# facebookresearch/DLRM-FlexFlow

Hardware: AMD Instinct MI355X
Metric: dlrm_training_samples_per_sec (higher is better)
Workload: dtype f32; 1 GPU; criteo-terabyte-shape: 26 tables (rows 39884406-39043-17289-7420-20263-3-7120-1543-63-38532951-2953546-403346-10-2208-11938-155-4-976-14-39979771-25641295-39664984-585935-12972-108-36), emb_dim 128, bag 1, bot 13-512-256-128, top 3456-1024-1024-512-256-1, cat interaction, SGD lr 0.01, MSE loss; global_batch=32768, per_gpu_batch=32768, parallelism=single GPU, hipGraph-replayed step, step_graph=True

## Files before the change

### dlrm_flexflow_amd/capi.py

```python
from __future__ import annotations

import ctypes as C
import os
import re

_HERE = os.path.dirname(os.path.abspath(__file__))
REPO_ROOT = os.path.dirname(_HERE)
HIP_LIB_PATH = os.path.join(_HERE, "csrc", "libffhip.so")
HEADER_PATH = os.path.join(REPO_ROOT, "include", "ff_hip.h")

FFH_OK = 0
FFH_ERR_BAD_ARG, FFH_ERR_HIP, FFH_ERR_UNSUPPORTED, FFH_ERR_WORKSPACE, FFH_ERR_NOMEM = -1, -2, -3, -4, -5
AC_MODE_NONE, AC_MODE_RELU, AC_MODE_SIGMOID, AC_MODE_TANH, AC_MODE_GELU = 10, 11, 12, 13, 14
AGGR_MODE_NONE, AGGR_MODE_SUM, AGGR_MODE_AVG = 20, 21, 22
MAX_TABLES = 64
EMB_CHUNK, EMB_CHUNK1 = 32, 1024
OPT_ZERO_GRAD = 1
CONCAT_BWD_OVERWRITE = 1
LINEAR_DX_OVERWRITE, LINEAR_ONLY_DW, LINEAR_ONLY_DX, LINEAR_DY_PREMASKED, LINEAR_DX_MASK_BY_X = 1, 2, 4, 8, 16
METRIC_ACCURACY, METRIC_MSE, METRIC_RMSE, METRIC_MAE = 1, 2, 4, 8

P = C.c_void_p
I = C.c_int
L = C.c_int64
# ... 692 lines not shown
        return getattr(self.lib, name)(self.ctx, *conv)

    def call(self, name: str, *args):
        self.base.check(self.rc(name, *args), name)


def cross_api(lib: FFHLib) -> CrossApi:
    return CrossApi(lib)


class AdagradApi:

    def __init__(self, lib: FFHLib):
        self.base = lib
        for name, (res, args) in _SIGS_ADAGRAD.items():
            fn = getattr(lib.lib, name, None)
            if fn is None:
                raise FFHError(f"{lib.path}: no Adagrad extension ({name} missing; include/ff_hip_adagrad.h)")
            fn.restype = res
            fn.argtypes = args
        got = lib.lib.ffh_adagrad_abi_version()
        if got != adagrad_header_abi_version():
            raise FFHError(f"{lib.path}: Adagrad ABI version {got}, include/ff_hip_adagrad.h says {adagrad_header_abi_version()} (rebuild)")
        self.lib = lib.lib
        self.ctx = lib.ctx

    def rc(self, name: str, *args) -> int:
        sig = _SIGS_ADAGRAD[name][1][1:]
        if len(args) != len(sig):
            raise TypeError(f"{name}: expected {len(sig)} args, got {len(args)}")
        conv = [ptr(a) if t is P else a for a, t in zip(args, sig)]
        return getattr(self.lib, name)(self.ctx, *conv)

    def call(self, name: str, *args):
        self.base.check(self.rc(name, *args), name)


def adagrad_api(lib: FFHLib) -> AdagradApi:
    return AdagradApi(lib)


class RowwiseApi:

    def __init__(self, lib: FFHLib):
        self.base = lib
        for name, (res, args) in _SIGS_ROWWISE.items():
            fn = getattr(lib.lib, name, None)
            if fn is None:
                raise FFHError(f"{lib.path}: no row-wise Adagrad extension ({name} missing; include/ff_hip_rowwise.h)")
            fn.restype = res
            fn.argtypes = args
        got = lib.lib.ffh_rowwise_abi_version()
        if got != rowwise_header_abi_version():
            raise FFHError(f"{lib.path}: row-wise Adagrad ABI version {got}, include/ff_hip_rowwise.h says {rowwise_header_abi_version()} (rebuild)")
        self.lib = lib.lib
        self.ctx = lib.ctx


def rowwise_api(lib: FFHLib) -> RowwiseApi:
    return RowwiseApi(lib)


FOLD_HEADER_PATH = os.path.join(REPO_ROOT, "include", "ff_hip_fold.h")


class FoldGroup(C.Structure):
    _fields_ = [("e", P), ("lde", L), ("col0", L), ("p", P), ("rows", L)]


class FoldSeg(C.Structure):
    _fields_ = [("k0", C.c_int32), ("len", C.c_int32)]


_SIGS_FOLD = {
    "ffh_fold_abi_version": (I, []),
    "ffh_fold_product": (I, [P, C.POINTER(FoldGroup), I, P, L, I, I, P]),
    "ffh_fold_gather_add": (I, [P, C.POINTER(EmbTable), I, I, I, L, I, P, L, P]),
    "ffh_fold_linear_fwd": (I, [P, P, L, P, L, P, P, I, I, L, I, C.POINTER(FoldSeg), I, P, L, P]),
    "ffh_fold_linear_fwd_plan": (I, [P, P, L, P, L, P, P, I, I, L, C.POINTER(FoldSeg), I, P, L]),
    "ffh_fold_segment_sum": (I, [P, C.POINTER(EmbTable), I, I, I, L, P]),
    "ffh_fold_dw_product": (I, [P, C.POINTER(FoldGroup), I, P, L, I, I, P]),
    "ffh_fold_linear_bwd_dw": (I, [P, P, L, P, L, P, P, I, I, L, C.POINTER(C.c_int32), I, P]),
    "ffh_fold_linear_bwd_dw_plan": (I, [P, P, L, P, L, P, P, I, I, L, C.POINTER(C.c_int32), I]),
}


def fold_header_symbols(header_path: str = FOLD_HEADER_PATH) -> list[str]:
    m = re.search(r"#define FFH_FOLD_API_LIST\(X\)(.*?)\n\n", open(header_path).read(), re.S)
    if not m:
        raise RuntimeError("FFH_FOLD_API_LIST not found in " + header_path)
    return re.findall(r"X\((\w+)\)", m.group(1))


def fold_header_abi_version(header_path: str = FOLD_HEADER_PATH) -> int:
    m = re.search(r"#define\s+FFH_FOLD_ABI_VERSION\s+(\d+)", open(header_path).read())
    if not m:
        raise RuntimeError("FFH_FOLD_ABI_VERSION not found in " + header_path)
    return int(m.group(1))


class FoldApi:

    def __init__(self, lib: "FFHLib"):
        self.base = lib
        for name, (res, args) in _SIGS_FOLD.items():
            fn = getattr(lib.lib, name, None)
            if fn is None:
                raise FFHError(f"{lib.path}: no fold extension ({name} missing; include/ff_hip_fold.h)")
            fn.restype = res
            fn.argtypes = args
        got = lib.lib.ffh_fold_abi_version()
        if got != fold_header_abi_version():
            raise FFHError(f"{lib.path}: fold ABI version {got}, include/ff_hip_fold.h says {fold_header_abi_version()} (rebuild)")
        self.lib = lib.lib
        self.ctx = lib.ctx

    @staticmethod
    def groups(entries) -> "C.Array":
        entries = list(entries)
        arr = (FoldGroup * len(entries))()
        for k, (e, lde, col0, p, rows) in enumerate(entries):
            arr[k] = FoldGroup(ptr(e), int(lde), int(col0), ptr(p), int(rows))
        return arr

    @staticmethod
    def segs(entries) -> "C.Array":
        entries = list(entries)
        arr = (FoldSeg * max(1, len(entries)))()
        for k, (k0, n) in enumerate(entries):
            arr[k] = FoldSeg(int(k0), int(n))
        return arr

    def rc(self, name: str, *args) -> int:
        sig = _SIGS_FOLD[name][1][1:]
        if len(args) != len(sig):
            raise TypeError(f"{name}: expected {len(sig)} args, got {len(args)}")
        conv = [ptr(a) if t is P else a for a, t in zip(args, sig)]
        return getattr(self.lib, name)(self.ctx, *conv)

    def call(self, name: str, *args):
        self.base.check(self.rc(name, *args), name)


def fold_api(lib: "FFHLib") -> FoldApi:
    return FoldApi(lib)


_hip_singleton: FFHLib | None = None


def load_hip(device: int = 0) -> FFHLib:
    global _hip_singleton
    if _hip_singleton is None:
        import torch
        _hip_singleton = FFHLib(HIP_LIB_PATH, device)
        if not _hip_singleton.backend.startswith("hip"):
            raise FFHError(f"{HIP_LIB_PATH} is not the HIP backend ({_hip_singleton.backend})")
    return _hip_singleton
```

### dlrm_flexflow_amd/csrc/fold.hip

```cpp
#include "fold_sum.h"
#include "linear_gemm.h"

#include "../../include/ff_hip_fold.h"

using namespace ffh_gemm;

namespace {

typedef float f32x4 __attribute__((ext_vector_type(4)));

struct FoldGemmGroup { const float* a; int64_t lda; int64_t wcol0; float* c; int64_t ldc; int rows; int tile0; };
struct FoldGemmArgs {
  FoldGemmGroup grp[FFH_FOLD_MAX_GROUPS];
  ffh_fold_seg  seg[FFH_FOLD_MAX_SEGS];
  const float*  w; int64_t ldw;
  const float*  bias;
  const float*  addend; int64_t ldadd;
  int ngroups, nseg, N, act, ntiles;
};
static_assert(sizeof(FoldGemmArgs) <= 4096, "kernel arguments");

template <bool EPI>
__global__ __launch_bounds__(256) void fold_gemm_kernel(const FoldGemmArgs g) {
  ffh_kernel_prio();
  const int lane = threadIdx.x & 63;
  const int wave = __builtin_amdgcn_readfirstlane((int)(threadIdx.x >> 6));
  const int c = lane & 15, q = lane >> 4;
  const int wt = (int)blockIdx.x * 4 + wave;
  if (wt >= g.ntiles) return;
  int gi = 0;
  while (gi + 1 < g.ngroups && g.grp[gi + 1].tile0 <= wt) gi++;
  const FoldGemmGroup G = g.grp[gi];
  const int ct = g.N / 64, local = wt - G.tile0;
  const int r0 = (local / ct) * 32, n0 = (local % ct) * 64;
  const float* ap[2];
  const float* wp[4];
#pragma unroll
  for (int mt = 0; mt < 2; mt++) {
    int r = r0 + 16 * mt + c;
    if (r > G.rows - 1) r = G.rows - 1;
    ap[mt] = G.a + (int64_t)r * G.lda + 4 * q;
  }
#pragma unroll
  for (int nt = 0; nt < 4; nt++) wp[nt] = g.w + (int64_t)(n0 + 16 * nt + c) * g.ldw + G.wcol0 + 4 * q;
  f32x4 acc[4][2];
#pragma unroll
  for (int nt = 0; nt < 4; nt++)
#pragma unroll
    for (int mt = 0; mt < 2; mt++) acc[nt][mt] = f32x4{0.f, 0.f, 0.f, 0.f};
  for (int si = 0; si < g.nseg; si++) {
    const int k0 = g.seg[si].k0, k1 = k0 + g.seg[si].len;
    for (int k = k0; k < k1; k += 16) {
      f32x4 a[2], b[4];
#pragma unroll
      for (int mt = 0; mt < 2; mt++) a[mt] = *reinterpret_cast<const f32x4*>(ap[mt] + k);
#pragma unroll
      for (int nt = 0; nt < 4; nt++) b[nt] = *reinterpret_cast<const f32x4*>(wp[nt] + k);
#pragma unroll
      for (int e = 0; e < 4; e++)
#pragma unroll
        for (int nt = 0; nt < 4; nt++)
#pragma unroll
          for (int mt = 0; mt < 2; mt++) acc[nt][mt] = __builtin_amdgcn_mfma_f32_16x16x4f32(b[nt][e], a[mt][e], acc[nt][mt], 0, 0, 0);
    }
  }
#pragma unroll
  for (int mt = 0; mt < 2; mt++) {
    const int r = r0 + 16 * mt + c;
    if (r >= G.rows) continue;
#pragma unroll
    for (int nt = 0; nt < 4; nt++) {
      const int n = n0 + 16 * nt + 4 * q;
      f32x4 v = acc[nt][mt];
      if constexpr (EPI) {
        if (g.addend) v += *reinterpret_cast<const f32x4*>(g.addend + (int64_t)r * g.ldadd + n);
        if (g.bias) v += f32x4{g.bias[n], g.bias[n + 1], g.bias[n + 2], g.bias[n + 3]};
        if (g.act != FFH_AC_MODE_NONE) { v.x = act_apply(v.x, g.act); v.y = act_apply(v.y, g.act); v.z = act_apply(v.z, g.act); v.w = act_apply(v.w, g.act); }
      }
      *reinterpret_cast<f32x4*>(G.c + (int64_t)r * G.ldc + n) = v;
    }
  }
}

struct FoldGatherTable { const int64_t* idx; const float* p; };
// ... 25 lines not shown
        }
      }
#pragma unroll
      for (int u = 0; u < 4; u++)
        if (j0 + u < n) acc = (j0 + u == 0) ? v[u] : acc + v[u];
    }
    *reinterpret_cast<f32x4*>(g.S + b * g.ldS + cv) = acc;
  }
}

constexpr int FOLD_DW_EP_LD = 68;
struct FoldDwGroup { const float* g; const float* e; int64_t lde; int64_t col0; int rows; int tile0; };
struct FoldDwArgs {
  FoldDwGroup grp[FFH_FOLD_MAX_GROUPS];
  float* dw; int64_t lddw;
  int ngroups, out, d, ntiles;
};
static_assert(sizeof(FoldDwArgs) <= 4096, "kernel arguments");

__global__ __launch_bounds__(256) void fold_dw_product_kernel(const FoldDwArgs g) {
  __shared__ __attribute__((aligned(16))) float ep_all[4][16 * FOLD_DW_EP_LD];
  ffh_kernel_prio();
  const int lane = threadIdx.x & 63;
  const int wave = __builtin_amdgcn_readfirstlane((int)(threadIdx.x >> 6));
  const int c = lane & 15, q = lane >> 4;
  const int wt = (int)blockIdx.x * 4 + wave;
  if (wt >= g.ntiles) return;
  int gi = 0;
  while (gi + 1 < g.ngroups && g.grp[gi + 1].tile0 <= wt) gi++;
  const FoldDwGroup G = g.grp[gi];
  const int ot = g.out / 64, dt = g.d / 64, local = wt - G.tile0;
  const int chunk = local / (ot * dt), rem = local - chunk * (ot * dt);
  const int o0 = (rem / dt) * 64, d0 = (rem % dt) * 64;
  const int rb = chunk * FFH_FOLD_DW_CHUNK;
  const int re = rb + FFH_FOLD_DW_CHUNK < G.rows ? rb + FFH_FOLD_DW_CHUNK : G.rows;
  const float* gp = G.g + o0 + 4 * c;
  const float* epn = G.e + d0 + 4 * c;
  f32x4 acc[4][4];
#pragma unroll
  for (int tm = 0; tm < 4; tm++)
#pragma unroll
    for (int tn = 0; tn < 4; tn++) acc[tm][tn] = f32x4{0.f, 0.f, 0.f, 0.f};
  f32x4 a[4], b[4], an[4], bn[4];
  auto load16 = [&](int k, f32x4* av, f32x4* bv) {
#pragma unroll
    for (int u = 0; u < 4; u++) {
      const int r = k + 4 * u + q;
      const int rc = r < re ? r : re - 1;
      av[u] = *reinterpret_cast<const f32x4*>(gp + (int64_t)rc * g.out);
      bv[u] = *reinterpret_cast<const f32x4*>(epn + (int64_t)rc * G.lde);
      if (r >= re) av[u] = f32x4{0.f, 0.f, 0.f, 0.f};
    }
  };
  load16(rb, a, b);
  for (int k = rb; k < re; k += 16) {
    if (k + 16 < re) load16(k + 16, an, bn);
#pragma unroll
    for (int u = 0; u < 4; u++)
#pragma unroll
      for (int tm = 0; tm < 4; tm++)
#pragma unroll
        for (int tn = 0; tn < 4; tn++) acc[tm][tn] = __builtin_amdgcn_mfma_f32_16x16x4f32(a[u][tm], b[u][tn], acc[tm][tn], 0, 0, 0);
#pragma unroll
    for (int u = 0; u < 4; u++) { a[u] = an[u]; b[u] = bn[u]; }
  }
  float* const ep = ep_all[wave];
  float* crow = g.dw + (int64_t)o0 * g.lddw + G.col0 + d0 + lane;
#pragma unroll
  for (int p = 0; p < 4; p++) {
    if (q == p) {
#pragma unroll
      for (int tm = 0; tm < 4; tm++)
#pragma unroll
        for (int i = 0; i < 4; i++)
          *reinterpret_cast<f32x4*>(ep + (4 * i + tm) * FOLD_DW_EP_LD + 4 * c) = f32x4{acc[tm][0][i], acc[tm][1][i], acc[tm][2][i], acc[tm][3][i]};
    }
    __builtin_amdgcn_wave_barrier();
#pragma unroll
    for (int r = 0; r < 16; r++) atomicAdd(crow + (int64_t)(16 * p + r) * g.lddw, ep[r * FOLD_DW_EP_LD + lane]);
    __builtin_amdgcn_wave_barrier();
  }
}

inline bool al16(const void* p) { return ((uintptr_t)p & 15) == 0; }

int fold_dw_check(ffh_ctx* c, const float* x, int64_t ldx, const float* dy, int64_t lddy, const float* dw, int in, int out, int64_t batch,
                  const int32_t* kept, int nkept) {
  FFH_REQUIRE(c, in > 0 && out > 0 && batch >= 0 && ldx >= in && lddy >= out, "fold_linear_bwd_dw: bad dims");
  FFH_REQUIRE(c, batch == 0 || (x && dy && dw), "fold_linear_bwd_dw: null pointer");
  FFH_REQUIRE(c, batch < (1LL << 31), "fold_linear_bwd_dw: batch too large");
  FFH_REQUIRE(c, nkept >= 1 && kept, "fold_linear_bwd_dw: bad tile list");
  for (int i = 0; i < nkept; i++)
    FFH_REQUIRE(c, kept[i] >= 0 && ((int64_t)kept[i] + 1) * FFH_FOLD_DW_NTILE <= in && (i == 0 || kept[i] > kept[i - 1]), "fold_linear_bwd_dw: tiles must ascend inside [0, in_dim)");
  return FFH_OK;
}
GemmArgs fold_dw_gemm(const float* x, int64_t ldx, const float* dy, int64_t lddy, float* dw, float* db, int in, int out, int64_t batch) {
  GemmArgs g{};
  g.A = dy; g.sAm = 1; g.sAk = lddy;
  g.B = x; g.sBn = 1; g.sBk = ldx;
  g.C = dw; g.ldc = in;
  g.M = out; g.N = in; g.K = (int)batch;
  g.epi = EPI_ATOMIC; g.act = FFH_AC_MODE_NONE;
  g.db = db;
  return g;
}

int fold_fwd_check(ffh_ctx* c, const float* x, int64_t ldx, const float* y, int64_t ldy, const float* w, int in, int out, int64_t batch,
                   const ffh_fold_seg* keep, int nkeep, const float* addend, int64_t ldadd) {
  FFH_REQUIRE(c, in > 0 && out > 0 && batch >= 0 && ldx >= in && ldy >= out, "fold_linear_fwd: bad dims");
  FFH_REQUIRE(c, batch == 0 || (x && y && w), "fold_linear_fwd: null pointer");
  FFH_REQUIRE(c, batch < (1LL << 31), "fold_linear_fwd: batch too large");
  FFH_REQUIRE(c, nkeep >= 0 && (nkeep == 0 || keep), "fold_linear_fwd: bad segment list");
  FFH_REQUIRE(c, !addend || ldadd >= out, "fold_linear_fwd: bad addend");
  int prev = 0;
  for (int i = 0; i < nkeep; i++) {
    FFH_REQUIRE(c, keep[i].k0 >= prev && keep[i].len > 0 && (int64_t)keep[i].k0 + keep[i].len <= in, "fold_linear_fwd: segments must ascend inside [0, in_dim)");
    prev = keep[i].k0 + keep[i].len;
  }
  return FFH_OK;
}
bool fold_fwd_served(const ffh_ctx* c, const float* x, int64_t ldx, const float* y, int64_t ldy, const float* w, int in, int out,
                     const ffh_fold_seg* keep, int nkeep, const float* addend, int64_t ldadd) {
  if (c->math_mode != FFH_MATH_DEFAULT) return false;
  if (in % FFH_FOLD_KTILE || out % FFH_FOLD_NTILE || nkeep > FFH_FOLD_MAX_SEGS) return false;
  if (!al16(x) || !al16(y) || !al16(w) || ldx % 4 || ldy % 4 || (addend && (!al16(addend) || ldadd % 4))) return false;
  for (int i = 0; i < nkeep; i++)
    if (keep[i].k0 % FFH_FOLD_KTILE || keep[i].len % FFH_FOLD_KTILE) return false;
  return true;
}
bool fold_keep_mask(int in, const ffh_fold_seg* keep, int nkeep, unsigned long long mask[2], int* nk_kept) {
  mask[0] = mask[1] = 0;
  *nk_kept = 0;
  if (in % 64 || in > 128 * 64) return false;
  const ffh_fold_seg all{0, in};
  if (nkeep == 0) { keep = &all; nkeep = 1; }
  for (int i = 0; i < nkeep; i++) {
    if (keep[i].k0 % 64 || keep[i].len % 64) return false;
    for (int kt = keep[i].k0 / 64; kt < (keep[i].k0 + keep[i].len) / 64; kt++) { mask[kt >> 6] |= 1ull << (kt & 63); (*nk_kept)++; }
  }
  return *nk_kept > 0;
}
GemmArgs fold_fwd_gemm(const float* x, int64_t ldx, float* y, int64_t ldy, const float* w, const float* bias, int in, int out, int64_t batch, int act) {
  GemmArgs g{};
  g.A = x; g.sAm = ldx; g.sAk = 1;
  g.B = w; g.sBn = in; g.sBk = 1;
  g.C = y; g.ldc = ldy; g.bias = bias;
  g.M = (int)batch; g.N = out; g.K = in;
  g.epi = EPI_STORE; g.act = act;
  return g;
}

}

extern "C" {

int ffh_fold_abi_version(void) { return FFH_FOLD_ABI_VERSION; }

int ffh_fold_product(ffh_ctx* c, const ffh_fold_group* groups, int ngroups, const float* w, int64_t ldw, int d, int out, ffh_stream s) {
  FFH_REQUIRE(c, groups && w && ngroups >= 1 && d > 0 && out > 0 && ldw >= d, "fold_product: bad arguments");
  if (ngroups > FFH_FOLD_MAX_GROUPS || d % FFH_FOLD_KTILE || out % FFH_FOLD_NTILE || !al16(w) || ldw % 4)
    return ffh_fail(c, FFH_ERR_UNSUPPORTED, "fold_product: d a multiple of 16, out_dim a multiple of 64, at most 64 tables, aligned weight");
  FoldGemmArgs a{};
  int64_t tiles = 0;
  for (int i = 0; i < ngroups; i++) {
    const ffh_fold_group& gr = groups[i];
    FFH_REQUIRE(c, gr.e && gr.p && gr.rows >= 1 && gr.rows < (1LL << 31) && gr.lde >= d && gr.col0 >= 0 && gr.col0 + d <= ldw, "fold_product: bad group");
    if (!al16(gr.e) || !al16(gr.p) || gr.lde % 4 || gr.col0 % FFH_FOLD_KTILE) return ffh_fail(c, FFH_ERR_UNSUPPORTED, "fold_product: group not aligned");
// ... 51 lines not shown
  unsigned long long mask[2]; int nk = 0;
  if (fold_keep_mask(in, keep, nkeep, mask, &nk) && (!bias || al16(bias))) {
    const int r = launch_gemm_sk_fold(c, g, mask, nk, addend, ldadd, false, s, "fold_linear_fwd gemm");
    if (r != 0) return r < 0 ? r : FFH_OK;
  }
  FoldGemmArgs a{};
  a.grp[0] = FoldGemmGroup{x, ldx, 0, y, ldy, (int)batch, 0};
  if (nkeep == 0) { a.seg[0] = ffh_fold_seg{0, in}; a.nseg = 1; }
  else { for (int i = 0; i < nkeep; i++) a.seg[i] = keep[i]; a.nseg = nkeep; }
  const int64_t tiles = ((batch + 31) / 32) * (out / 64);
  FFH_REQUIRE(c, tiles < (1LL << 30), "fold_linear_fwd: too many tiles");
  a.w = w; a.ldw = in; a.bias = bias; a.addend = addend; a.ldadd = ldadd; a.ngroups = 1; a.N = out; a.act = act; a.ntiles = (int)tiles;
  hipLaunchKernelGGL(fold_gemm_kernel<true>, dim3((unsigned)((tiles + 3) / 4)), dim3(256), 0, as_stream(s), a);
  FFH_LAUNCH_CHECK(c, "fold_gemm_kernel (forward)");
  ffh_route_add(c, "fold_linear_fwd gemm|mfma_32x64x16");
  return FFH_OK;
}

int ffh_fold_segment_sum(ffh_ctx* c, const ffh_emb_table* tables, int ntables, int in_dim, int width, int64_t batch, ffh_stream s) {
  FFH_REQUIRE(c, tables && ntables >= 1 && in_dim >= 1 && width > 0 && batch >= 0, "fold_segment_sum: bad arguments");
  if (ntables > FFH_MAX_TABLES || batch * in_dim >= (1LL << 31)) return ffh_fail(c, FFH_ERR_UNSUPPORTED, "fold_segment_sum: at most 64 tables, batch * in_dim < 2^31");
  for (int t = 0; t < ntables; t++)
    FFH_REQUIRE(c, tables[t].weight && tables[t].num_entries >= 1 && (batch == 0 || (tables[t].idx && tables[t].io && tables[t].ld >= width)), "fold_segment_sum: bad table");
  if (batch > 0 && (!c->ws || c->ws_bytes < ffh_embedding_bwd_workspace_bytes(ntables, in_dim, width, batch) || ((uintptr_t)c->ws & 15)))
    return ffh_fail(c, FFH_ERR_WORKSPACE, "fold_segment_sum: workspace too small (ffh_embedding_bwd_workspace_bytes) or not 16-byte aligned");
  if (batch > 0) {
    const int wide = ffh_emb::fold_sum_wide(c, tables, ntables, in_dim, width, batch, s);
    if (wide != 0) return wide < 0 ? wide : FFH_OK;
  }
  for (int t = 0; t < ntables;) {
    char* p0 = (char*)tables[t].weight;
    size_t bytes = 0;
    for (; t < ntables && (char*)tables[t].weight == p0 + bytes; t++) bytes += (size_t)tables[t].num_entries * (size_t)width * 4;
    const int rc = ffh_zero(c, p0, bytes, s);
    if (rc != FFH_OK) return rc;
  }
  if (batch == 0) return FFH_OK;
  return ffh_embedding_bwd_sgd_fused_multi(c, tables, ntables, in_dim, width, batch, FFH_AGGR_MODE_SUM, -1.0f, s);
}

int ffh_fold_dw_product(ffh_ctx* c, const ffh_fold_group* groups, int ngroups, float* dw, int64_t lddw, int d, int out, ffh_stream s) {
  FFH_REQUIRE(c, groups && dw && ngroups >= 1 && d > 0 && out > 0 && lddw >= d, "fold_dw_product: bad arguments");
  if (ngroups > FFH_FOLD_MAX_GROUPS || d % 64 || out % FFH_FOLD_NTILE) return ffh_fail(c, FFH_ERR_UNSUPPORTED, "fold_dw_product: d and out_dim multiples of 64, at most 64 tables");
  FoldDwArgs a{};
  int64_t tiles = 0;
  for (int i = 0; i < ngroups; i++) {
    const ffh_fold_group& gr = groups[i];
    FFH_REQUIRE(c, gr.e && gr.p && gr.rows >= 1 && gr.rows < (1LL << 31) && gr.lde >= d && gr.col0 >= 0 && gr.col0 + d <= lddw, "fold_dw_product: bad group");
    if (!al16(gr.e) || !al16(gr.p) || gr.lde % 4) return ffh_fail(c, FFH_ERR_UNSUPPORTED, "fold_dw_product: group not aligned");
    a.grp[i] = FoldDwGroup{gr.p, gr.e, gr.lde, gr.col0, (int)gr.rows, (int)tiles};
    tiles += ((gr.rows + FFH_FOLD_DW_CHUNK - 1) / FFH_FOLD_DW_CHUNK) * (out / 64) * (d / 64);
    FFH_REQUIRE(c, tiles < (1LL << 30), "fold_dw_product: too many rows");
  }
  a.dw = dw; a.lddw = lddw; a.ngroups = ngroups; a.out = out; a.d = d; a.ntiles = (int)tiles;
  hipLaunchKernelGGL(fold_dw_product_kernel, dim3((unsigned)((tiles + 3) / 4)), dim3(256), 0, as_stream(s), a);
  FFH_LAUNCH_CHECK(c, "fold_dw_product_kernel");
  return FFH_OK;
}

int ffh_fold_linear_bwd_dw_plan(ffh_ctx* c, const float* x, int64_t ldx, const float* dy, int64_t lddy, const float* dw, const float* db, int in, int out,
                                int64_t batch, const int32_t* kept, int nkept) {
  const int rc = fold_dw_check(c, x, ldx, dy, lddy, dw, in, out, batch, kept, nkept);
  if (rc != FFH_OK) return rc;
  if (batch == 0 || c->math_mode != FFH_MATH_DEFAULT) return 0;
  const GemmArgs g = fold_dw_gemm(x, ldx, dy, lddy, const_cast<float*>(dw), const_cast<float*>(db), in, out, batch);
  if (!gemm_sk_serves(c, g, SK_FORM_DW)) return 0;
  return launch_gemm_sk_kept(c, g, kept, nkept, true, nullptr, "") == 1 ? 1 : 0;
}

int ffh_fold_linear_bwd_dw(ffh_ctx* c, const float* x, int64_t ldx, const float* dy, int64_t lddy, float* dw, float* db, int in, int out, int64_t batch,
                           const int32_t* kept, int nkept, ffh_stream s) {
  const int rc = fold_dw_check(c, x, ldx, dy, lddy, dw, in, out, batch, kept, nkept);
  if (rc != FFH_OK) return rc;
  ffh_route_clear(c);
  if (batch == 0 || c->math_mode != FFH_MATH_DEFAULT) return ffh_fail(c, FFH_ERR_UNSUPPORTED, "fold_linear_bwd_dw: empty batch / math mode not served");
  const GemmArgs g = fold_dw_gemm(x, ldx, dy, lddy, dw, db, in, out, batch);
  if (!gemm_sk_serves(c, g, SK_FORM_DW)) return ffh_fail(c, FFH_ERR_UNSUPPORTED, "fold_linear_bwd_dw: the layer's weight gradient does not run the stream-K form");
  const int r = launch_gemm_sk_kept(c, g, kept, nkept, false, s, "fold_linear_bwd_dw gemm");
  if (r < 0) return r;
  if (r == 0) return ffh_fail(c, FFH_ERR_UNSUPPORTED, "fold_linear_bwd_dw: too few kept tiles for the stream-K form, deterministic mode, or a bias gradient without tile 0");
  return FFH_OK;
}

}
```

### dlrm_flexflow_amd/csrc/linear_gemm.h

```cpp
#pragma once
#include "ffh_common.h"

#include <hip/hip_runtime.h>

namespace ffh_gemm {

typedef float f32x16 __attribute__((ext_vector_type(16)));

enum { EPI_STORE = 0, EPI_ADD = 1, EPI_ATOMIC = 2 };

struct GemmArgs {
  const float* A;
  const float* B;
  float*       C;
  const float* bias;
  int64_t sAm, sAk, sBn, sBk, ldc;
  int64_t bsA, bsB, bsC;
  int M, N, K;
  int k_per_split;
  int splitk;
  int epi;
  int act;
  const float* act_y;
  int64_t      ld_act_y;
  float*       db;
  int          fuse;
  const float* mask;
  int64_t      ldmask;
  const ffh_col_dest* colmap;
  float* colsum;
  const unsigned short* A16;
  const unsigned short* B16;
  unsigned short*       C16;
  int                   a_not_twinned;
  int                   db_done;
};

constexpr int kSplitGran = 32;

__device__ __forceinline__ float act_apply(float v, int act) {
  if (act == FFH_AC_MODE_RELU) return v > 0.0f ? v : 0.0f;
  if (act == FFH_AC_MODE_SIGMOID) return 1.0f / (1.0f + expf(-v));
  if (act == FFH_AC_MODE_GELU) {
    constexpr float B = 0.7978845608028654f, C = 0.035677408136300125f;
    return v * (0.5f + 0.5f * tanhf(v * (C * v * v + B)));
  }
  return v;
}

__device__ __forceinline__ float4 load4_guard(const float* p, bool row_ok, int c0, int climit, bool vec_ok) {
  float4 v = make_float4(0.f, 0.f, 0.f, 0.f);
  if (!row_ok) return v;
  if (vec_ok && c0 + 3 < climit) return ld4u(p);
  if (c0 + 0 < climit) v.x = p[0];
  if (c0 + 1 < climit) v.y = p[1];
  if (c0 + 2 < climit) v.z = p[2];
  if (c0 + 3 < climit) v.w = p[3];
  return v;
}

template <typename K>
bool glds_set_lds(K kern, int bytes) {
  if (hipFuncSetAttribute((const void*)kern, hipFuncAttributeMaxDynamicSharedMemorySize, bytes) != hipSuccess) { (void)hipGetLastError(); return false; }
  return true;
}

inline bool use_bf16(const ffh_ctx* c, int in, int out, int64_t batch) {
  if (in < FFH_BF16_MIN_DIM || out < FFH_BF16_MIN_DIM) return false;
  if (c->math_mode == FFH_MATH_TENSOR_OP_BF16) return true;
  return c->math_mode == FFH_MATH_FP32_SPLIT_BF16X3_ALL || (c->math_mode == FFH_MATH_FP32_SPLIT_BF16X3 && 2.0 * (double)batch * (double)in * (double)out >= FFH_BF16X3_MIN_FLOP);
}

enum { BF16_FORM_FWD = 0,
       BF16_FORM_DW = 1,
       BF16_FORM_DX = 2,
       BF16_FORM_DX_MASK = 3 };
int launch_gemm_bf16_form(ffh_ctx* c, GemmArgs& g, int form, ffh_stream s, const char* name);
int launch_gemm_bf16_dma(ffh_ctx* c, const GemmArgs& g, int form, ffh_stream s, const char* name);
int launch_gemm_x3_dma(ffh_ctx* c, const GemmArgs& g, int form, ffh_stream s, const char* name);
float* dw_tile_slots(const ffh_ctx* c, ffh_stream s, int64_t tiles, int splitk, int64_t ldc);
void launch_dw_tile_reduce(const float* slots, float* C, int64_t ldc, int M, int N, int64_t tiles, int splitk, ffh_stream s);

enum { SK_FORM_FWD = 0, SK_FORM_DX = 1, SK_FORM_DW = 2 };
bool gemm_sk_serves(const ffh_ctx* c, const GemmArgs& g, int form);
int launch_gemm_sk(ffh_ctx* c, const GemmArgs& g, int form, ffh_stream s, const char* name);
int launch_gemm_sk_fold(ffh_ctx* c, const GemmArgs& g, const unsigned long long keep[2], int nk_kept, const float* addend, int64_t ldadd, bool dry,
                        ffh_stream s, const char* name);
int launch_gemm_sk_kept(ffh_ctx* c, const GemmArgs& g, const int* tiles, int nkept, bool dry, ffh_stream s, const char* name);

}
```

### dlrm_flexflow_amd/csrc/linear_sk.hip

```cpp
#include "linear_gemm.h"

#include <stdlib.h>
#include <atomic>
#include <type_traits>
#include <utility>

using namespace ffh_gemm;

namespace {

typedef float f32x4 __attribute__((ext_vector_type(4)));
typedef unsigned u32x4 __attribute__((ext_vector_type(4)));

constexpr int SK_BM = 128, SK_BN = 128, SK_BK = 64;
constexpr int SK_LDS_KC = 128 * 256 + 32 * 32;
constexpr int SK_LDS_KR = 64 * 512;
constexpr int sk_lds_kc_a(int TMW) { return 32 * TMW * 256 + 32 * 32; }

enum { SK_EPI_FWD = 0, SK_EPI_DX_STORE = 1, SK_EPI_DX_ADD = 2, SK_EPI_DW_ATOMIC = 3, SK_EPI_DX_CMAP = 4 };

struct SkArgs {
  const float* A; const float* B; float* C;
  const float* bias;
  float*       db;
  const float* mask;
  const ffh_col_dest* colmap;
  float*       colsum;
  int64_t lda, ldb, ldc, ldmask;
  int M, N, K;
  int act;
  unsigned a_bytes, b_bytes, bias_bytes, mask_bytes;
  float*    sk_slots;
  unsigned* sk_cnt;
};

struct SkArgsFold : SkArgs {
  unsigned long long keep[2];
  unsigned           nk_kept;
  const float*       addend;
  int64_t            ldadd;
};

struct SkArgsKept : SkArgs {
  unsigned       nkept;
  unsigned short tile[128];
};

template <int... I, class F>
__device__ __forceinline__ void sk_static_for_impl(std::integer_sequence<int, I...>, F&& f) { (f(std::integral_constant<int, I>{}), ...); }
template <int N_, class F>
__device__ __forceinline__ void sk_static_for(F&& f) { sk_static_for_impl(std::make_integer_sequence<int, N_>{}, static_cast<F&&>(f)); }

#define SK_PIN() __builtin_amdgcn_sched_barrier(0)

constexpr int SK_EP_LD = 68;
constexpr int SK_EP_ROWS = 16;
constexpr int SK_EP_WAVE = SK_EP_ROWS * SK_EP_LD * 4;

template <bool AKR, bool BKR, int EPI, bool DB = false, bool SPLIT = false, int TMW = 4, bool FOLD = false, bool KEPT = false>
__global__ __launch_bounds__(256, 1) void gemm_sk_kernel(const std::conditional_t<KEPT, SkArgsKept, std::conditional_t<FOLD, SkArgsFold, SkArgs>> g) {
  static_assert(!KEPT || (EPI == SK_EPI_DW_ATOMIC && AKR && BKR && !FOLD), "kept column tiles: the weight-gradient form");
  static_assert(!FOLD || (EPI == SK_EPI_FWD && !SPLIT && !DB && TMW == 4), "kept k-tiles + addend: the whole-tile forward form");
  static_assert(!DB || (EPI == SK_EPI_DW_ATOMIC && AKR), "the bias gradient rides on the weight-gradient form");
  static_assert(!SPLIT || EPI != SK_EPI_DW_ATOMIC, "the weight gradient meets by atomics");
  static_assert(TMW == 4 || (TMW == 2 && !AKR && EPI != SK_EPI_DW_ATOMIC), "64-row tiles: forward and data gradient (A k-contiguous)");
  extern __shared__ __attribute__((aligned(16))) char sk_lds[];
  constexpr bool ATOMIC = EPI == SK_EPI_DW_ATOMIC;
  constexpr bool STREAMK = ATOMIC || SPLIT;
  constexpr int BM = 32 * TMW;
  constexpr int NM = 64 * TMW;
  constexpr int NPA = 2 * TMW, NP = NPA + 8;
  constexpr int LDS_A = AKR ? SK_LDS_KR : sk_lds_kc_a(TMW);
  char* const ldsA = sk_lds;
  char* const ldsB = sk_lds + LDS_A;
  const int tid = threadIdx.x, lane = tid & 63;
  const int wave = __builtin_amdgcn_readfirstlane(tid >> 6);
  const int wy = wave >> 1, wx = wave & 1;
  const int c16 = lane & 15, q = lane >> 4;

  const int fra = AKR ? (q * 2048 + wy * 256 + c16 * 16) : ((16 * TMW * wy + TMW * c16) * 256 + (16 * wy + c16) * 32 + q * 16);
  const int frb = BKR ? (q * 2048 + wx * 256 + c16 * 16) : ((64 * wx + 4 * c16) * 256 + (16 * wx + c16) * 32 + q * 16);
  const int srowA = AKR ? (tid >> 5) : (tid >> 4), schA = AKR ? (tid & 31) : (tid & 15);
  const int srowB = BKR ? (tid >> 5) : (tid >> 4), schB = BKR ? (tid & 31) : (tid & 15);
  const unsigned voffA = (unsigned)((srowA * g.lda + schA * 4) * 4);
  const unsigned voffB = (unsigned)((srowB * g.ldb + schB * 4) * 4);
  const int swA = AKR ? (srowA * 512 + schA * 16) : (srowA * 256 + (srowA / TMW) * 32 + schA * 16);
  const int swB = BKR ? (srowB * 512 + schB * 16) : (srowB * 256 + (srowB >> 2) * 32 + schB * 16);
  constexpr int SW_STEP_A = AKR ? 4096 : (4096 + (16 / TMW) * 32), SW_STEP_B = BKR ? 4096 : 4224;
  const unsigned ioffA = (unsigned)((AKR ? 8 : 16) * g.lda * 4), ioffB = (unsigned)((BKR ? 8 : 16) * g.ldb * 4);
  const unsigned kadvA = AKR ? (unsigned)(SK_BK * g.lda * 4) : (unsigned)(SK_BK * 4), kadvB = BKR ? (unsigned)(SK_BK * g.ldb * 4) : (unsigned)(SK_BK * 4);

  const __amdgpu_buffer_rsrc_t rsA = __builtin_amdgcn_make_buffer_rsrc(const_cast<float*>(g.A), 0, g.a_bytes, 0x00020000);
  const __amdgpu_buffer_rsrc_t rsB = __builtin_amdgcn_make_buffer_rsrc(const_cast<float*>(g.B), 0, g.b_bytes, 0x00020000);

  unsigned nbx = (unsigned)(g.N / SK_BN);
  if constexpr (KEPT) nbx = g.nkept;
  const unsigned nby = (unsigned)(g.M / BM), ntiles = nbx * nby;
  unsigned nk = (unsigned)(g.K / SK_BK);
  if constexpr (FOLD) nk = g.nk_kept;
  auto first_kept = [&]() -> unsigned {
    if constexpr (FOLD) return g.keep[0] ? (unsigned)__builtin_ctzll(g.keep[0]) : 64u + (unsigned)__builtin_ctzll(g.keep[1]);
    else return 0u;
  };
  auto next_kept = [&](unsigned p) -> unsigned {
    if constexpr (FOLD) {
      p++;
      if (p < 64u) {
        const unsigned long long m = g.keep[0] >> p;
        if (m) return p + (unsigned)__builtin_ctzll(m);
        p = 64u;
      }
      const unsigned long long m = p < 128u ? g.keep[1] >> (p - 64u) : 0ull;
      return m ? p + (unsigned)__builtin_ctzll(m) : p;
    } else return p + 1u;
  };
  const unsigned G = gridDim.x, w = blockIdx.x;
  const unsigned total_it = ntiles * nk;
  const unsigned wperm = (w & 7u) * (G >> 3) + (w >> 3);
  unsigned it_b, it_e;
  const unsigned ipw = (total_it + G - 1) / G;
  const unsigned rng = SPLIT ? wperm : w;
  if (STREAMK) {
    it_b = rng * ipw; it_e = it_b + ipw < total_it ? it_b + ipw : total_it;
    if (it_b > total_it) it_b = total_it;
  } else {
    const unsigned mine = ntiles / G + (wperm < ntiles % G ? 1u : 0u);
    it_b = 0; it_e = mine * nk;
  }
  const unsigned n_it = it_e - it_b;
  if (n_it == 0) return;

  struct Cursor { unsigned seq, kt, m0, n0, offA, offB, kp; };
  auto place = [&](Cursor& c) {
    unsigned lin;
    if (STREAMK) lin = it_b / nk + c.seq;
    else lin = c.seq * G + wperm;
    if (lin >= ntiles) lin = ntiles - 1;
    const unsigned by = lin / nbx, bx = lin - by * nbx;
    c.m0 = by * BM;
    if constexpr (KEPT) c.n0 = (unsigned)g.tile[bx] * SK_BN;
    else c.n0 = bx * SK_BN;
    c.kp = FOLD ? first_kept() : c.kt;
    c.offA = (AKR ? c.m0 * 4u : (unsigned)(c.m0 * g.lda * 4)) + c.kp * kadvA;
    c.offB = (BKR ? c.n0 * 4u : (unsigned)(c.n0 * g.ldb * 4)) + c.kp * kadvB;
// ... 382 lines not shown
    const hipError_t e = hipGetLastError();
    if (e == hipErrorInvalidValue || e == hipErrorInvalidConfiguration || e == hipErrorLaunchOutOfResources || e == hipErrorSharedObjectInitFailed) return 0;
    if (e != hipSuccess) return ffh_fail_hip(c, e, name);
  }
  { char tok[96]; snprintf(tok, sizeof tok, "%s|sk_%dx128x64%s%s%s|wgs=%d", name, 32 * p.tmw, g.colmap ? "|colmap" : "", p.split ? "|streamk" : "", a.colsum ? "|colsum" : "", G); ffh_route_add(c, tok); }
  return 1;
}

int launch_gemm_sk_fold(ffh_ctx* c, const GemmArgs& g, const unsigned long long keep[2], int nk_kept, const float* addend, int64_t ldadd, bool dry,
                        ffh_stream s, const char* name) {
  if (g.K % SK_BK || g.K > 128 * SK_BK || nk_kept < 1 || nk_kept > g.K / SK_BK) return 0;
  if (addend && !sk_aligned(addend, ldadd)) return 0;
  GemmArgs gk = g;
  gk.K = nk_kept * SK_BK;
  SkPlan p{};
  if (!sk_plan(c, gk, SK_FORM_FWD, p) || p.split || p.tmw != 4) return 0;
  const int64_t a_bytes = ((int64_t)(g.M - 1) * p.lda + g.K) * 4, b_bytes = ((int64_t)(g.N - 1) * p.ldb + g.K) * 4;
  if (a_bytes >= (1LL << 32) || b_bytes >= (1LL << 32)) return 0;
  if (dry) return 1;
  SkArgsFold a{};
  a.A = g.A; a.B = g.B; a.C = g.C; a.bias = g.bias;
  a.lda = p.lda; a.ldb = p.ldb; a.ldc = g.ldc;
  a.M = g.M; a.N = g.N; a.K = g.K; a.act = g.act;
  a.a_bytes = (unsigned)a_bytes; a.b_bytes = (unsigned)b_bytes;
  a.bias_bytes = g.bias ? (unsigned)g.N * 4u : 0u;
  a.keep[0] = keep[0]; a.keep[1] = keep[1]; a.nk_kept = (unsigned)nk_kept; a.addend = addend; a.ldadd = ldadd;
  {
    auto kern = gemm_sk_kernel<false, false, SK_EPI_FWD, false, false, 4, true>;
    constexpr int LDSB = 2 * SK_LDS_KC;
    static std::atomic<signed char> ok[64];
    const int dev = c->device & 63;
    if (ok[dev].load(std::memory_order_acquire) == 0) ok[dev].store(sk_set_lds(kern, LDSB) ? 1 : -1, std::memory_order_release);
    if (ok[dev].load(std::memory_order_acquire) < 0) return 0;
    hipLaunchKernelGGL(kern, dim3((unsigned)p.G), dim3(256), LDSB, as_stream(s), a);
    const hipError_t e = hipGetLastError();
    if (e == hipErrorInvalidValue || e == hipErrorInvalidConfiguration || e == hipErrorLaunchOutOfResources || e == hipErrorSharedObjectInitFailed) return 0;
    if (e != hipSuccess) return ffh_fail_hip(c, e, name);
  }
  { char tok[96]; snprintf(tok, sizeof tok, "%s|sk_128x128x64|kept=%d/%d%s|wgs=%d", name, nk_kept, g.K / SK_BK, addend ? "|addend" : "", p.G); ffh_route_add(c, tok); }
  return 1;
}

int launch_gemm_sk_kept(ffh_ctx* c, const GemmArgs& g, const int* tiles, int nkept, bool dry, ffh_stream s, const char* name) {
  if (g.N % SK_BN || g.N / SK_BN > 128 || nkept < 1 || nkept > g.N / SK_BN) return 0;
  for (int i = 0; i < nkept; i++)
    if (tiles[i] < 0 || tiles[i] >= g.N / SK_BN || (i > 0 && tiles[i] <= tiles[i - 1])) return 0;
  if (g.db && tiles[0] != 0) return 0;
  GemmArgs gk = g;
  gk.N = nkept * SK_BN;
  SkPlan p{};
  if (!sk_plan(c, gk, SK_FORM_DW, p)) return 0;
  const int64_t b_bytes = ((int64_t)(g.K - 1) * p.ldb + g.N) * 4;
  if (b_bytes >= (1LL << 32)) return 0;
  if (dry) return 1;
  SkArgsKept a{};
  a.A = g.A; a.B = g.B; a.C = g.C; a.db = g.db;
  a.lda = p.lda; a.ldb = p.ldb; a.ldc = g.ldc;
  a.M = g.M; a.N = g.N; a.K = g.K; a.act = g.act;
  a.a_bytes = (unsigned)p.a_bytes; a.b_bytes = (unsigned)b_bytes;
  a.nkept = (unsigned)nkept;
  for (int i = 0; i < nkept; i++) a.tile[i] = (unsigned short)tiles[i];
  constexpr int LDSB = 2 * SK_LDS_KR + 4 * SK_EP_WAVE;
#define FFH_SK_KEPT_LAUNCH(DBV)                                                                                  \
  {                                                                                                              \
    auto kern = gemm_sk_kernel<true, true, SK_EPI_DW_ATOMIC, DBV, false, 4, false, true>;                        \
    static std::atomic<signed char> ok[64];       \
    const int dev = c->device & 63;                                                                              \
    if (ok[dev].load(std::memory_order_acquire) == 0) ok[dev].store(sk_set_lds(kern, LDSB) ? 1 : -1, std::memory_order_release); \
    if (ok[dev].load(std::memory_order_acquire) < 0) return 0;                                                   \
    hipLaunchKernelGGL(kern, dim3((unsigned)p.G), dim3(256), LDSB, as_stream(s), a);                             \
  }
  if (g.db) FFH_SK_KEPT_LAUNCH(true)
  else FFH_SK_KEPT_LAUNCH(false)
#undef FFH_SK_KEPT_LAUNCH
  {
    const hipError_t e = hipGetLastError();
    if (e == hipErrorInvalidValue || e == hipErrorInvalidConfiguration || e == hipErrorLaunchOutOfResources || e == hipErrorSharedObjectInitFailed) return 0;
    if (e != hipSuccess) return ffh_fail_hip(c, e, name);
  }
  { char tok[96]; snprintf(tok, sizeof tok, "%s|sk_128x128x64|kept=%d/%d%s|wgs=%d", name, nkept, g.N / SK_BN, g.db ? "|db" : "", p.G); ffh_route_add(c, tok); }
  return 1;
}

}
```

### dlrm_flexflow_amd/host/backend.cc

```cpp
#include "backend.h"

#include <dlfcn.h>
#include <cstdio>
#include <cstdlib>
#include <map>
#include <mutex>

static bool g_env_override = false;
std::string default_backend_path() {
  if (const char* e = getenv("FFH_BACKEND_LIB")) { g_env_override = true; return std::string(e); }
  Dl_info info;
  std::string dir = ".";
  if (dladdr((void*)&default_backend_path, &info) && info.dli_fname) {
    std::string p(info.dli_fname);
    size_t k = p.rfind('/');
    if (k != std::string::npos) dir = p.substr(0, k);
  }
  return dir + "/../csrc/libffhip.so";
}

const KernelApi* load_kernel_api(const std::string& path_in) {
  static std::map<std::string, KernelApi*>& cache = *new std::map<std::string, KernelApi*>();
  static std::mutex mu;
  std::lock_guard<std::mutex> lock(mu);
  const std::string path = path_in.empty() ? default_backend_path() : path_in;
  auto it = cache.find(path);
  if (it != cache.end()) return it->second;
  void* h = dlopen(path.c_str(), RTLD_NOW | RTLD_LOCAL);
  if (!h) {
    fprintf(stderr, "FATAL: cannot load kernel library %s: %s\n"
                    "       build it with: python -c 'import __graft_entry__ as g; g.build()'\n", path.c_str(), dlerror());
    abort();
  }
  KernelApi* api = new KernelApi();
  api->handle = h;
  api->path = path;
  api->overridden = !path_in.empty() || g_env_override;
#define FFH_LOAD(name)                                                        \
  api->name = reinterpret_cast<decltype(api->name)>(dlsym(h, #name));         \
  if (!api->name) {                                                           \
    fprintf(stderr, "FATAL: %s does not export %s\n", path.c_str(), #name);   \
    abort();                                                                  \
  }
  FFH_API_LIST(FFH_LOAD)
#undef FFH_LOAD
  if (api->ffh_abi_version() != FFH_ABI_VERSION) {
    fprintf(stderr, "FATAL: %s has ABI version %d, expected %d\n", path.c_str(), api->ffh_abi_version(), FFH_ABI_VERSION);
    abort();
  }
  if (dlsym(h, "ffh_bf16_abi_version")) {
    KernelApiBf16* b = new KernelApiBf16();
#define FFH_LOAD(name)                                                        \
  b->name = reinterpret_cast<decltype(b->name)>(dlsym(h, #name));             \
  if (!b->name) {                                                             \
    fprintf(stderr, "FATAL: %s exports part of include/ff_hip_bf16.h: %s is missing\n", path.c_str(), #name);   \
    abort();                                                                  \
  }
    FFH_BF16_API_LIST(FFH_LOAD)
#undef FFH_LOAD
    if (b->ffh_bf16_abi_version() != FFH_BF16_ABI_VERSION) {
      fprintf(stderr, "FATAL: %s has bf16 ABI version %d, expected %d\n", path.c_str(), b->ffh_bf16_abi_version(), FFH_BF16_ABI_VERSION);
      abort();
    }
    api->bf16 = b;
  }
  if (dlsym(h, "ffh_ctr_abi_version")) {
    KernelApiCtr* b = new KernelApiCtr();
#define FFH_LOAD(name)                                                        \
  b->name = reinterpret_cast<decltype(b->name)>(dlsym(h, #name));             \
  if (!b->name) {                                                             \
    fprintf(stderr, "FATAL: %s exports part of include/ff_hip_ctr.h: %s is missing\n", path.c_str(), #name);   \
    abort();                                                                  \
  }
    FFH_CTR_API_LIST(FFH_LOAD)
#undef FFH_LOAD
    if (b->ffh_ctr_abi_version() != FFH_CTR_ABI_VERSION) {
      fprintf(stderr, "FATAL: %s has CTR ABI version %d, expected %d\n", path.c_str(), b->ffh_ctr_abi_version(), FFH_CTR_ABI_VERSION);
      abort();
    }
    api->ctr = b;
  }
  if (dlsym(h, "ffh_lr_abi_version")) {
    KernelApiLr* b = new KernelApiLr();
#define FFH_LOAD(name)                                                        \
  b->name = reinterpret_cast<decltype(b->name)>(dlsym(h, #name));             \
  if (!b->name) {                                                             \
    fprintf(stderr, "FATAL: %s exports part of include/ff_hip_lr.h: %s is missing\n", path.c_str(), #name);   \
// ... 9 lines not shown
  }
  if (dlsym(h, "ffh_data_abi_version")) {
    KernelApiData* b = new KernelApiData();
#define FFH_LOAD(name)                                                        \
  b->name = reinterpret_cast<decltype(b->name)>(dlsym(h, #name));             \
  if (!b->name) {                                                             \
    fprintf(stderr, "FATAL: %s exports part of include/ff_hip_data.h: %s is missing\n", path.c_str(), #name);   \
    abort();                                                                  \
  }
    FFH_DATA_API_LIST(FFH_LOAD)
#undef FFH_LOAD
    if (b->ffh_data_abi_version() != FFH_DATA_ABI_VERSION) {
      fprintf(stderr, "FATAL: %s has data ABI version %d, expected %d\n", path.c_str(), b->ffh_data_abi_version(), FFH_DATA_ABI_VERSION);
      abort();
    }
    api->data = b;
  }
  if (dlsym(h, "ffh_cross_abi_version")) {
    KernelApiCross* b = new KernelApiCross();
#define FFH_LOAD(name)                                                        \
  b->name = reinterpret_cast<decltype(b->name)>(dlsym(h, #name));             \
  if (!b->name) {                                                             \
    fprintf(stderr, "FATAL: %s exports part of include/ff_hip_cross.h: %s is missing\n", path.c_str(), #name);   \
    abort();                                                                  \
  }
    FFH_CROSS_API_LIST(FFH_LOAD)
#undef FFH_LOAD
    if (b->ffh_cross_abi_version() != FFH_CROSS_ABI_VERSION) {
      fprintf(stderr, "FATAL: %s has cross ABI version %d, expected %d\n", path.c_str(), b->ffh_cross_abi_version(), FFH_CROSS_ABI_VERSION);
      abort();
    }
    api->cross = b;
  }
  if (dlsym(h, "ffh_digest_abi_version")) {
    KernelApiDigest* b = new KernelApiDigest();
#define FFH_LOAD(name)                                                        \
  b->name = reinterpret_cast<decltype(b->name)>(dlsym(h, #name));             \
  if (!b->name) {                                                             \
    fprintf(stderr, "FATAL: %s exports part of include/ff_hip_digest.h: %s is missing\n", path.c_str(), #name);   \
    abort();                                                                  \
  }
    FFH_DIGEST_API_LIST(FFH_LOAD)
#undef FFH_LOAD
    if (b->ffh_digest_abi_version() != FFH_DIGEST_ABI_VERSION) {
      fprintf(stderr, "FATAL: %s has digest ABI version %d, expected %d\n", path.c_str(), b->ffh_digest_abi_version(), FFH_DIGEST_ABI_VERSION);
      abort();
    }
    api->digest = b;
  }
  if (dlsym(h, "ffh_adagrad_abi_version")) {
    KernelApiAdagrad* b = new KernelApiAdagrad();
#define FFH_LOAD(name)                                                        \
  b->name = reinterpret_cast<decltype(b->name)>(dlsym(h, #name));             \
  if (!b->name) {                                                             \
    fprintf(stderr, "FATAL: %s exports part of include/ff_hip_adagrad.h: %s is missing\n", path.c_str(), #name);   \
    abort();                                                                  \
  }
    FFH_ADAGRAD_API_LIST(FFH_LOAD)
#undef FFH_LOAD
    if (b->ffh_adagrad_abi_version() != FFH_ADAGRAD_ABI_VERSION) {
      fprintf(stderr, "FATAL: %s has Adagrad ABI version %d, expected %d\n", path.c_str(), b->ffh_adagrad_abi_version(), FFH_ADAGRAD_ABI_VERSION);
      abort();
    }
    api->adagrad = b;
  }
  if (dlsym(h, "ffh_rowwise_abi_version")) {
    KernelApiRowwise* b = new KernelApiRowwise();
#define FFH_LOAD(name)                                                        \
  b->name = reinterpret_cast<decltype(b->name)>(dlsym(h, #name));             \
  if (!b->name) {                                                             \
    fprintf(stderr, "FATAL: %s exports part of include/ff_hip_rowwise.h: %s is missing\n", path.c_str(), #name);   \
    abort();                                                                  \
  }
    FFH_ROWWISE_API_LIST(FFH_LOAD)
#undef FFH_LOAD
    if (b->ffh_rowwise_abi_version() != FFH_ROWWISE_ABI_VERSION) {
      fprintf(stderr, "FATAL: %s has row-wise Adagrad ABI version %d, expected %d\n", path.c_str(), b->ffh_rowwise_abi_version(), FFH_ROWWISE_ABI_VERSION);
      abort();
    }
    api->rowwise = b;
  }
  if (dlsym(h, "ffh_fold_abi_version")) {
    KernelApiFold* b = new KernelApiFold();
#define FFH_LOAD(name)                                                        \
  b->name = reinterpret_cast<decltype(b->name)>(dlsym(h, #name));             \
  if (!b->name) {                                                             \
    fprintf(stderr, "FATAL: %s exports part of include/ff_hip_fold.h: %s is missing\n", path.c_str(), #name);   \
    abort();                                                                  \
  }
    FFH_FOLD_API_LIST(FFH_LOAD)
#undef FFH_LOAD
    if (b->ffh_fold_abi_version() != FFH_FOLD_ABI_VERSION) {
      fprintf(stderr, "FATAL: %s has fold ABI version %d, expected %d\n", path.c_str(), b->ffh_fold_abi_version(), FFH_FOLD_ABI_VERSION);
      abort();
    }
    api->fold = b;
  }
  if (path_in.empty() && g_env_override)
    fprintf(stderr, "[DLRM] FFH_BACKEND_LIB: kernel library %s (%s)\n", path.c_str(), api->ffh_backend_name());
  cache[path] = api;
  return api;
}
```

### dlrm_flexflow_amd/host/ffmodel.h

```cpp
#pragma once

#include <cstddef>
#include <cstdint>
#include <condition_variable>
#include <deque>
#include <functional>
#include <map>
#include <mutex>
#include <thread>
#include <string>
#include <vector>

#include "../../include/ff_hip.h"
#include "../../include/ff_hip_bf16.h"
#include "../../include/ff_hip_ctr.h"
#include "../../include/ff_hip_lr.h"
#include "../../include/ff_hip_cross.h"
#include "../../include/ff_hip_adagrad.h"
#include "../../include/ff_hip_rowwise.h"
#include "../../include/ff_hip_fold.h"
#include "ffcomm.h"

enum ActiMode { AC_MODE_NONE = 10, AC_MODE_RELU = 11, AC_MODE_SIGMOID = 12, AC_MODE_TANH = 13, AC_MODE_GELU = 14 };
enum AggrMode { AGGR_MODE_NONE = 20, AGGR_MODE_SUM = 21, AGGR_MODE_AVG = 22 };
// ... 8 lines not shown
};
enum CompMode { COMP_MODE_TRAINING = 70, COMP_MODE_INFERENCE = 71 };
enum ParameterSyncType { NONE = 80, PS = 81, NCCL = 82 };
enum MetricsType {
  METRICS_ACCURACY = 1001,
  METRICS_CATEGORICAL_CROSSENTROPY = 1002,
  METRICS_SPARSE_CATEGORICAL_CROSSENTROPY = 1004,
  METRICS_MEAN_SQUARED_ERROR = 1008,
  METRICS_ROOT_MEAN_SQUARED_ERROR = 1016,
  METRICS_MEAN_ABSOLUTE_ERROR = 1032,
  METRICS_BINARY_CROSSENTROPY = 2001,
  METRICS_AUC = 2002,
};
enum OperatorType { OP_INPUT, OP_LINEAR, OP_EMBEDDING, OP_CONCAT, OP_BATCHMATMUL, OP_TRANSPOSE, OP_RESHAPE, OP_FLAT, OP_TRIL, OP_DOT_INTERACTION, OP_CROSS_COMBINE };

#define MAX_TENSOR_DIM 4
#define MAX_NUM_INPUTS 256
#define MAX_OPNAME 64

class FFModel;
class Op;
struct KernelApi;

struct ParallelConfig {
  enum DeviceType { GPU = 0, CPU = 1 };
  ParallelConfig() : device_type(GPU), nDims(0) { for (int& d : dim) d = 1; }
  int num_parts() const { int n = 1; for (int i = 0; i < nDims; i++) n *= dim[i]; return n; }
  bool is_data_parallel() const;
  bool operator==(const ParallelConfig& rhs) const;
  DeviceType device_type;
  int nDims, dim[MAX_TENSOR_DIM];
  std::vector<int> device_ids;
};
typedef size_t MappingTagID;
bool load_strategies_from_file(const std::string& filename, std::map<MappingTagID, ParallelConfig>& strategies);
bool save_strategies_to_file(const std::string& filename, const std::map<std::string, ParallelConfig>& strategies);

class FFConfig {
 public:
  FFConfig();
  void parse_args(char** argv, int argc);
  int epochs, batchSize, printFreq;
  int numNodes, cpusPerNode, workersPerNode;
  float learningRate, weightDecay;
  size_t workSpaceSize;
  bool syntheticInput, profiling, perform_fusion;
  CompMode computationMode;
  std::string dataset_path;
  std::string import_strategy_file, export_strategy_file;
  std::map<MappingTagID, ParallelConfig> strategies;
  static MappingTagID get_hash_id(const std::string& pcname);
  bool find_parallel_config(int ndims, const std::string& pcname, ParallelConfig& config) const;
  std::string save_checkpoint_dir, load_checkpoint_dir;
  int checkpoint_every_epochs;
  std::string backend_lib;
  int device;
  uint64_t seed;
  bool enable_graph;
  bool overlap_embedding;
  bool dense_embedding_update;
  int64_t column_shard_rows;
  bool deterministic;
  bool fp32_split_bf16x3;
  bool allow_tensor_op_math_conversion;
  bool bf16_convert_twins;
  bool bf16_exact_small_backward;
  bool bf16_twins, force_async_launch;
  bool capture_exchange;
  bool pad_linear_k;
  bool sparse_embedding_optimizer;
  int early_sort;
  bool dx_colsum;
  bool dx_scatter;
  bool fuse_pair;
  int  bucket_allreduce;
  bool direct_allreduce;
  int64_t allreduce_bucket_floats;
  int64_t big_dw_min_weights;
  int  big_dw_chunks;
  int  trace_mode;
  bool fold_small_tables;
  int64_t fold_max_rows;
  bool fold_dw;
  bool mlp_chain;
  int64_t mlp_chain_max_batch;
  int64_t mlp_chain_fwd_max_batch;
  int64_t mlp_chain_fwd_min_batch;
  int64_t mlp_chain_max_weights;
  bool attach_events;
  bool timing_events;
  int driver_loss;
  int eval_batches;
  int synthetic_labels;
  bool eval_only;
  int data_randomize;
  bool fuse_loss;
  int64_t replicate_embedding_rows;
  int64_t row_shard_rows;
  bool async_launch;
  bool parallel_dw;
  bool force_exchange;
  DataType embedding_dtype;
  int embedding_rounding;
  int64_t lr_warmup_steps, lr_decay_start_step, lr_num_decay_steps;
  bool device_lr;
  bool host_lr_schedule;
  double adagrad_eps;
  double adagrad_initial_accumulator;
  bool adagrad_rowwise;
  ffcomm comm;
};

struct TensorPiece {
  float*  ptr;
  float*  grad;
  int64_t ld;
  int     cols;
};

struct TensorImpl {
  void*   ptr = nullptr;
  int64_t ld = 0;
  float*  grad = nullptr;
  int64_t grad_ld = 0;
  bool    alias = false;
  bool    grad_alias = false;
  bool    is_input = false;
  size_t  bytes = 0;
  int64_t rows_local = 0;
  int     guid = -1;
  std::vector<TensorPiece> pieces;
};

struct Tensor {
  Tensor(void);
  size_t get_volume() const;
  int64_t rows() const;
  int64_t cols() const { return adim[0]; }
  template <typename T> bool set_tensor(const FFModel* model, const std::vector<int>& dims, const T* data);
  template <typename T> bool get_tensor(const FFModel* model, T* data) const;
  template <typename T> bool get_grad(const FFModel* model, T* data) const;
  int numDim, adim[MAX_TENSOR_DIM];
  DataType data_type;
  ParameterSyncType sync_type;
  Op* owner_op;
  int owner_idx;
  TensorImpl* impl;
};

struct Parameter : Tensor {
  template <typename T> bool set_weights(const FFModel* model, const std::vector<int>& dims, const T* data);
  template <typename T> bool get_weights(const FFModel* model, T* data) const;
};

class Initializer {
 public:
  virtual ~Initializer() {}
  virtual void init(const FFModel* ff, const Parameter* p) = 0;
};
class ZeroInitializer : public Initializer {
 public:
  void init(const FFModel* ff, const Parameter* p) override;
};
class ConstantInitializer : public Initializer {
 public:
  explicit ConstantInitializer(float v) : value(v) {}
// ... 362 lines not shown
  bool use_workers() const { return dw_worker != nullptr && capturing_trace < 0; }
  ffh_event ev_fork, ev_join, ev_grad_ready, ev_update_done;
  int rank, world_size;
  bool exchange;
  int64_t local_batch;
  bool compiled;

  void* dmalloc(size_t bytes) const;
  void check(int rc, const char* what) const;

  std::vector<Embedding*> embeddings;
  void embedding_group_forward(ffh_stream s, ffh_ctx* on_ctx = nullptr) const;
  void replicated_embedding_grads() const;
  void embedding_group_update(ffh_stream s, ffh_ctx* on_ctx = nullptr) const;
  void embedding_kernels_only(bool fwd, ffh_stream s, const std::vector<const int64_t*>* idx_override = nullptr) const;
  mutable bool probe_events_on = false;
  static constexpr int kProbeEvents = 30;
  mutable ffh_event probe_ev[kProbeEvents] = {};
  void probe_record(int which, ffh_stream s, ffh_ctx* cx) const;
  uint64_t* bf16_counter = nullptr;
  ffh_bf16_rounding bf16_rounding() const;
  uint64_t read_bf16_counter() const;
  void advance_bf16_counter(ffh_stream s, ffh_ctx* cx) const;
  size_t bf16_tables_per_launch() const;
  enum LrRoute { kLrOff = 0, kLrHost = 1, kLrDevice = 2 };
  int lr_route = kLrOff;
  std::string lr_route_why;
  double lr_base = 0.0;
  int64_t lr_host_steps = 0;
  ffh_lr_state* lr_block[2] = {nullptr, nullptr};
  void lr_choose_route();
  void lr_allocate();
  void lr_host_set(int64_t k);
  void advance_lr(int which, ffh_stream s, ffh_ctx* cx) const;
  double current_lr();
  int64_t lr_steps();
  std::string lr_schedule_line() const;
  struct CheckpointInfo { int64_t epochs_done = 0, steps = 0; uint64_t digest = 0; size_t bytes = 0; };
  CheckpointInfo save_checkpoint(const std::string& dir, int64_t epochs_done);
  CheckpointInfo load_checkpoint(const std::string& dir);
  uint64_t state_digest();
  int64_t n_update_calls = 0;
  uint64_t* digest_acc = nullptr;
  mutable int64_t n_graph_replays = 0;
  mutable int64_t n_early_sorts = 0;
  bool fused_embedding_update() const;
  bool sparse_rule(ffh_sparse_opt& rule) const;
  mutable bool opt_next_done = false;
  void embedding_dense_update() const;
  void issue_embedding_forward_on_side_stream() const;
  void join_embedding_forward() const;
  void issue_embedding_update_on_side_stream() const;
  void order_input_writes_behind_update() const;
  void profiled(const Op* op, bool fwd, const std::function<void()>& fn) const;
  mutable bool emb_forward_issued, emb_forward_joined, emb_update_pending;
  static constexpr int early_sort_big_batch_mode = 0;
  bool early_sort_possible(int where) const;
  mutable bool emb_sorted_early;
  int scatter_attach_layer;
  std::vector<Initializer*> owned_initializers;
  int grad_attach_layer;
  void* w_twin = nullptr; void* act_twin = nullptr; void* grad_twin = nullptr;
  mutable bool w_twin_dirty = false;
  void refresh_weight_twin() const;
  int64_t weight_mirror_stale_bytes();
  void note_weight_write(const void* p) const;
  mutable bool bwd_alltoall_issued = false;
  int n_twin_regions = 0;
  struct FoldRoute {
    Linear* layer = nullptr;
    std::vector<Embedding*> tables;
    std::vector<ffh_fold_group> groups;
    std::vector<ffh_emb_table> gather;
    std::vector<ffh_fold_seg> keep;
    float* P = nullptr;
    float* S = nullptr;
    std::vector<Embedding*> dw_tables;
    std::vector<ffh_emb_table> dw_sum;
    std::vector<ffh_fold_group> dw_groups;
    std::vector<int32_t> dw_kept;
    float* G = nullptr;
    ffh_ctx* sum_ctx = nullptr;
    void* sum_ws = nullptr;
  } fold;
  ffh_event ev_fold_e_read = nullptr;
  mutable bool fold_e_read_recorded = false;
  void fold_weight_gradient(const Linear* li, float* dbp, ffh_stream dws) const;
  ffh_event ev_fold_w = nullptr;
  ffh_event ev_fold_done = nullptr;
  mutable bool fold_w_recorded = false, fold_on_side = false;
  void plan_fold();
  void plan_fold_dw(FoldRoute& r);
  void fold_products_and_sum(ffh_stream s, ffh_ctx* cx) const;
  void fold_linear_forward(const Linear* li) const;
  int z_reader_layer;
  ffh_event ev_z_free;
  mutable bool z_free_recorded;
  mutable bool grad_ready_attached;

  float *mlp_weights, *mlp_grads;  size_t mlp_count;
  char* act_slab;
  char* act_grad_slab;  size_t act_grad_bytes;
  void* workspace;  size_t workspace_bytes;
  void* repl_workspace;  size_t repl_workspace_bytes;
  ffh_perf_metrics* d_perf;
  float* d_bce_sum;
  ffh_ctr_eval* d_eval;
  bool want_eval;
  bool evaluating;
  struct EmbShard { Embedding* e; int owner; int col0; int cols; int64_t off; };
  std::vector<EmbShard> shards;
  std::vector<int64_t> rank_width;
  float *xsend, *xrecv, *gsend, *grecv;
  std::vector<int64_t> fwd_send_counts, fwd_recv_counts;
  std::vector<int> owned_tables;
  int tables_of_rank(int r) const;

  std::map<int, ffh_graph> graphs;
  int capturing_trace, replaying_trace;
  struct TraceTune { int calls = 0; int decided = 0; ffh_event ev[4] = {nullptr, nullptr, nullptr, nullptr}; float eager_ms = 0.f, graph_ms = 0.f; };
  std::map<int, TraceTune> trace_tune;
  bool trace_adaptive() const { return config.trace_mode == 0 && !exchange; }
  bool trace_replays(int trace_id) const;
  mutable bool inputs_dirty;
  mutable bool fork_recorded;

  std::vector<TensorImpl*> tensor_impls;
  std::vector<Tensor*> input_tensors;
 private:
  void allocate();
  void apply_strategies();
};
```

### dlrm_flexflow_amd/host/ffmodel_c.cc

```cpp
#include <cstring>
#include "ffmodel_c.h"
#include <string>

#include <chrono>

#include <cstdio>
#include <cstdlib>
#include <vector>

#include "backend.h"
#include "dlrm.h"
#include "ffmodel.h"

namespace {
FFConfig* C(flexflow_config_t h) { return (FFConfig*)h.impl; }
FFModel* M(flexflow_model_t h) { return (FFModel*)h.impl; }
Tensor* T(flexflow_tensor_t h) { return (Tensor*)h.impl; }
Initializer* I(flexflow_initializer_t h) { return (Initializer*)h.impl; }
DLRMApp* A(flexflow_dlrm_t h) { return (DLRMApp*)h.impl; }
flexflow_tensor_t wrap(const Tensor& t) { flexflow_tensor_t h; h.impl = new Tensor(t); return h; }
std::vector<int> dims_vec(const int* dims, int n) { return std::vector<int>(dims, dims + n); }
}

extern "C" {
// ... 71 lines not shown
}
flexflow_tensor_t flexflow_model_add_batch_matmul(flexflow_model_t m, flexflow_tensor_t a, flexflow_tensor_t b, int asd, int bsd) {
  return wrap(M(m)->batch_matmul(*T(a), *T(b), asd, bsd));
}
flexflow_initializer_t flexflow_zero_initializer_create(void) { flexflow_initializer_t h; h.impl = new ZeroInitializer(); return h; }
flexflow_initializer_t flexflow_uniform_initializer_create(int seed, float lo, float hi) { flexflow_initializer_t h; h.impl = new UniformInitializer(seed, lo, hi); return h; }
flexflow_initializer_t flexflow_norm_initializer_create(int seed, float mean, float sd) { flexflow_initializer_t h; h.impl = new NormInitializer(seed, mean, sd); return h; }
flexflow_initializer_t flexflow_glorot_uniform_initializer_create(int seed) { flexflow_initializer_t h; h.impl = new GlorotUniform(seed); return h; }
flexflow_sgd_optimizer_t flexflow_sgd_optimizer_create(flexflow_model_t m, double lr, double mom, bool nest, double wd) {
  flexflow_sgd_optimizer_t h; h.impl = new SGDOptimizer(M(m), lr, mom, nest, wd); return h;
}
void flexflow_model_set_sgd_optimizer(flexflow_model_t m, flexflow_sgd_optimizer_t o) { M(m)->optimizer = (SGDOptimizer*)o.impl; }
flexflow_adam_optimizer_t flexflow_adam_optimizer_create(flexflow_model_t m, double alpha, double b1, double b2, double wd, double eps) {
  flexflow_adam_optimizer_t h; h.impl = new AdamOptimizer(M(m), alpha, b1, b2, wd, eps); return h;
}
void flexflow_adam_optimizer_set_lr(flexflow_adam_optimizer_t o, double lr) { ((AdamOptimizer*)o.impl)->alpha = lr; }
void flexflow_model_set_adam_optimizer(flexflow_model_t m, flexflow_adam_optimizer_t o) { M(m)->optimizer = (AdamOptimizer*)o.impl; }
int64_t flexflow_model_weight_mirror_stale_bytes(flexflow_model_t m) { return M(m)->weight_mirror_stale_bytes(); }
void flexflow_config_set_adagrad(flexflow_config_t h, double eps, double acc) { C(h)->adagrad_eps = eps; C(h)->adagrad_initial_accumulator = acc; }
flexflow_adagrad_optimizer_t flexflow_adagrad_optimizer_create(flexflow_model_t m, double lr, double wd, double eps, double acc) {
  flexflow_adagrad_optimizer_t h;
  h.impl = new AdagradOptimizer(M(m), lr, wd, eps != eps ? M(m)->config.adagrad_eps : eps, acc != acc ? M(m)->config.adagrad_initial_accumulator : acc);
  return h;
}
void flexflow_model_set_adagrad_optimizer(flexflow_model_t m, flexflow_adagrad_optimizer_t o) { M(m)->optimizer = (AdagradOptimizer*)o.impl; }
void flexflow_config_set_adagrad_rowwise(flexflow_config_t h, int on) { C(h)->adagrad_rowwise = on != 0; }
void flexflow_adagrad_optimizer_set_rowwise(flexflow_adagrad_optimizer_t o, int on) { ((AdagradOptimizer*)o.impl)->rowwise = on != 0; }
void flexflow_model_compile(flexflow_model_t m, int loss, const int* metrics, int nb, int comp_mode) {
  std::vector<MetricsType> v;
  for (int i = 0; i < nb; i++) v.push_back((MetricsType)metrics[i]);
  M(m)->compile((LossType)loss, v, (CompMode)comp_mode);
}
void flexflow_model_init_layers(flexflow_model_t m) { M(m)->init_layers(); }
void flexflow_model_reset_metrics(flexflow_model_t m) { M(m)->reset_metrics(); }
void flexflow_model_forward(flexflow_model_t m, int sl) { M(m)->forward(sl); }
void flexflow_model_zero_gradients(flexflow_model_t m) { M(m)->zero_gradients(); }
void flexflow_model_backward(flexflow_model_t m, int sl) { M(m)->backward(sl); }
void flexflow_model_update(flexflow_model_t m) { M(m)->update(); }
void flexflow_model_begin_trace(flexflow_model_t m, int id) { M(m)->begin_trace(id); }
void flexflow_model_end_trace(flexflow_model_t m, int id) { M(m)->end_trace(id); }
void flexflow_model_sync(flexflow_model_t m) { M(m)->sync(); }
const char* flexflow_model_get_backend_name(flexflow_model_t m) { return M(m)->api->ffh_backend_name(); }
const char* flexflow_model_get_backend_path(flexflow_model_t m) { return M(m)->api->path.c_str(); }
void flexflow_model_get_perf_metrics(flexflow_model_t m, flexflow_perf_metrics_t* out) {
  PerfMetrics p = M(m)->get_perf_metrics();
  out->train_all = p.train_all; out->train_correct = p.train_correct; out->cce_loss = p.cce_loss;
  out->sparse_cce_loss = p.sparse_cce_loss; out->mse_loss = p.mse_loss; out->rmse_loss = p.rmse_loss; out->mae_loss = p.mae_loss;
}
flexflow_tensor_t flexflow_model_get_label_tensor(flexflow_model_t m) { return wrap(M(m)->label_tensor); }
int flexflow_model_get_num_layers(flexflow_model_t m) { return (int)M(m)->layers.size(); }
const char* flexflow_model_get_layer_name(flexflow_model_t m, int l) { return M(m)->layers.at(l)->name; }
int flexflow_model_get_layer_num_weights(flexflow_model_t m, int l) { return M(m)->layers.at(l)->numWeights; }
flexflow_tensor_t flexflow_model_get_parameter(flexflow_model_t m, int l, int i) {
  Op* op = M(m)->layers.at(l);
  if (i < 0 || i >= op->numWeights) { fprintf(stderr, "FATAL: %s has %d weights\n", op->name, op->numWeights); abort(); }
  return wrap(op->weights[i]);
}
flexflow_tensor_t flexflow_model_get_layer_output(flexflow_model_t m, int l) { return wrap(M(m)->layers.at(l)->outputs[0]); }
void* flexflow_model_get_stream(flexflow_model_t m) { return M(m)->stream; }
double flexflow_model_get_current_lr(flexflow_model_t m) { return M(m)->current_lr(); }
int flexflow_model_uses_graph(flexflow_model_t m) { return M(m)->config.enable_graph ? 1 : 0; }
void flexflow_model_set_trace_mode(flexflow_model_t m, int mode) { M(m)->config.trace_mode = mode; }
int flexflow_model_trace_replays(flexflow_model_t m, int trace_id) { return M(m)->trace_replays(trace_id) ? 1 : 0; }
int64_t flexflow_model_get_counter(flexflow_model_t m, const char* name) {
  const std::string n(name ? name : "");
  if (n == "mlp_chain_fwd_calls") return M(m)->n_chain_fwd_calls;
  if (n == "mlp_chain_bwd_calls") return M(m)->n_chain_bwd_calls;
  if (n == "fused_loss_calls") return M(m)->n_fused_loss_calls;
  if (n == "allreduce_bucket_calls") return M(m)->n_bucket_allreduces;
  if (n == "allreduce_buckets") return (int64_t)M(m)->grad_buckets.size();
  if (n.rfind("allreduce_bucket_floats_", 0) == 0) {
    const size_t k = (size_t)atoi(n.c_str() + 24);
    return k < M(m)->grad_buckets.size() ? (int64_t)M(m)->grad_buckets[k].count : -1;
  }
  if (n == "allreduce_bucket_channel_own") return M(m)->config.comm.bucket_channel_own;
  if (n == "direct_allreduces") return M(m)->n_direct_allreduces;
  if (n == "bf16_updates") return (int64_t)M(m)->read_bf16_counter();
  if (n == "early_sorts") return M(m)->n_early_sorts;
  if (n == "lr_steps") return M(m)->lr_steps();
  if (n == "lr_route") return M(m)->lr_route;
  if (n == "graph_replays") return M(m)->n_graph_replays;
  if (n == "folded_tables") return (int64_t)M(m)->fold.tables.size();
  if (n == "folded_dw_tables") return (int64_t)M(m)->fold.dw_tables.size();
  if (n == "tensor_op_exact_backward_layers") {
    int64_t k = 0;
    for (Op* op : M(m)->layers) if (op->op_type == OP_LINEAR && static_cast<Linear*>(op)->bwd_exact) k++;
    return k;
  }
  return -1;
}

int flexflow_model_save_checkpoint(flexflow_model_t m, const char* dir, int64_t epochs_done) { M(m)->save_checkpoint(dir ? dir : "", epochs_done); return 0; }
int flexflow_model_load_checkpoint(flexflow_model_t m, const char* dir, int64_t* epochs_done) {
  const FFModel::CheckpointInfo info = M(m)->load_checkpoint(dir ? dir : "");
  if (epochs_done) *epochs_done = info.epochs_done;
  return 0;
}
uint64_t flexflow_model_state_digest(flexflow_model_t m) { return M(m)->state_digest(); }
uint64_t flexflow_state_digest_host(const void* base, int64_t rows, int64_t row_bytes, int64_t ld_bytes, uint64_t seed, uint64_t index_base) {
  return ffh_state_digest_host(base, rows, row_bytes, ld_bytes, seed, index_base);
}
uint64_t flexflow_digest_record_seed(uint64_t ordinal) { return ffh_digest_record_seed(ordinal); }

int flexflow_tensor_get_num_dims(flexflow_tensor_t t) { return T(t)->numDim; }
void flexflow_tensor_get_dims(flexflow_tensor_t t, int* dims) { for (int i = 0; i < T(t)->numDim; i++) dims[i] = T(t)->adim[T(t)->numDim - 1 - i]; }
int64_t flexflow_tensor_get_local_rows(flexflow_tensor_t t) { return T(t)->impl ? T(t)->impl->rows_local : 0; }
bool flexflow_tensor_is_local(flexflow_tensor_t t) { return T(t)->impl && T(t)->impl->ptr != nullptr; }
void* flexflow_tensor_get_device_ptr(flexflow_tensor_t t) { return T(t)->impl ? T(t)->impl->ptr : nullptr; }
int64_t flexflow_tensor_get_ld(flexflow_tensor_t t) { return T(t)->impl ? T(t)->impl->ld : 0; }
void flexflow_tensor_set_float(flexflow_tensor_t t, flexflow_model_t m, const int* dims, int nd, const float* d) { T(t)->set_tensor<float>(M(m), dims_vec(dims, nd), d); }
void flexflow_tensor_set_int64(flexflow_tensor_t t, flexflow_model_t m, const int* dims, int nd, const int64_t* d) { T(t)->set_tensor<int64_t>(M(m), dims_vec(dims, nd), d); }
void flexflow_tensor_get_float(flexflow_tensor_t t, flexflow_model_t m, float* d) { T(t)->get_tensor<float>(M(m), d); }
void flexflow_tensor_get_int64(flexflow_tensor_t t, flexflow_model_t m, int64_t* d) { T(t)->get_tensor<int64_t>(M(m), d); }
void flexflow_tensor_get_grad_float(flexflow_tensor_t t, flexflow_model_t m, float* d) { T(t)->get_grad<float>(M(m), d); }
int flexflow_tensor_get_data_type(flexflow_tensor_t t) { return (int)T(t)->data_type; }
void flexflow_tensor_set_bf16(flexflow_tensor_t t, flexflow_model_t m, const int* dims, int nd, const uint16_t* d) {
  if (T(t)->data_type != DT_BF16) { fprintf(stderr, "FATAL: flexflow_tensor_set_bf16: not a bf16 tensor\n"); abort(); }
  T(t)->set_tensor<uint16_t>(M(m), dims_vec(dims, nd), d);
}
void flexflow_tensor_get_bf16(flexflow_tensor_t t, flexflow_model_t m, uint16_t* d) {
  if (T(t)->data_type != DT_BF16) { fprintf(stderr, "FATAL: flexflow_tensor_get_bf16: not a bf16 tensor\n"); abort(); }
  T(t)->get_tensor<uint16_t>(M(m), d);
}

flexflow_dlrm_t flexflow_dlrm_create(int argc, char** argv, const ffcomm* comm) { flexflow_dlrm_t h; h.impl = new DLRMApp(argc, argv, comm); return h; }
void flexflow_dlrm_destroy(flexflow_dlrm_t h) { delete A(h); }
int flexflow_dlrm_get_start_epoch(flexflow_dlrm_t h) { return A(h)->start_epoch; }
flexflow_model_t flexflow_dlrm_get_model(flexflow_dlrm_t h) { flexflow_model_t m; m.impl = A(h)->ff; return m; }
int flexflow_dlrm_get_num_samples(flexflow_dlrm_t h) { return A(h)->loader->num_samples; }
int flexflow_dlrm_get_num_tables(flexflow_dlrm_t h) { return (int)A(h)->sparse_inputs.size(); }
flexflow_tensor_t flexflow_dlrm_get_sparse_input(flexflow_dlrm_t h, int t) { return wrap(A(h)->sparse_inputs.at(t)); }
flexflow_tensor_t flexflow_dlrm_get_dense_input(flexflow_dlrm_t h) { return wrap(A(h)->dense_input); }
void flexflow_dlrm_warmup(flexflow_dlrm_t h) { A(h)->warmup(); }
static void to_c(const EvalMetrics& m, flexflow_eval_metrics_t* out) {
  out->samples = m.samples; out->positives = m.positives; out->correct = m.correct; out->nan_predictions = m.nan_predictions;
  out->logloss_sum = m.logloss_sum; out->auc = m.auc;
}
double flexflow_dlrm_evaluate(flexflow_dlrm_t h, int epoch, flexflow_eval_metrics_t* out) {
  EvalMetrics m;
  const double secs = A(h)->evaluate(epoch, &m);
  if (out) to_c(m, out);
  return secs;
}
float flexflow_perf_metrics_get_bce_loss(flexflow_model_t m) { return M(m)->get_perf_metrics().bce_loss; }
void flexflow_model_eval_batch(flexflow_model_t m) { M(m)->eval_batch(); }
void flexflow_model_reset_eval_metrics(flexflow_model_t m) { M(m)->reset_eval_metrics(); }
void flexflow_model_get_eval_metrics(flexflow_model_t m, flexflow_eval_metrics_t* out, uint64_t* hist_pos, uint64_t* hist_neg) {
  const EvalMetrics e = M(m)->get_eval_metrics(hist_pos || hist_neg);
  to_c(e, out);
  if (hist_pos) memcpy(hist_pos, e.hist_pos.data(), sizeof(uint64_t) * FFH_AUC_BINS);
  if (hist_neg) memcpy(hist_neg, e.hist_neg.data(), sizeof(uint64_t) * FFH_AUC_BINS);
}
int flexflow_auc_bins(void) { return FFH_AUC_BINS; }
double flexflow_auc_from_histograms(const uint64_t* hist_pos, const uint64_t* hist_neg, int bins) { return ffh_auc_from_histograms(hist_pos, hist_neg, bins); }
void flexflow_dlrm_train_steps(flexflow_dlrm_t h, int n, bool trace) { A(h)->train_steps(n, trace); }
double flexflow_dlrm_run_epochs(flexflow_dlrm_t h) { return A(h)->run_epochs(); }

void flexflow_dlrm_probe_step(flexflow_dlrm_t h, int iters, float* out, int nout) {
  DLRMApp* app = A(h);
  FFModel* ff = app->ff;
  for (int k = 0; k < nout; k++) out[k] = 0.0f;
  if (!app->warmed_up) app->warmup();
  ff->sync();
  ff->probe_events_on = true;
  const int npairs = FFModel::kProbeEvents / 2;
  std::vector<double> sum(npairs, 0.0);
// ... 115 lines not shown
```

### dlrm_flexflow_amd/host/model.cc

```cpp
#include "ffmodel.h"
#include "model_internal.h"


LaunchWorker::LaunchWorker(const KernelApi* _api, int _device) : api(_api), device(_device), wctx(nullptr), stop(false), busy(false) {
  th = std::thread([this] { run(); });
  drain();
}
LaunchWorker::~LaunchWorker() {
  {
    std::lock_guard<std::mutex> lk(mu);
    stop = true;
  }
  cv.notify_all();
  if (th.joinable()) th.join();
  if (wctx) api->ffh_ctx_destroy(wctx);
}
void LaunchWorker::run() {
  {
    ffh_ctx* c = nullptr;
    if (api->ffh_ctx_create(&c, device) != FFH_OK) die("launch worker: ffh_ctx_create(device %d) failed", device);
    std::lock_guard<std::mutex> lk(mu);
    wctx = c;
  }
  cv_idle.notify_all();
// ... 263 lines not shown
    c.overlap_embedding = false; c.enable_graph = false; c.parallel_dw = false; c.async_launch = false;
    c.fuse_pair = false; c.mlp_chain = false; c.attach_events = false; c.dx_scatter = false; c.timing_events = true;
  }
  return c;
}

FFModel::FFModel(FFConfig& _config)
    : op_global_guid(100), config(profiling_schedule(_config)), optimizer(nullptr), loss_type(LOSS_MEAN_SQUARED_ERROR_AVG_REDUCE),
      metrics_flags(0), seq_length(-1), api(nullptr), ctx(nullptr), stream(nullptr), side_stream(nullptr),
      ev_fork(nullptr), ev_join(nullptr), ev_grad_ready(nullptr), ev_update_done(nullptr), compiled(false),
      emb_forward_issued(false), emb_forward_joined(false), emb_update_pending(false), emb_sorted_early(false), mlp_weights(nullptr), mlp_grads(nullptr), mlp_count(0),
      act_slab(nullptr), act_grad_slab(nullptr), act_grad_bytes(0), workspace(nullptr), workspace_bytes(0), repl_workspace(nullptr), repl_workspace_bytes(0), d_perf(nullptr), d_bce_sum(nullptr), d_eval(nullptr), want_eval(false), evaluating(false),
      xsend(nullptr), xrecv(nullptr), gsend(nullptr), grecv(nullptr), capturing_trace(-1), replaying_trace(-1), inputs_dirty(true), fork_recorded(false) {
  seed_counter = 0;
  dw_stream = nullptr; ev_dw_done = nullptr; big_dw_layer = -1; need_zero_act_grads = true; need_zero_gsend = true; dw_forked = false; mlp_grads_clean = false; dw_worker = side_worker = nullptr;
  rank = config.comm.world_size > 1 ? config.comm.rank : 0;
  world_size = config.comm.world_size > 1 ? config.comm.world_size : 1;
  if (world_size == 1 && config.workersPerNode > 1)
    die("-ll:gpu %d: one process per GPU and no communicator was supplied; use the `dlrm` binary (it starts its own %d ranks),\n"
        "       python dlrm_flexflow_amd/run_dlrm.py <flags>, or bench.py --gpus %d",
        config.workersPerNode, config.workersPerNode, config.workersPerNode);
  if (world_size > 1 && (!config.comm.alltoall_f32 || !config.comm.allreduce_sum_f32))
    die("world_size %d needs the ffcomm callbacks", world_size);
  if (config.batchSize % world_size != 0) die("batch size %d is not divisible by %d ranks", config.batchSize, world_size);
  local_batch = config.batchSize / world_size;
  exchange = world_size > 1 || (config.force_exchange && config.comm.alltoall_f32 && config.comm.allreduce_sum_f32);
  api = load_kernel_api(config.backend_lib);
  int rc = api->ffh_ctx_create(&ctx, config.device);
  if (rc != FFH_OK || !ctx) die("ffh_ctx_create(device %d) failed with %d on %s -- no usable GPU?", config.device, rc, api->path.c_str());
  if (config.allow_tensor_op_math_conversion) check(api->ffh_ctx_set_math_mode(ctx, FFH_MATH_TENSOR_OP_BF16), "tensor-op math mode");
  else if (config.fp32_split_bf16x3) check(api->ffh_ctx_set_math_mode(ctx, FFH_MATH_FP32_SPLIT_BF16X3), "split-bf16x3 math mode");
  if (config.deterministic) { check(api->ffh_ctx_set_deterministic(ctx, 1), "deterministic mode"); config.async_launch = false; }
  check(api->ffh_stream_create(ctx, &stream), "stream create");
  check(api->ffh_ctx_reserve_scratch(ctx, stream), "reserve scratch");
  check(api->ffh_stream_create(ctx, &side_stream), "stream create");
  check(api->ffh_stream_create(ctx, &dw_stream), "stream create");
  check(api->ffh_ctx_reserve_scratch(ctx, dw_stream), "reserve scratch");
  check(api->ffh_stream_create(ctx, &ar_stream), "stream create");
  check((config.timing_events ? api->ffh_event_create : api->ffh_event_create_sync)(ctx, &ev_dw_done), "event create");
  check((config.timing_events ? api->ffh_event_create : api->ffh_event_create_sync)(ctx, &ev_z_free), "event create");
  z_reader_layer = -1; z_free_recorded = false;
  dw_worker = side_worker = nullptr;
  if (config.async_launch && (std::string(api->ffh_backend_name()).rfind("hip", 0) == 0 || config.force_async_launch)) {
    dw_worker = new LaunchWorker(api, config.device);
    side_worker = new LaunchWorker(api, config.device);
    const int mm = config.allow_tensor_op_math_conversion ? FFH_MATH_TENSOR_OP_BF16 : (config.fp32_split_bf16x3 ? FFH_MATH_FP32_SPLIT_BF16X3 : FFH_MATH_DEFAULT);
    if (mm != FFH_MATH_DEFAULT) {
      check(api->ffh_ctx_set_math_mode(dw_worker->ctx(), mm), "math mode");
      check(api->ffh_ctx_set_math_mode(side_worker->ctx(), mm), "math mode");
    }
  }
  check((config.timing_events ? api->ffh_event_create : api->ffh_event_create_sync)(ctx, &ev_fork), "event create");
  check((config.timing_events ? api->ffh_event_create : api->ffh_event_create_sync)(ctx, &ev_join), "event create");
  check((config.timing_events ? api->ffh_event_create : api->ffh_event_create_sync)(ctx, &ev_grad_ready), "event create");
  check((config.timing_events ? api->ffh_event_create : api->ffh_event_create_sync)(ctx, &ev_update_done), "event create");
}

FFModel::~FFModel() {
  if (!ctx) return;
  delete dw_worker; delete side_worker;
  api->ffh_device_sync(ctx);
  for (ffh_event e : layer_events) api->ffh_event_destroy(ctx, e);
  for (auto& kv : graphs) api->ffh_graph_destroy(ctx, kv.second);
  for (TensorImpl* t : tensor_impls) {
    if (t->ptr && !t->alias && t->bytes) api->ffh_free(ctx, t->ptr);
    delete t;
  }
  for (void* p : {w_twin, act_twin, grad_twin, (void*)ar_scratch}) if (p) api->ffh_free(ctx, p);
  for (void* p : {(void*)mlp_weights, (void*)mlp_grads, (void*)act_slab, (void*)act_grad_slab, workspace, repl_workspace, (void*)d_perf, (void*)d_bce_sum, (void*)d_eval, (void*)digest_acc, (void*)xsend,
                  (void*)xrecv, (void*)gsend, (void*)grecv})
    if (p) api->ffh_free(ctx, p);
  for (Embedding* e : embeddings)
    for (void* p : {(void*)e->local_idx, (void*)e->partial, (void*)e->gfull, (void*)e->opt_state[0], (void*)e->opt_state[1]})
      if (p) api->ffh_free(ctx, p);
  for (Op* op : layers)
    if (op->op_type == OP_LINEAR && static_cast<Linear*>(op)->dx_map) api->ffh_free(ctx, static_cast<Linear*>(op)->dx_map);
  api->ffh_event_destroy(ctx, ev_fork); api->ffh_event_destroy(ctx, ev_join);
  api->ffh_event_destroy(ctx, ev_grad_ready); api->ffh_event_destroy(ctx, ev_update_done);
  api->ffh_event_destroy(ctx, ev_dw_done);
  api->ffh_event_destroy(ctx, ev_z_free);
  if (ev_fold_w) api->ffh_event_destroy(ctx, ev_fold_w);
  if (ev_fold_done) api->ffh_event_destroy(ctx, ev_fold_done);
  if (ev_fold_e_read) api->ffh_event_destroy(ctx, ev_fold_e_read);
  for (void* p : {(void*)fold.P, (void*)fold.S, (void*)fold.G, fold.sum_ws}) if (p) api->ffh_free(ctx, p);
  if (fold.sum_ctx) api->ffh_ctx_destroy(fold.sum_ctx);
  for (auto& kv : trace_tune) for (ffh_event& e : kv.second.ev) if (e) { api->ffh_event_destroy(ctx, e); e = nullptr; }
  for (ffh_event& e : probe_ev) if (e) { api->ffh_event_destroy(ctx, e); e = nullptr; }
  api->ffh_stream_destroy(ctx, stream); api->ffh_stream_destroy(ctx, side_stream); api->ffh_stream_destroy(ctx, dw_stream); api->ffh_stream_destroy(ctx, ar_stream);
  for (GradBucket& b : grad_buckets) { api->ffh_event_destroy(ctx, b.ready); api->ffh_event_destroy(ctx, b.ready_dw); api->ffh_event_destroy(ctx, b.done); }
  api->ffh_ctx_destroy(ctx);
  for (Op* op : layers) delete op;
  for (Initializer* i : owned_initializers) delete i;
  for (Tensor* t : input_tensors) delete t;
}

void FFModel::check(int rc, const char* what) const {
  if (rc != FFH_OK) die("%s failed (%d): %s", what, rc, api->ffh_last_error_string(ctx));
}

void* FFModel::dmalloc(size_t bytes) const {
  void* p = nullptr;
  int rc = api->ffh_malloc(ctx, &p, bytes);
  if (rc != FFH_OK || !p) die("device allocation of %zu bytes failed: %s", bytes, api->ffh_last_error_string(ctx));
  return p;
}

template <int NDIM>
Tensor FFModel::create_tensor(const int dims[], DataType data_type, const Op* owner_op, bool create_grad) {
  (void)create_grad;
  Tensor t;
  t.numDim = NDIM;
  t.data_type = data_type;
  t.owner_op = const_cast<Op*>(owner_op);
  for (int i = 0; i < NDIM; i++) t.adim[i] = dims[NDIM - 1 - i];
  t.impl = new TensorImpl();
  tensor_impls.push_back(t.impl);
  t.impl->guid = (int)tensor_impls.size() - 1;
  t.impl->is_input = owner_op == nullptr;
  if (owner_op == nullptr) {
    Tensor* keep = new Tensor(t);
    input_tensors.push_back(keep);
  }
  return t;
}
template Tensor FFModel::create_tensor<1>(const int[], DataType, const Op*, bool);
template Tensor FFModel::create_tensor<2>(const int[], DataType, const Op*, bool);
template Tensor FFModel::create_tensor<3>(const int[], DataType, const Op*, bool);
template Tensor FFModel::create_tensor<4>(const int[], DataType, const Op*, bool);

template <int NDIM>
Parameter FFModel::create_weight(const int dims[], const Op* op, DataType data_type, Initializer* initializer, bool) {
  Parameter p;
  p.numDim = NDIM;
  p.data_type = data_type;
  p.owner_op = const_cast<Op*>(op);
  p.sync_type = world_size > 1 ? NCCL : PS;
  for (int i = 0; i < NDIM; i++) p.adim[i] = dims[NDIM - 1 - i];
  p.impl = new TensorImpl();
  tensor_impls.push_back(p.impl);
  p.impl->guid = (int)tensor_impls.size() - 1;
  (void)initializer;
  return p;
}
template Parameter FFModel::create_weight<1>(const int[], const Op*, DataType, Initializer*, bool);
template Parameter FFModel::create_weight<2>(const int[], const Op*, DataType, Initializer*, bool);

Tensor FFModel::dense(const Tensor& input, int outDim, ActiMode activation, bool use_bias, const Op* shared_op,
                      Initializer* kernel_initializer, Initializer* bias_initializer, const char* name) {
  if (kernel_initializer == nullptr) kernel_initializer = new GlorotUniform(next_seed());
  if (bias_initializer == nullptr) bias_initializer = new ZeroInitializer();
  Linear* li = new Linear(*this, input, outDim, activation, use_bias, shared_op, kernel_initializer, bias_initializer, name);
  li->layer_index = (int)layers.size();
  layers.push_back(li);
  return li->outputs[0];
}

Tensor FFModel::embedding(const Tensor& input, int num_entries, int outDim, AggrMode aggr, const Op* shared_op,
                          Initializer* kernel_initializer, const char* name) {
  if (kernel_initializer == nullptr) kernel_initializer = new GlorotUniform(next_seed());
  Embedding* e = new Embedding(*this, input, num_entries, outDim, aggr, shared_op, kernel_initializer, name);
  e->layer_index = (int)layers.size();
  layers.push_back(e);
  return e->outputs[0];
}

Tensor FFModel::concat(int n, const Tensor* tensors, int axis, const char* name) {
// ... 24 lines not shown
  outputs[0].adim[0] = out_dim;
  numWeights = use_bias ? 2 : 1;
}
void Linear::create_output_and_partition(FFModel&) {}
void Linear::create_weights(FFModel& model) {
  const int kdims[2] = {out_channels, in_channels};
  weights[0] = model.create_weight<2>(kdims, this, DT_FLOAT, kernel_initializer);
  if (use_bias) {
    const int bdims[1] = {out_channels};
    weights[1] = model.create_weight<1>(bdims, this, DT_FLOAT, bias_initializer);
  }
}
void Linear::forward(const FFModel& ff) {
  const Tensor& x = inputs[0];
  const Tensor& y = outputs[0];
  const int64_t b = local_rows(y, &ff);
  if (fwd_done_by_pair) { fwd_done_by_pair = false; return; }
  if (fwd_done_by_chain) { fwd_done_by_chain = false; return; }
  if (!chain_fwd.empty() && ff.mlp_chain_usable(b, true)) {
    const int rc = ff.run_chain_fwd(this);
    if (rc == FFH_OK) { for (size_t i = 1; i < chain_fwd.size(); i++) chain_fwd[i]->fwd_done_by_chain = true; return; }
    if (rc != FFH_ERR_UNSUPPORTED) ff.check(rc, name);
    chain_fwd.clear();
  }
  if (pair_upper) {
    Linear* up = pair_upper;
    const Tensor& yu = up->outputs[0];
    const int rc = ff.api->ffh_linear_pair_fwd(ff.ctx, (const float*)x.impl->ptr, x.impl->ld, (const float*)weights[0].impl->ptr,
                                               use_bias ? (const float*)weights[1].impl->ptr : nullptr, in_channels, (int)activation, (float*)y.impl->ptr,
                                               y.impl->ld, out_channels, (const float*)up->weights[0].impl->ptr,
                                               up->use_bias ? (const float*)up->weights[1].impl->ptr : nullptr, up->out_channels, (int)up->activation,
                                               (float*)yu.impl->ptr, yu.impl->ld, b, ff.stream);
    if (rc == FFH_OK) { up->fwd_done_by_pair = true; return; }
    if (rc != FFH_ERR_UNSUPPORTED) ff.check(rc, name);
    pair_upper = nullptr;
  }
  if (ff.fold.layer == this) { ff.fold_linear_forward(this); return; }
  ff.check(ff.api->ffh_linear_fwd(ff.ctx, (const float*)x.impl->ptr, x.impl->ld, (float*)y.impl->ptr, y.impl->ld,
                                  (const float*)weights[0].impl->ptr, use_bias ? (const float*)weights[1].impl->ptr : nullptr,
                                  in_padded, out_channels, b, (int)activation, ff.stream), name);
  if (out_twin && out_twin_x3) ff.check(ff.api->ffh_convert_f32_to_bf16x3(ff.ctx, (const float*)y.impl->ptr, b, out_channels, y.impl->ld, ff.stream), name);
  else if (out_twin) ff.check(ff.api->ffh_convert_f32_to_bf16(ff.ctx, out_twin, (const float*)y.impl->ptr, b * (int64_t)y.impl->ld, ff.stream), name);
}
int Linear::backward_pair(const FFModel& ff) {
  Linear* lo = pair_lower;
  const Tensor &xu = inputs[0], &yu = outputs[0], &xl = lo->inputs[0];
  const int64_t b = local_rows(yu, &ff);
  const int flags_u = dy_premasked ? FFH_LINEAR_DY_PREMASKED : 0;
  const int flags_l = (lo->dx_overwrite ? FFH_LINEAR_DX_OVERWRITE : 0) | (lo->dx_mask_by_x ? FFH_LINEAR_DX_MASK_BY_X : 0);
  const int rc = ff.api->ffh_linear_pair_bwd(
      ff.ctx, (const float*)xu.impl->ptr, xu.impl->ld, (const float*)yu.impl->ptr, yu.impl->ld, yu.impl->grad, yu.impl->grad_ld,
      (const float*)weights[0].impl->ptr, weights[0].impl->grad, (use_bias && !db_from_upper) ? weights[1].impl->grad : nullptr, in_channels, out_channels,
      (int)activation, flags_u, (const float*)xl.impl->ptr, xl.impl->ld, xl.impl->grad, xl.impl->grad_ld, xu.impl->grad, xu.impl->grad_ld,
      (const float*)lo->weights[0].impl->ptr, lo->in_channels, (int)lo->activation, flags_l, b, ff.stream);
  if (rc != FFH_OK) return rc;
  db_from_upper = false;
  ff.check(ff.api->ffh_linear_bwd_ex(ff.ctx, (const float*)xl.impl->ptr, xl.impl->ld, nullptr, xl.impl->grad_ld, (const float*)xu.impl->ptr, xu.impl->ld,
                                     xu.impl->grad, xu.impl->grad_ld, (const float*)lo->weights[0].impl->ptr, lo->weights[0].impl->grad,
                                     lo->use_bias ? lo->weights[1].impl->grad : nullptr, lo->in_channels, lo->out_channels, b, (int)lo->activation,
                                     FFH_LINEAR_ONLY_DW | FFH_LINEAR_DY_PREMASKED, ff.stream, nullptr), lo->name);
  return FFH_OK;
}
void Linear::backward(const FFModel& ff) { backward_part(ff, 0); }

void Linear::backward_part(const FFModel& ff, int part) {
  if (activation == AC_MODE_GELU) die("%s: GELU has no backward (forward / inference only, as in the reference)", name);
  const Tensor& x = inputs[0];
  const Tensor& y = outputs[0];
  const int64_t b = local_rows(y, &ff);
  float* dx = discard_input_grad ? nullptr : x.impl->grad;
  const double macs = (double)in_channels * out_channels * (double)b;
  const bool fork = ff.config.parallel_dw && macs >= 1.0e8;
  const int flags = (dx_overwrite ? FFH_LINEAR_DX_OVERWRITE : 0) | (dx_mask_by_x ? FFH_LINEAR_DX_MASK_BY_X : 0) | (dy_premasked ? FFH_LINEAR_DY_PREMASKED : 0);
  const float *xp = (const float*)x.impl->ptr, *yp = (const float*)y.impl->ptr, *wp = (const float*)weights[0].impl->ptr;
  float *dyp = y.impl->grad, *dwp = weights[0].impl->grad, *dbp = (use_bias && !db_from_upper) ? weights[1].impl->grad : nullptr;
  const int64_t ldx = x.impl->ld, lddx = x.impl->grad_ld, ldy = y.impl->ld, lddy = y.impl->grad_ld;
  if (part != 1) db_from_upper = false;
  struct ColsumScope {
    const FFModel& ff; Linear* lo;
    ColsumScope(const FFModel& f, Linear* l, bool produces_dx) : ff(f), lo(produces_dx ? l : nullptr) {
      if (lo) ff.check(ff.api->ffh_linear_bwd_set_dx_colsum(ff.ctx, lo->weights[1].impl->grad, lo->out_channels), "dx colsum");
    }
    ~ColsumScope() { if (lo) lo->db_from_upper = ff.api->ffh_linear_dx_colsum_used(ff.ctx) != 0; }
  } colsum_scope(ff, colsum_lower, dx != nullptr && (part == 0 || part == 1) && !ff.use_workers() && !ff.config.profiling);
  auto image_dx = [&] {
    if (dx_image && dx) ff.check(ff.api->ffh_convert_f32_to_bf16x3(ff.ctx, dx, b, in_channels, lddx, ff.stream), name);
    if (bwd_exact && dx && dx_twin) ff.check(ff.api->ffh_convert_f32_to_bf16(ff.ctx, dx_twin, dx, b * (int64_t)in_channels, ff.stream), name);
  };
  struct ExactScope {
    const FFModel& ff; bool on;
    ExactScope(const FFModel& f, bool o) : ff(f), on(o) { if (on) ff.check(ff.api->ffh_ctx_set_math_mode(ff.ctx, FFH_MATH_DEFAULT), "math mode"); }
    ~ExactScope() { if (on) ff.check(ff.api->ffh_ctx_set_math_mode(ff.ctx, FFH_MATH_TENSOR_OP_BF16), "math mode"); }
  } exact_scope(ff, bwd_exact && !ff.use_workers());
  if (part == 1) {
    ff.check(ff.api->ffh_linear_bwd_ex(ff.ctx, xp, ldx, dx, lddx, yp, ldy, dyp, lddy, wp, dwp, dbp, in_padded, out_channels, b, (int)activation,
                                       flags | FFH_LINEAR_ONLY_DX, ff.stream, nullptr), name);
    image_dx();
    return;
  }
  if (fork && ff.use_workers()) {
    const KernelApi* api = ff.api;
    ffh_stream dws = ff.dw_stream;
    ffh_event ev = ff.layer_events[layer_index];
    const int in = in_padded, out = out_channels, act = (int)activation;
    const char* nm = name;
    auto dw_call = [=](ffh_ctx* wc) {
      int rc = api->ffh_stream_wait_event(wc, dws, ev);
      if (rc == FFH_OK) rc = api->ffh_linear_bwd_ex(wc, xp, ldx, nullptr, lddx, yp, ldy, dyp, lddy, wp, dwp, dbp, in, out, b, act, flags | FFH_LINEAR_ONLY_DW, dws, nullptr);
      if (rc != FFH_OK) die("%s (weight gradient) failed (%d): %s", nm, rc, api->ffh_last_error_string(wc));
    };
    const bool sig = activation == AC_MODE_SIGMOID;
    if (!sig) { ff.check(api->ffh_event_record(ff.ctx, ev, ff.stream), "event"); ff.dw_worker->post(dw_call); }
    ff.check(api->ffh_linear_bwd_ex(ff.ctx, xp, ldx, dx, lddx, yp, ldy, dyp, lddy, wp, dwp, dbp, in, out, b, act, flags | FFH_LINEAR_ONLY_DX, ff.stream, nullptr), name);
    if (sig) { ff.check(api->ffh_event_record(ff.ctx, ev, ff.stream), "event"); ff.dw_worker->post(dw_call); }
    ff.dw_forked = true;
    return;
  }
  ffh_stream dws = ff.dw_stream;
  if (part == 0 && ff.fold.layer == this && !ff.fold.dw_tables.empty()) {
    if (fork) {
      ffh_event ev = ff.layer_events[layer_index];
      ff.check(ff.api->ffh_event_record(ff.ctx, ev, ff.stream), "event");
      ff.check(ff.api->ffh_stream_wait_event(ff.ctx, dws, ev), "event");
    }
    if (dx) {
      ff.check(ff.api->ffh_linear_bwd_ex(ff.ctx, xp, ldx, dx, lddx, yp, ldy, dyp, lddy, wp, dwp, dbp, in_padded, out_channels, b, (int)activation,
                                         flags | FFH_LINEAR_ONLY_DX, ff.stream, nullptr), name);
      image_dx();
    }
    ff.fold_weight_gradient(this, dbp, fork ? dws : ff.stream);
    if (fork) { ff.dw_forked = true; ff.dw1_used = true; ff.dw_stream_used_directly = true; }
    return;
  }
  ff.check(ff.api->ffh_linear_bwd_ex(ff.ctx, xp, ldx, dx, lddx, yp, ldy, dyp, lddy, wp, dwp, dbp, in_padded, out_channels, b, (int)activation,
                                     flags, ff.stream, fork ? dws : nullptr), name);
  image_dx();
  if (fork) { ff.dw_forked = true; ff.dw1_used = true; }
}

void Linear::backward_dw_rows(const FFModel& ff, int row0, int nrows) {
  const Tensor& x = inputs[0];
  const Tensor& y = outputs[0];
  const int64_t b = local_rows(y, &ff);
  const float *xp = (const float*)x.impl->ptr, *yp = (const float*)y.impl->ptr + row0;
  float *dyp = y.impl->grad + row0, *dwp = weights[0].impl->grad + (size_t)row0 * (size_t)weights[0].impl->ld;
  const float* wp = (const float*)weights[0].impl->ptr + (size_t)row0 * (size_t)weights[0].impl->ld;
  float* dbp = (use_bias && !db_from_upper) ? weights[1].impl->grad + row0 : nullptr;
  const int flags = FFH_LINEAR_ONLY_DW | FFH_LINEAR_DY_PREMASKED;
  ff.check(ff.api->ffh_linear_bwd_ex(ff.ctx, xp, x.impl->ld, nullptr, x.impl->grad_ld, yp, y.impl->ld, dyp, y.impl->grad_ld, wp, dwp, dbp, in_padded, nrows, b,
                                     (int)activation, flags, ff.dw_stream, nullptr), name);
  ff.dw_forked = true;
  ff.dw1_used = true;
  ff.dw_stream_used_directly = true;
}

bool FFModel::mlp_chain_usable(int64_t rows, bool fwd) const {
  return config.mlp_chain && !config.profiling && !use_workers() && !config.allow_tensor_op_math_conversion && rows <= config.mlp_chain_max_batch && (!fwd || (rows >= config.mlp_chain_fwd_min_batch && rows <= config.mlp_chain_fwd_max_batch));
}
static void fill_chain(const std::vector<Linear*>& ch, ffh_chain_layer* out) {
  for (size_t i = 0; i < ch.size(); i++) {
    const Linear* li = ch[i];
    ffh_chain_layer& d = out[i];
    d.w = (const float*)li->weights[0].impl->ptr;
    d.bias = li->use_bias ? (const float*)li->weights[1].impl->ptr : nullptr;
    d.y = (float*)li->outputs[0].impl->ptr; d.ldy = li->outputs[0].impl->ld;
    d.dy = li->outputs[0].impl->grad; d.lddy = li->outputs[0].impl->grad_ld;
    d.dw = li->weights[0].impl->grad;
    d.db = (li->use_bias && !li->db_from_upper) ? li->weights[1].impl->grad : nullptr;
    d.ldw = (int)li->weights[0].impl->ld; d.in_dim = li->in_padded; d.out_dim = li->out_channels; d.activation = (int)li->activation;
  }
}
int FFModel::run_chain_fwd(const Linear* lowest) const {
  const std::vector<Linear*>& ch = lowest->chain_fwd;
  ffh_chain_layer ls[FFH_CHAIN_MAX_LAYERS];
  fill_chain(ch, ls);
  const Tensor& x = lowest->inputs[0];
  const int rc = api->ffh_mlp_chain_fwd(ctx, (const float*)x.impl->ptr, x.impl->ld, ls, (int)ch.size(), local_rows(lowest->outputs[0], this), stream);
  if (rc == FFH_OK) n_chain_fwd_calls++;
  return rc;
}
int FFModel::run_chain_bwd(Linear* top) {
  const std::vector<Linear*>& ch = top->chain_bwd;
  ffh_chain_layer ls[FFH_CHAIN_MAX_LAYERS];
  fill_chain(ch, ls);
  Linear* lo = ch.front();
  const Tensor& x = lo->inputs[0];
  const int flags = (top->dy_premasked ? FFH_LINEAR_DY_PREMASKED : 0) | (lo->dx_overwrite ? FFH_LINEAR_DX_OVERWRITE : 0) |
                    (lo->dx_mask_by_x ? FFH_LINEAR_DX_MASK_BY_X : 0);
  const int rc = api->ffh_mlp_chain_bwd(ctx, (const float*)x.impl->ptr, x.impl->ld, lo->discard_input_grad ? nullptr : x.impl->grad, x.impl->grad_ld, ls,
                                        (int)ch.size(), local_rows(top->outputs[0], this), flags, stream);
  if (rc == FFH_OK) { n_chain_bwd_calls++; for (Linear* li : ch) li->db_from_upper = false; }
  return rc;
}

Embedding::Embedding(FFModel& model, const Tensor& input, int _num_entries, int outDim, AggrMode _aggr, const Op* shared_op,
                     Initializer* ki, const char* name)
    : Op(model, OP_EMBEDDING, name, 1, &input), num_entries(_num_entries), out_channels(outDim), aggr(_aggr),
      kernel_initializer(ki) {
  if (shared_op) die("%s: weight sharing is not supported on this path", this->name);
  if (input.data_type != DT_INT64) die("%s: input must be DT_INT64", this->name);
  if (input.numDim != 2) die("%s: input must be [batch][bag]", this->name);
  if (input.owner_op != nullptr) die("%s: input must be a model input tensor", this->name);
  if (aggr != AGGR_MODE_SUM && aggr != AGGR_MODE_AVG) die("%s: aggr must be SUM or AVG", this->name);
  outputs[0].numDim = 2;
  outputs[0].adim[0] = outDim;
  outputs[0].adim[1] = input.adim[1];
  numWeights = 1;
  table_index = (int)model.embeddings.size();
// ... 491 lines not shown
```

### dlrm_flexflow_amd/host/model_allocate.cc

```cpp
#include "model_internal.h"

int FFModel::tables_of_rank(int r) const {
  int n = 0;
  for (const Embedding* e : embeddings) n += e->owner_rank == r;
  return n;
}

int FFModel::next_seed() {
  return (int)(ffh_hash(config.seed * 0x9E3779B97F4A7C15ULL + 0x5EED, seed_counter++) & 0x7fffffffULL);
}

bool FFModel::fused_embedding_update() const {
  if (config.dense_embedding_update) return false;
  const SGDOptimizer* sgd = dynamic_cast<const SGDOptimizer*>(optimizer);
  if (sgd && sgd->momentum == 0.0 && sgd->weight_decay == 0.0) return true;
  const AdagradOptimizer* adagrad = dynamic_cast<const AdagradOptimizer*>(optimizer);
  if (adagrad && adagrad->weight_decay == 0.0) return true;
  return config.sparse_embedding_optimizer && (sgd || adagrad || dynamic_cast<const AdamOptimizer*>(optimizer));
}

bool FFModel::sparse_rule(ffh_sparse_opt& o) const {
  memset(&o, 0, sizeof o);
  if (const SGDOptimizer* sgd = dynamic_cast<const SGDOptimizer*>(optimizer)) {
    o.lr = (float)sgd->lr;
// ... 875 lines not shown
    const int out = li->out_channels;
    r.P = (float*)dmalloc((size_t)prows * out * 4);
    r.S = (float*)dmalloc((size_t)local_batch * out * 4);
    const int plan = api->fold->ffh_fold_linear_fwd_plan(ctx, (const float*)x.impl->ptr, x.impl->ld, (const float*)li->outputs[0].impl->ptr, li->outputs[0].impl->ld,
                                                         (const float*)li->weights[0].impl->ptr, li->use_bias ? (const float*)li->weights[1].impl->ptr : nullptr,
                                                         li->in_padded, out, local_rows(li->outputs[0], this), r.keep.data(), (int)r.keep.size(), r.S, out);
    if (plan < 1) { api->ffh_free(ctx, r.P); api->ffh_free(ctx, r.S); continue; }
    int64_t prow = 0, col = 0;
    size_t k = 0;
    for (int i = 0; i < c->numInputs; i++) {
      const Tensor& in = c->inputs[i];
      if (k < r.tables.size() && in.owner_op == r.tables[k]) {
        Embedding* e = r.tables[k++];
        float* p = r.P + (size_t)prow * out;
        r.groups.push_back(ffh_fold_group{(const float*)e->weights[0].impl->ptr, (int64_t)e->out_channels, col, p, (int64_t)e->num_entries});
        ffh_emb_table t;
        t.idx = (const int64_t*)e->inputs[0].impl->ptr;
        t.weight = p;
        t.num_entries = e->num_entries;
        t.io = nullptr;
        t.ld = out;
        r.gather.push_back(t);
        prow += e->num_entries;
      }
      col += in.adim[0];
    }
    r.layer = li;
    plan_fold_dw(r);
    fold = r;
    if (!ev_fold_w) check((config.timing_events ? api->ffh_event_create : api->ffh_event_create_sync)(ctx, &ev_fold_w), "event create");
    if (!ev_fold_done) check((config.timing_events ? api->ffh_event_create : api->ffh_event_create_sync)(ctx, &ev_fold_done), "event create");
    return;
  }
}

void FFModel::plan_fold_dw(FoldRoute& r) {
  Linear* li = r.layer;
  if (!config.fold_dw || config.deterministic || config.profiling || dw_worker || side_worker) return;
  if (!(li->dy_premasked || li->activation == AC_MODE_NONE) || li->pair_lower || li->bwd_exact || li->dx_image || li->dx_map) return;
  const int64_t rows = local_rows(li->outputs[0], this);
  if (!li->chain_bwd.empty() && mlp_chain_usable(rows, false)) return;
  if (li->in_padded % FFH_FOLD_DW_NTILE || li->weights[0].impl->ld != li->in_padded) return;
  const int out = li->out_channels, ntile = li->in_padded / FFH_FOLD_DW_NTILE;
  std::vector<char> folded(ntile, 0);
  std::vector<size_t> pick;
  int64_t grows = 0;
  for (size_t k = 0; k < r.tables.size(); k++) {
    const int64_t col0 = r.groups[k].col0, d = r.tables[k]->out_channels;
    if (col0 % FFH_FOLD_DW_NTILE || d % FFH_FOLD_DW_NTILE) continue;
    for (int64_t t = col0 / FFH_FOLD_DW_NTILE; t < (col0 + d) / FFH_FOLD_DW_NTILE; t++) folded[t] = 1;
    pick.push_back(k);
    grows += r.tables[k]->num_entries;
  }
  if (pick.empty()) return;
  for (int t = 0; t < ntile; t++) if (!folded[t]) r.dw_kept.push_back(t);
  const Tensor &x = li->inputs[0], &y = li->outputs[0];
  const int plan = r.dw_kept.empty() ? 0 : api->fold->ffh_fold_linear_bwd_dw_plan(ctx, (const float*)x.impl->ptr, x.impl->ld, y.impl->grad, y.impl->grad_ld, li->weights[0].impl->grad,
                                                                                  li->use_bias ? li->weights[1].impl->grad : nullptr, li->in_padded, out, rows,
                                                                                  r.dw_kept.data(), (int)r.dw_kept.size());
  if (plan != 1) { r.dw_kept.clear(); return; }
  const Embedding* e0 = r.tables[pick[0]];
  const int L = (int)e0->inputs[0].adim[0];
  r.G = (float*)dmalloc((size_t)grows * out * 4);
  const size_t ws_bytes = api->ffh_embedding_bwd_workspace_bytes((int)pick.size(), L, out, local_batch) + 256;
  r.sum_ws = dmalloc(ws_bytes);
  if (api->ffh_ctx_create(&r.sum_ctx, config.device) != FFH_OK || !r.sum_ctx) die("fold: ffh_ctx_create(device %d) failed", config.device);
  check(api->ffh_ctx_set_workspace(r.sum_ctx, r.sum_ws, ws_bytes), "set workspace");
  int64_t grow = 0;
  for (size_t k : pick) {
    Embedding* e = r.tables[k];
    float* g = r.G + (size_t)grow * out;
    r.dw_tables.push_back(e);
    r.dw_groups.push_back(ffh_fold_group{(const float*)e->weights[0].impl->ptr, (int64_t)e->out_channels, r.groups[k].col0, g, (int64_t)e->num_entries});
    ffh_emb_table t;
    t.idx = (const int64_t*)e->inputs[0].impl->ptr;
    t.weight = g;
    t.num_entries = e->num_entries;
    t.io = y.impl->grad;
    t.ld = y.impl->grad_ld;
    r.dw_sum.push_back(t);
    grow += e->num_entries;
  }
  if (!ev_fold_e_read) check((config.timing_events ? api->ffh_event_create : api->ffh_event_create_sync)(ctx, &ev_fold_e_read), "event create");
}

void FFModel::init_layers() {
  if (!compiled) die("init_layers() before compile()");
  for (Op* op : layers) op->init(*this);
}

void FFModel::print_layers(int id) {
  if (id == -1) for (Op* op : layers) op->print_layer(*this);
  else layers.at(id)->print_layer(*this);
}
```

### dlrm_flexflow_amd/host/model_exchange.cc

```cpp
#include "model_internal.h"

void launch_shard_groups(const FFModel* ff, ShardLaunch what, ffh_stream s, ffh_ctx* cx, const std::vector<const int64_t*>* idx_override) {
  const bool fwd = what == kGather;
  ffh_sparse_opt rule;
  const bool ruled = (what == kFusedUpdate || what == kApplyOnly) && ff->sparse_rule(rule);
  const ffh_lr_state* lrb = ff->lr_route == FFModel::kLrDevice ? ff->lr_block[1] : nullptr;
  const KernelApiLr* lra = ff->api->lr;
  const int L = ff->embeddings[0]->inputs[0].adim[0];
  const int aggr = (int)ff->embeddings[0]->aggr;
  struct Group { std::vector<ffh_emb_table> t; std::vector<ffh_emb_table_bf16> t16; std::vector<ffh_emb_state> st; };
  std::map<std::pair<int, bool>, Group> groups;
  size_t owned_i = 0;
  for (const FFModel::EmbShard& sh : ff->shards) {
    if (sh.owner != ff->rank) continue;
    const Embedding* e = sh.e;
    ffh_emb_table t;
    t.idx = (const int64_t*)e->inputs[0].impl->ptr;
    if (idx_override && owned_i < idx_override->size()) t.idx = (*idx_override)[owned_i];
    owned_i++;
    t.weight = (float*)e->weights[0].impl->ptr;
    t.num_entries = e->num_entries;
    if (!ff->exchange) {
      t.io = fwd ? (float*)e->outputs[0].impl->ptr : e->outputs[0].impl->grad;
      t.ld = fwd ? e->outputs[0].impl->ld : e->outputs[0].impl->grad_ld;
    } else {
      t.io = (fwd ? ff->xsend : ff->grecv) + sh.off;
      t.ld = ff->rank_width[ff->rank];
    }
    Group& g = groups[{sh.cols, e->bf16_weights()}];
    if (e->bf16_weights()) g.t16.push_back(ffh_emb_table_bf16{t.idx, (uint16_t*)t.weight, t.io, t.num_entries, t.ld, e->table_index, sh.col0});
    else g.t.push_back(t);
    g.st.push_back(ffh_emb_state{e->opt_state[0], e->opt_state[1]});
  }
  const int64_t B = ff->config.batchSize;
  for (auto& kv : groups) {
    const int D = kv.first.first;
    const Group& g = kv.second;
    if (kv.first.second) {
      const KernelApiBf16* b16 = ff->api->bf16;
      const ffh_bf16_rounding rnd = ff->bf16_rounding();
      const size_t per = ff->bf16_tables_per_launch();
      for (size_t b = 0; b < g.t16.size(); b += per) {
        const int n = (int)std::min<size_t>(per, g.t16.size() - b);
        const ffh_emb_table_bf16* tb = g.t16.data() + b;
        const ffh_emb_state* st = g.st.data() + b;
        switch (what) {
          case kGather: ff->check(b16->ffh_embedding_fwd_multi_bf16(cx, tb, n, L, D, B, aggr, s), "embedding_fwd_multi_bf16"); break;
          case kFusedUpdate:
            if (lrb) ff->check(lra->ffh_embedding_bwd_opt_fused_multi_bf16_lr(cx, tb, st, n, L, D, B, aggr, &rule, &rnd, lrb, s), "embedding_bwd_opt_fused_multi_bf16_lr");
            else if (ruled) ff->check(b16->ffh_embedding_bwd_opt_fused_multi_bf16(cx, tb, st, n, L, D, B, aggr, &rule, &rnd, s), "embedding_bwd_opt_fused_multi_bf16");
            else ff->check(b16->ffh_embedding_bwd_sgd_fused_multi_bf16(cx, tb, n, L, D, B, aggr, rule.lr, &rnd, s), "embedding_bwd_sgd_fused_multi_bf16");
            break;
          case kSortOnly: ff->check(b16->ffh_embedding_bwd_sort_multi_bf16(cx, tb, n, L, D, B, s), "embedding_bwd_sort_multi_bf16"); ff->n_early_sorts++; break;
          case kApplyOnly:
            if (lrb) ff->check(lra->ffh_embedding_bwd_opt_apply_multi_bf16_lr(cx, tb, st, n, L, D, B, aggr, &rule, &rnd, lrb, s), "embedding_bwd_opt_apply_multi_bf16_lr");
            else if (ruled) ff->check(b16->ffh_embedding_bwd_opt_apply_multi_bf16(cx, tb, st, n, L, D, B, aggr, &rule, &rnd, s), "embedding_bwd_opt_apply_multi_bf16");
            else ff->check(b16->ffh_embedding_bwd_sgd_apply_multi_bf16(cx, tb, n, L, D, B, aggr, rule.lr, &rnd, s), "embedding_bwd_sgd_apply_multi_bf16");
            break;
        }
      }
      continue;
    }
    const std::vector<ffh_emb_table>& tabs = g.t;
    const std::vector<ffh_emb_state>& sts = g.st;
    for (size_t b = 0; b < tabs.size(); b += FFH_MAX_TABLES) {
      const int n = (int)std::min<size_t>(FFH_MAX_TABLES, tabs.size() - b);
      switch (what) {
        case kGather: ff->check(ff->api->ffh_embedding_fwd_multi(cx, tabs.data() + b, n, L, D, B, aggr, s), "embedding_fwd_multi"); break;
        case kFusedUpdate:
          if (lrb) ff->check(lra->ffh_embedding_bwd_opt_fused_multi_lr(cx, tabs.data() + b, sts.data() + b, n, L, D, B, aggr, &rule, lrb, s), "embedding_bwd_opt_fused_multi_lr");
          else if (ruled) ff->check(ff->api->ffh_embedding_bwd_opt_fused_multi(cx, tabs.data() + b, sts.data() + b, n, L, D, B, aggr, &rule, s), "embedding_bwd_opt_fused_multi");
          else ff->check(ff->api->ffh_embedding_bwd_sgd_fused_multi(cx, tabs.data() + b, n, L, D, B, aggr, rule.lr, s), "embedding_bwd_sgd_fused_multi");
          break;
        case kSortOnly: ff->check(ff->api->ffh_embedding_bwd_sort_multi(cx, tabs.data() + b, n, L, D, B, s), "embedding_bwd_sort_multi"); ff->n_early_sorts++; break;
        case kApplyOnly:
          if (lrb) ff->check(lra->ffh_embedding_bwd_opt_apply_multi_lr(cx, tabs.data() + b, sts.data() + b, n, L, D, B, aggr, &rule, lrb, s), "embedding_bwd_opt_apply_multi_lr");
          else if (ruled) ff->check(ff->api->ffh_embedding_bwd_opt_apply_multi(cx, tabs.data() + b, sts.data() + b, n, L, D, B, aggr, &rule, s), "embedding_bwd_opt_apply_multi");
          else ff->check(ff->api->ffh_embedding_bwd_sgd_apply_multi(cx, tabs.data() + b, n, L, D, B, aggr, rule.lr, s), "embedding_bwd_sgd_apply_multi");
          break;
      }
    }
  }
}

static constexpr uint64_t kBf16SeedSalt = 0xBF16;
ffh_bf16_rounding FFModel::bf16_rounding() const {
  ffh_bf16_rounding r;
  r.mode = config.embedding_rounding;
  r.reserved_ = 0;
  r.seed = ffh_hash(config.seed, kBf16SeedSalt);
  r.counter = bf16_counter;
  return r;
}
void FFModel::advance_bf16_counter(ffh_stream s, ffh_ctx* cx) const {
  if (bf16_counter) check(api->bf16->ffh_bf16_counter_advance(cx, bf16_counter, s), "bf16_counter_advance");
}
size_t FFModel::bf16_tables_per_launch() const {
  ffh_sparse_opt rule;
  bool any16 = false;
  for (const Embedding* e : embeddings) any16 = any16 || e->bf16_weights();
  return any16 && fused_embedding_update() && sparse_rule(rule) && rule.kind != FFH_SPARSE_OPT_ADAGRAD && rule.kind != FFH_SPARSE_OPT_ROWWISE_ADAGRAD ? FFH_BF16_MAX_STATEFUL_TABLES : FFH_MAX_TABLES;
}
uint64_t FFModel::read_bf16_counter() const {
  if (!bf16_counter) return 0;
  if (dw_worker) dw_worker->drain();
  if (side_worker) side_worker->drain();
  check(api->ffh_stream_sync(ctx, side_stream), "bf16 counter sync");
  check(api->ffh_stream_sync(ctx, stream), "bf16 counter sync");
  uint64_t v = 0;
  check(api->ffh_memcpy_d2h(ctx, &v, bf16_counter, sizeof v, stream), "bf16 counter");
  check(api->ffh_stream_sync(ctx, stream), "bf16 counter sync");
  return v;
}

void FFModel::embedding_kernels_only(bool fwd, ffh_stream s, const std::vector<const int64_t*>* idx_override) const {
  if (embeddings.empty() || (!fwd && !fused_embedding_update())) return;
  launch_shard_groups(this, fwd ? kGather : kFusedUpdate, s, ctx, idx_override);
  if (!fwd) advance_bf16_counter(s, ctx);
}

bool FFModel::early_sort_possible(int where) const {
  if (!config.early_sort || !config.overlap_embedding || !fused_embedding_update() || config.profiling) return false;
  if (config.computationMode != COMP_MODE_TRAINING || use_workers() || evaluating) return false;
  const bool exact_gemms = !config.allow_tensor_op_math_conversion && !config.fp32_split_bf16x3;
  const int mode = config.early_sort > 0 ? config.early_sort : ((!exchange && local_batch >= 8192 && exact_gemms) ? early_sort_big_batch_mode : 1);
  if (mode != where) return false;
  int n = 0, cols = -1;
  for (const EmbShard& sh : shards) {
    if (sh.owner != rank) continue;
    if (cols >= 0 && sh.cols != cols) return false;
    cols = sh.cols;
    n++;
  }
  for (const Embedding* e : embeddings)
    if (e->row_sharded) return false;
  return n > 0 && (size_t)n <= bf16_tables_per_launch();
}

void FFModel::probe_record(int which, ffh_stream s, ffh_ctx* cx) const {
  if (!probe_events_on) return;
  if (!probe_ev[which]) check(api->ffh_event_create(ctx, &probe_ev[which]), "probe event");
  check(api->ffh_event_record(cx, probe_ev[which], s), "probe event");
}

void FFModel::embedding_group_forward(ffh_stream s, ffh_ctx* on_ctx) const {
  if (embeddings.empty()) return;
  launch_shard_groups(this, kGather, s, on_ctx ? on_ctx : ctx);
  ffh_ctx* cx = on_ctx ? on_ctx : ctx;
  if (exchange) {
    probe_record(4, s, cx);
    if (!shards.empty() && config.comm.alltoall_f32(config.comm.user, xsend, fwd_send_counts.data(), xrecv, fwd_recv_counts.data(), s) != 0)
      die("alltoall (embedding forward) failed");
    probe_record(5, s, cx);
  }
  {
    std::vector<ffh_emb_table> tabs;
    const int Lr = embeddings[0]->inputs[0].adim[0];
    for (const Embedding* e : embeddings) {
      if (!e->replicated) continue;
      ffh_emb_table t;
      t.idx = (const int64_t*)e->inputs[0].impl->ptr + (int64_t)rank * local_batch * Lr;
      t.weight = (float*)e->weights[0].impl->ptr;
      t.num_entries = e->num_entries;
      t.io = (float*)e->outputs[0].impl->ptr;
      t.ld = e->outputs[0].impl->ld;
      tabs.push_back(t);
    }
    for (size_t b = 0; b < tabs.size(); b += FFH_MAX_TABLES) {
      const int n = (int)std::min<size_t>(FFH_MAX_TABLES, tabs.size() - b);
      check(api->ffh_embedding_fwd_multi(cx, tabs.data() + b, n, Lr, embeddings[0]->out_channels, local_batch, (int)embeddings[0]->aggr, s),
            "embedding_fwd_multi (data-parallel tables)");
    }
  }
  for (const Embedding* e : embeddings) {
    if (!e->row_sharded) continue;
    const int L = e->inputs[0].adim[0], D = e->out_channels;
    check(api->ffh_embedding_localize_rows(cx, (const int64_t*)e->inputs[0].impl->ptr, e->local_idx, (int64_t)config.batchSize * L,
                                           e->row_begin, e->rows_local, s), "embedding_localize_rows");
    check(api->ffh_embedding_fwd(cx, e->local_idx, e->partial, (const float*)e->weights[0].impl->ptr, L, D, config.batchSize,
                                 e->rows_local + 1, D, (int)e->aggr, s), e->name);
    if (config.comm.reduce_scatter_sum_f32(config.comm.user, e->partial, (float*)e->outputs[0].impl->ptr, local_batch * D, s) != 0)
      die("reduce-scatter (row-sharded embedding forward) failed");
  }
}

void FFModel::replicated_embedding_grads() const {
  if (!repl_workspace) return;
  std::vector<ffh_emb_table> tabs;
  const int L = embeddings[0]->inputs[0].adim[0], D = embeddings[0]->out_channels;
  for (const Embedding* e : embeddings) {
    if (!e->replicated) continue;
    ffh_emb_table t;
    t.idx = (const int64_t*)e->inputs[0].impl->ptr + (int64_t)rank * local_batch * L;
    t.weight = e->weights[0].impl->grad;
    t.num_entries = e->num_entries;
    t.io = e->outputs[0].impl->grad;
    t.ld = e->outputs[0].impl->grad_ld;
    tabs.push_back(t);
  }
  check(api->ffh_ctx_set_workspace(ctx, repl_workspace, repl_workspace_bytes), "set workspace");
// ... 138 lines not shown
```

### dlrm_flexflow_amd/host/model_flags.cc

```cpp
#include "model_internal.h"

FFConfig::FFConfig() {
  epochs = 1;
  batchSize = 64;
  printFreq = 10;
  numNodes = 1;
  cpusPerNode = 0;
  workersPerNode = 0;
  learningRate = 0.01f;
  weightDecay = 0.0001f;
  workSpaceSize = (size_t)1 << 30;
  syntheticInput = false;
  profiling = false;
  perform_fusion = false;
  computationMode = COMP_MODE_TRAINING;
  device = 0;
  seed = 0;
  enable_graph = true;
  overlap_embedding = true;
  dense_embedding_update = false;
  force_exchange = false;
  parallel_dw = true;
  async_launch = false;
  column_shard_rows = 0;
  row_shard_rows = 0;
  replicate_embedding_rows = 0;
  fuse_loss = true;
  driver_loss = LOSS_MEAN_SQUARED_ERROR_AVG_REDUCE;
  eval_batches = 0;
  eval_only = false;
  synthetic_labels = 0;
  data_randomize = 0;
  timing_events = false;
  attach_events = true;
  fuse_pair = true;
  mlp_chain = true;
  fold_small_tables = true;
  fold_max_rows = 7420;
  fold_dw = true;
  trace_mode = -1;
  bucket_allreduce = -1;
  allreduce_bucket_floats = 1 << 20;
  direct_allreduce = false;
  big_dw_chunks = 0;
  big_dw_min_weights = 2 << 20;
  mlp_chain_max_batch = 8192;
  mlp_chain_fwd_max_batch = 4096;
  mlp_chain_fwd_min_batch = 4096;
  mlp_chain_max_weights = 200000;
  dx_scatter = true;
  dx_colsum = true;
  early_sort = -1;
  pad_linear_k = true;
  capture_exchange = false;
  bf16_twins = true;
  bf16_convert_twins = true;
  bf16_exact_small_backward = true;
  force_async_launch = false;
  sparse_embedding_optimizer = false;
  allow_tensor_op_math_conversion = false;
  fp32_split_bf16x3 = false;
  deterministic = false;
  embedding_dtype = DT_FLOAT;
  embedding_rounding = FFH_BF16_ROUND_STOCHASTIC;
  lr_warmup_steps = lr_decay_start_step = lr_num_decay_steps = 0;
  device_lr = false;
  host_lr_schedule = false;
  checkpoint_every_epochs = 0;
  adagrad_eps = 1e-10;
  adagrad_initial_accumulator = 0.0;
  adagrad_rowwise = false;
  memset(&comm, 0, sizeof comm);
  comm.rank = 0;
  comm.world_size = 1;
}

void FFConfig::parse_args(char** argv, int argc) {
  for (int i = 1; i < argc; i++) {
    const char* eq = strncmp(argv[i], "--", 2) == 0 ? strchr(argv[i], '=') : nullptr;
    auto is = [&](const char* a) { return eq ? (strlen(a) == (size_t)(eq - argv[i]) && !strncmp(argv[i], a, (size_t)(eq - argv[i]))) : !strcmp(argv[i], a); };
    auto next = [&]() -> const char* {
      if (eq) return eq + 1;
      if (i + 1 >= argc) die("flag %s needs a value", argv[i]);
      return argv[++i];
    };
    if (is("-e") || is("--epochs")) { epochs = atoi(next()); continue; }
    if (is("-b") || is("--batch-size")) { batchSize = atoi(next()); continue; }
    if (is("--lr") || is("--learning-rate")) { learningRate = (float)atof(next()); continue; }
    if (is("--wd") || is("--weight-decay")) { weightDecay = (float)atof(next()); continue; }
    if (is("-p") || is("--print-freq")) { printFreq = atoi(next()); continue; }
    if (is("-d") || is("--dataset")) { dataset_path = next(); continue; }
    if (is("--import") || is("--import-strategy")) { import_strategy_file = next(); continue; }
    if (is("--export") || is("--export-strategy")) { export_strategy_file = next(); continue; }
    if (is("-ll:gpu")) { workersPerNode = atoi(next()); continue; }
    if (is("--nodes")) { numNodes = atoi(next()); continue; }
    if (is("-ll:cpu")) { cpusPerNode = atoi(next()); continue; }
    if (is("--profiling")) { profiling = true; continue; }
    if (is("--fusion")) { perform_fusion = true; continue; }
    if (is("-ll:fsize") || is("-ll:zsize") || is("-ll:util") || is("-ll:csize") || is("--budget") || is("--search-budget") ||
        is("--alpha") || is("--search-alpha") || is("--simulator-workspace-size") || is("--strategy") ||
        is("--machine-model-version") || is("--machine-model-file") || is("--simulator-segment-size") ||
        is("--simulator-max-num-segments") || is("--taskgraph")) { next(); continue; }
    if (is("--allow-tensor-op-math-conversion")) { allow_tensor_op_math_conversion = true; continue; }
    if (is("--fp32-split-bf16x3")) { fp32_split_bf16x3 = true; continue; }
    if (is("-dm:memoize") || is("-dm:memorize") || is("--overlap") || is("--enable-parameter-parallel") ||
        is("--enable-attribute-parallel") || is("--enable-propagation")) continue;
    if (is("--seed")) { seed = strtoull(next(), nullptr, 10); continue; }
    if (is("--deterministic")) { deterministic = true; continue; }
    if (is("--backend")) { backend_lib = next(); continue; }
    if (is("--device")) { device = atoi(next()); continue; }
    if (is("--no-trace")) { enable_graph = false; continue; }
    if (is("--no-overlap")) { overlap_embedding = false; continue; }
    if (is("--dense-embedding-update")) { dense_embedding_update = true; continue; }
    if (is("--force-exchange")) { force_exchange = true; continue; }
    if (is("--serial-dw")) { parallel_dw = false; continue; }
    if (is("--inline-launch")) { async_launch = false; continue; }
    if (is("--async-launch")) { async_launch = true; continue; }
    if (is("--column-shard-rows")) { column_shard_rows = atoll(next()); continue; }
    if (is("--row-shard-rows")) { row_shard_rows = atoll(next()); continue; }
    if (is("--replicate-embedding-rows")) { replicate_embedding_rows = atoll(next()); continue; }
    if (is("--no-fused-loss")) { fuse_loss = false; continue; }
    if (is("--loss")) {
      const char* v = next();
      if (!strcmp(v, "mse")) driver_loss = LOSS_MEAN_SQUARED_ERROR_AVG_REDUCE;
      else if (!strcmp(v, "bce")) driver_loss = LOSS_BINARY_CROSSENTROPY;
      else die("--loss %s: 'mse' or 'bce'", v);
      continue;
    }
    if (is("--eval-batches")) { eval_batches = atoi(next()); if (eval_batches < 0) die("--eval-batches %d: must be >= 0", eval_batches); continue; }
    if (is("--eval-only")) { eval_only = true; continue; }
    if (is("--synthetic-labels")) {
      const char* v = next();
      if (!strcmp(v, "bernoulli")) synthetic_labels = 0;
      else if (!strcmp(v, "logistic")) synthetic_labels = 1;
      else die("--synthetic-labels %s: 'bernoulli' or 'logistic'", v);
      continue;
    }
    if (is("--data-randomize")) {
      const char* v = next();
      if (!strcmp(v, "none")) data_randomize = 0;
      else if (!strcmp(v, "total")) data_randomize = 1;
      else die("--data-randomize %s: 'none' or 'total'", v);
      continue;
    }
    if (is("--timing-events")) { timing_events = true; continue; }
    if (is("--no-attach-event")) { attach_events = false; continue; }
    if (is("--no-fused-pair")) { fuse_pair = false; continue; }
    if (is("--no-mlp-chain")) { mlp_chain = false; continue; }
    if (is("--no-fold-small-tables")) { fold_small_tables = false; continue; }
    if (is("--no-fold-dw")) { fold_dw = false; continue; }
    if (is("--fold-max-rows")) { fold_max_rows = atoll(next()); continue; }
    if (is("--always-replay")) { trace_mode = 1; continue; }
    if (is("--adaptive-replay")) { trace_mode = 0; continue; }
    if (is("--bucket-allreduce")) { bucket_allreduce = 1; continue; }
    if (is("--no-bucket-allreduce")) { bucket_allreduce = 0; continue; }
    if (is("--allreduce-bucket-floats")) { allreduce_bucket_floats = atoll(next()); continue; }
    if (is("--direct-allreduce")) { direct_allreduce = true; continue; }
    if (is("--big-dw-chunks")) { big_dw_chunks = atoi(next()); continue; }
    if (is("--big-dw-min-weights")) { big_dw_min_weights = atoll(next()); continue; }
    if (is("--mlp-chain-max-batch")) { mlp_chain_max_batch = atoll(next()); continue; }
    if (is("--mlp-chain-fwd-min-batch")) { mlp_chain_fwd_min_batch = atoll(next()); continue; }
    if (is("--mlp-chain-fwd-max-batch")) { mlp_chain_fwd_max_batch = atoll(next()); continue; }
    if (is("--mlp-chain-max-weights")) { mlp_chain_max_weights = atoll(next()); continue; }
    if (is("--no-dx-scatter")) { dx_scatter = false; continue; }
    if (is("--no-dx-colsum")) { dx_colsum = false; continue; }
    if (is("--no-early-sort")) { early_sort = 0; continue; }
    if (is("--early-sort")) { early_sort = 1; continue; }
    if (is("--no-pad-linear-k")) { pad_linear_k = false; continue; }
    if (is("--capture-exchange")) { capture_exchange = true; continue; }
    if (is("--no-bf16-exact-small-backward")) { bf16_exact_small_backward = false; continue; }
    if (is("--no-bf16-convert-twins")) { bf16_convert_twins = false; continue; }
    if (is("--no-bf16-twins")) { bf16_twins = false; continue; }
    if (is("--force-async-launch")) { force_async_launch = true; continue; }
    if (is("--sparse-embedding-optimizer")) { sparse_embedding_optimizer = true; continue; }
    if (is("--embedding-dtype")) {
      const char* v = next();
      if (!strcmp(v, "fp32")) embedding_dtype = DT_FLOAT;
      else if (!strcmp(v, "bf16")) embedding_dtype = DT_BF16;
      else die("--embedding-dtype %s: 'fp32' or 'bf16'", v);
      continue;
    }
    if (is("--lr-num-warmup-steps")) { lr_warmup_steps = atoll(next()); continue; }
    if (is("--lr-decay-start-step")) { lr_decay_start_step = atoll(next()); continue; }
    if (is("--lr-num-decay-steps")) { lr_num_decay_steps = atoll(next()); continue; }
    if (is("--save-checkpoint")) { save_checkpoint_dir = next(); if (save_checkpoint_dir.empty()) die("--save-checkpoint: needs a directory"); continue; }
    if (is("--load-checkpoint")) { load_checkpoint_dir = next(); if (load_checkpoint_dir.empty()) die("--load-checkpoint: needs a directory"); continue; }
    if (is("--checkpoint-every-epochs")) {
      checkpoint_every_epochs = atoi(next());
      if (checkpoint_every_epochs < 1) die("--checkpoint-every-epochs %d: must be >= 1", checkpoint_every_epochs);
      continue;
    }
    if (is("--adagrad-eps")) { adagrad_eps = atof(next()); continue; }
    if (is("--adagrad-initial-accumulator")) { adagrad_initial_accumulator = atof(next()); continue; }
    if (is("--adagrad-rowwise")) { adagrad_rowwise = eq ? atoi(eq + 1) != 0 : true; continue; }
    if (is("--device-lr")) { device_lr = true; continue; }
    if (is("--host-lr-schedule")) { host_lr_schedule = true; continue; }
    if (is("--embedding-rounding")) {
      const char* v = next();
      if (!strcmp(v, "stochastic")) embedding_rounding = FFH_BF16_ROUND_STOCHASTIC;
      else if (!strcmp(v, "nearest")) embedding_rounding = FFH_BF16_ROUND_NEAREST;
      else die("--embedding-rounding %s: 'stochastic' or 'nearest'", v);
      continue;
    }
  }
}
```

### dlrm_flexflow_amd/host/model_internal.h

```cpp
#pragma once
#include "ffmodel.h"


#include <algorithm>
#include <set>
#include <cassert>
#include <chrono>
#include <cmath>
#include <cstdarg>
#include <cstdio>
#include <cstdlib>
#include <cstring>
#include <functional>
#include <type_traits>

#include "../../include/ffh_rng.h"
#include "../../include/ffh_bf16.h"
#include "backend.h"

[[noreturn]] inline void die(const char* fmt, ...) {
  va_list ap;
  va_start(ap, fmt);
  fprintf(stderr, "FATAL: ");
  vfprintf(stderr, fmt, ap);
  fprintf(stderr, "\n");
  va_end(ap);
  abort();
}

inline double now_us() {
  return std::chrono::duration<double, std::micro>(std::chrono::steady_clock::now().time_since_epoch()).count();
}

inline size_t dtype_size(DataType t) {
  switch (t) {
    case DT_FLOAT: return 4;
    case DT_DOUBLE: return 8;
    case DT_INT32: return 4;
    case DT_INT64: return 8;
    case DT_BOOLEAN: return 1;
    case DT_BF16: return 2;
    default: return 0;
  }
}

constexpr size_t kBf16Chunk = (size_t)1 << 22;

inline size_t align_up(size_t x, size_t a = 256) { return (x + a - 1) / a * a; }

inline int64_t local_rows(const Tensor& t, const FFModel*) { return t.impl ? t.impl->rows_local : 0; }

inline bool in_dense_slab(const Parameter& p) {
  if (p.owner_op->op_type == OP_LINEAR) return true;
  return p.owner_op->op_type == OP_EMBEDDING && static_cast<const Embedding*>(p.owner_op)->replicated;
}

enum ShardLaunch { kGather, kFusedUpdate, kSortOnly, kApplyOnly };
void launch_shard_groups(const FFModel* ff, ShardLaunch what, ffh_stream s, ffh_ctx* cx, const std::vector<const int64_t*>* idx_override = nullptr);
```

### dlrm_flexflow_amd/host/model_step.cc

```cpp
#include "model_internal.h"

void FFModel::reset_metrics() {
  if (replaying_trace >= 0) return;
  check(api->ffh_zero(ctx, d_perf, sizeof(ffh_perf_metrics), stream), "reset_metrics");
  if (d_bce_sum) check(api->ffh_zero(ctx, d_bce_sum, sizeof(float), stream), "reset_metrics");
}

void FFModel::refresh_weight_twin() const {
  if (!w_twin || !w_twin_dirty) return;
  if (config.fp32_split_bf16x3 && !config.allow_tensor_op_math_conversion) check(api->ffh_convert_f32_to_bf16x3(ctx, mlp_weights, 1, (int64_t)mlp_count, (int64_t)mlp_count, stream), "weight image");
  else check(api->ffh_convert_f32_to_bf16(ctx, w_twin, mlp_weights, (int64_t)mlp_count, stream), "weight twin");
  w_twin_dirty = false;
}
int64_t FFModel::weight_mirror_stale_bytes() {
  if (!w_twin) return -1;
  if (w_twin_dirty) return -2;
  sync();
  const bool x3 = config.fp32_split_bf16x3 && !config.allow_tensor_op_math_conversion;
  const size_t bytes = x3 ? FFH_BF16X3_IMAGE_BYTES((size_t)mlp_count * 4) : (size_t)mlp_count * 2;
  std::vector<char> kept(bytes), fresh(bytes);
  check(api->ffh_memcpy_d2h(ctx, kept.data(), w_twin, bytes, stream), "weight mirror d2h");
  w_twin_dirty = true;
  refresh_weight_twin();
  check(api->ffh_memcpy_d2h(ctx, fresh.data(), w_twin, bytes, stream), "weight mirror d2h");
// ... 28 lines not shown
    profiled(op, true, [&] { op->forward(*this); });
  }
  if (emb_forward_issued && !emb_forward_joined) join_embedding_forward();
}

void FFModel::profiled(const Op* op, bool fwd, const std::function<void()>& fn) const {
  ffh_event e0, e1;
  check(api->ffh_event_create(ctx, &e0), "event");
  check(api->ffh_event_create(ctx, &e1), "event");
  check(api->ffh_event_record(ctx, e0, stream), "event");
  fn();
  check(api->ffh_event_record(ctx, e1, stream), "event");
  check(api->ffh_event_sync(ctx, e1), "event");
  float ms = 0.0f;
  check(api->ffh_event_elapsed_ms(ctx, e0, e1, &ms), "event");
  api->ffh_event_destroy(ctx, e0);
  api->ffh_event_destroy(ctx, e1);
  const char* dir = fwd ? "forward" : "backward";
  switch (op->op_type) {
    case OP_LINEAR:
      if (fwd) printf("%s [Linear] forward time = %.2lfms\n", op->name, (double)ms);
      else printf("Linear backward time = %.2lfms\n", (double)ms);
      break;
    case OP_BATCHMATMUL: printf("BatchMatmul %s time = %.2lfms\n", dir, (double)ms); break;
    case OP_EMBEDDING:
      printf("[Embedding x%zu] %s time = %.4f ms\n", embeddings.size(), dir, ms);
      break;
    default: printf("[%s] %s time = %.4f ms\n", op->name, dir, ms); break;
  }
}

void FFModel::issue_embedding_forward_on_side_stream() const {
  if (use_workers()) {
    const FFModel* self = this;
    side_worker->post([self](ffh_ctx* wc) {
      self->check(self->api->ffh_stream_wait_event(wc, self->side_stream, self->ev_fork), "fork");
      self->embedding_group_forward(self->side_stream, wc);
      self->check(self->api->ffh_event_record(wc, self->ev_join, self->side_stream), "join");
    });
  } else {
    if (fork_recorded) check(api->ffh_stream_wait_event(ctx, side_stream, ev_fork), "fork");
    probe_record(0, side_stream, ctx);
    embedding_group_forward(side_stream);
    probe_record(1, side_stream, ctx);
    check(api->ffh_event_record(ctx, ev_join, side_stream), "join");
    if (fold.layer && fold_w_recorded) {
      check(api->ffh_stream_wait_event(ctx, side_stream, ev_fold_w), "fold: weights ready");
      fold_products_and_sum(side_stream, ctx);
      check(api->ffh_event_record(ctx, ev_fold_done, side_stream), "fold: sum ready");
      fold_on_side = true;
    }
    if (early_sort_possible(1)) {
      launch_shard_groups(this, kSortOnly, side_stream, ctx);
      emb_sorted_early = true;
    }
  }
  emb_forward_issued = true;
  emb_forward_joined = false;
}

void FFModel::fold_products_and_sum(ffh_stream s, ffh_ctx* cx) const {
  const Linear* li = fold.layer;
  const Embedding* e0 = fold.tables[0];
  check(api->fold->ffh_fold_product(cx, fold.groups.data(), (int)fold.groups.size(), (const float*)li->weights[0].impl->ptr, li->in_padded, e0->out_channels,
                                    li->out_channels, s), "fold_product");
  check(api->fold->ffh_fold_gather_add(cx, fold.gather.data(), (int)fold.gather.size(), e0->inputs[0].adim[0], li->out_channels, local_batch, FFH_AGGR_MODE_SUM,
                                       fold.S, li->out_channels, s), "fold_gather_add");
}

void FFModel::fold_weight_gradient(const Linear* li, float* dbp, ffh_stream dws) const {
  const Tensor &x = li->inputs[0], &y = li->outputs[0];
  const Embedding* e0 = fold.dw_tables[0];
  const int64_t b = local_rows(y, this);
  const int out = li->out_channels, ng = (int)fold.dw_groups.size();
  if (api->fold->ffh_fold_segment_sum(fold.sum_ctx, fold.dw_sum.data(), ng, e0->inputs[0].adim[0], out, b, dws) != FFH_OK)
    die("%s: fold_segment_sum failed: %s", li->name, api->ffh_last_error_string(fold.sum_ctx));
  check(api->fold->ffh_fold_dw_product(ctx, fold.dw_groups.data(), ng, li->weights[0].impl->grad, li->in_padded, e0->out_channels, out, dws), "fold_dw_product");
  check(api->ffh_event_record(ctx, ev_fold_e_read, dws), "fold: table rows read");
  fold_e_read_recorded = true;
  check(api->fold->ffh_fold_linear_bwd_dw(ctx, (const float*)x.impl->ptr, x.impl->ld, y.impl->grad, y.impl->grad_ld, li->weights[0].impl->grad, dbp, li->in_padded, out, b,
                                          fold.dw_kept.data(), (int)fold.dw_kept.size(), dws), li->name);
}

void FFModel::fold_linear_forward(const Linear* li) const {
  if (fold_on_side) check(api->ffh_stream_wait_event(ctx, stream, ev_fold_done), "fold: sum ready");
  else fold_products_and_sum(stream, ctx);
  const Tensor& x = li->inputs[0];
  const Tensor& y = li->outputs[0];
  check(api->fold->ffh_fold_linear_fwd(ctx, (const float*)x.impl->ptr, x.impl->ld, (float*)y.impl->ptr, y.impl->ld, (const float*)li->weights[0].impl->ptr,
                                       li->use_bias ? (const float*)li->weights[1].impl->ptr : nullptr, li->in_padded, li->out_channels, local_rows(y, this),
                                       (int)li->activation, fold.keep.data(), (int)fold.keep.size(), fold.S, li->out_channels, stream), li->name);
}

void FFModel::join_embedding_forward() const {
  if (side_worker) side_worker->drain();
  probe_record(10, stream, ctx);
  check(api->ffh_stream_wait_event(ctx, stream, ev_join), "join");
  probe_record(11, stream, ctx);
  emb_forward_joined = true;
}

void FFModel::issue_embedding_update_on_side_stream() const {
  if (use_workers()) {
    const FFModel* self = this;
    side_worker->post([self](ffh_ctx* wc) {
      self->check(self->api->ffh_stream_wait_event(wc, self->side_stream, self->ev_grad_ready), "event");
      self->embedding_group_update(self->side_stream, wc);
      self->check(self->api->ffh_event_record(wc, self->ev_update_done, self->side_stream), "event");
    });
  } else {
    check(api->ffh_stream_wait_event(ctx, side_stream, ev_grad_ready), "event");
    if (fold_e_read_recorded) check(api->ffh_stream_wait_event(ctx, side_stream, ev_fold_e_read), "fold: table rows read");
    probe_record(2, side_stream, ctx);
    embedding_group_update(side_stream);
    probe_record(3, side_stream, ctx);
    check(api->ffh_event_record(ctx, ev_update_done, side_stream), "event");
  }
}

void FFModel::order_input_writes_behind_update() const {
  if (embeddings.empty() || !config.overlap_embedding || !fused_embedding_update()) return;
  if (side_worker) side_worker->drain();
  check(api->ffh_stream_wait_event(ctx, stream, ev_update_done), "inputs behind the table update");
}

void FFModel::zero_gradients() {
  if (replaying_trace >= 0) return;
  if (need_zero_act_grads) check(api->ffh_zero(ctx, act_grad_slab, act_grad_bytes, stream), "zero_gradients");
  if (!mlp_grads_clean) check(api->ffh_zero(ctx, mlp_grads, mlp_count * 4, stream), "zero_gradients");
  if (exchange && gsend && need_zero_gsend) {
    size_t n = 0;
    for (int64_t c : fwd_recv_counts) n += (size_t)c;
    check(api->ffh_zero(ctx, gsend, n * 4, stream), "zero_gradients");
  }
  if (!fused_embedding_update())
    for (Embedding* e : embeddings)
      if (e->held_here(rank) && !e->replicated)
        check(api->ffh_zero(ctx, e->weights[0].impl->grad, e->weights[0].impl->bytes + (e->row_sharded ? (size_t)e->out_channels * 4 : 0), stream), "zero_gradients");
}

void FFModel::compute_metrics() {
  if (replaying_trace >= 0) return;
  const Tensor& fin = layers.back()->outputs[0];
  check(api->ffh_metrics_update(ctx, (const float*)fin.impl->ptr, (const float*)label_tensor.impl->ptr, d_perf,
                                local_rows(fin, this), fin.adim[0], metrics_flags, stream), "compute_metrics");
}

void FFModel::backward(int _seq_length) {
  if (replaying_trace >= 0) return;
  seq_length = _seq_length;
  if (config.computationMode != COMP_MODE_TRAINING) die("backward() in inference mode");
  const Tensor& fin = layers.back()->outputs[0];
  const bool bce = loss_type == LOSS_BINARY_CROSSENTROPY;
  const float scale = (bce || loss_type == LOSS_MEAN_SQUARED_ERROR_AVG_REDUCE) ? 1.0f / (float)fin.adim[fin.numDim - 1] : 1.0f;
  if (fin.impl->grad_ld != fin.adim[0] || fin.impl->ld != fin.adim[0]) die("final layer output must be contiguous");
  dw_forked = false;
  fold_e_read_recorded = false;
  opt_next_done = false;
  int first = (int)layers.size() - 1;
  emb_update_pending = false;
  mlp_grads_clean = false;
  Linear* last = (config.fuse_loss && !config.profiling) ? dynamic_cast<Linear*>(layers.back()) : nullptr;
  int rc = FFH_ERR_UNSUPPORTED;
  if (last) {
    const Tensor& x = last->inputs[0];
    const int flags = (last->dx_overwrite ? FFH_LINEAR_DX_OVERWRITE : 0) | (last->dx_mask_by_x ? FFH_LINEAR_DX_MASK_BY_X : 0);
    if (bce)
      rc = api->ctr->ffh_linear_bwd_bce(ctx, (const float*)x.impl->ptr, x.impl->ld, last->discard_input_grad ? nullptr : x.impl->grad, x.impl->grad_ld,
                                        (const float*)fin.impl->ptr, fin.impl->ld, fin.impl->grad, fin.impl->grad_ld,
                                        (const float*)last->weights[0].impl->ptr, last->weights[0].impl->grad,
                                        last->use_bias ? last->weights[1].impl->grad : nullptr, last->in_channels, last->out_channels,
                                        local_rows(fin, this), (int)last->activation, flags, (const float*)label_tensor.impl->ptr, scale, d_perf,
                                        d_bce_sum, metrics_flags, stream);
    else
    rc = api->ffh_linear_bwd_mse(ctx, (const float*)x.impl->ptr, x.impl->ld, last->discard_input_grad ? nullptr : x.impl->grad, x.impl->grad_ld,
                                 (const float*)fin.impl->ptr, fin.impl->ld, fin.impl->grad, fin.impl->grad_ld,
                                 (const float*)last->weights[0].impl->ptr, last->weights[0].impl->grad,
                                 last->use_bias ? last->weights[1].impl->grad : nullptr, last->in_channels, last->out_channels,
                                 local_rows(fin, this), (int)last->activation, flags, (const float*)label_tensor.impl->ptr, scale, d_perf,
                                 metrics_flags, stream);
    if (rc == FFH_OK) n_fused_loss_calls++;
    if (rc == FFH_OK) first--;
    else if (rc != FFH_ERR_UNSUPPORTED) check(rc, "loss + last layer backward");
  }
  if (rc != FFH_OK && bce)
    check(api->ctr->ffh_bce_bwd_metrics(ctx, fin.impl->grad, (const float*)fin.impl->ptr, (const float*)label_tensor.impl->ptr, d_perf, d_bce_sum,
                                        local_rows(fin, this), fin.adim[0], scale, metrics_flags, stream), "metrics + loss backward (bce)");
  else if (rc != FFH_OK)
    check(api->ffh_mse_bwd_metrics(ctx, fin.impl->grad, (const float*)fin.impl->ptr, (const float*)label_tensor.impl->ptr, d_perf,
                                   local_rows(fin, this), fin.adim[0], scale, metrics_flags, stream), "metrics + loss backward");
  grad_ready_attached = false;
  z_free_recorded = false;
  auto mark_z_free = [&](int l) {
    if (l == z_reader_layer && dw_forked && !dw_worker && capturing_trace < 0) {
      check(api->ffh_event_record(ctx, ev_z_free, dw_stream), "z free");
      z_free_recorded = true;
    }
  };
  bwd_alltoall_issued = false;
  for (GradBucket& b : grad_buckets) b.issued = b.inline_issued = false;
  const int dw_chunks = big_dw_chunks_now();
  auto chunked_big_backward = [&](Linear* up, int l) {
    ffh_event ev = layer_events[l];
    check(api->ffh_event_record(ctx, ev, stream), "event");
    check(api->ffh_stream_wait_event(ctx, dw_stream, ev), "event");
    up->backward_part(*this, 1);
    const int per = up->out_channels / dw_chunks;
    for (size_t k = 0; k < grad_buckets.size(); k++) {
      GradBucket& b = grad_buckets[k];
      if (b.chunk_layer != l) continue;
      up->backward_dw_rows(*this, b.chunk_index * per, per);
      if (!buckets_held()) issue_one_bucket(k, false);
    }
    up->db_from_upper = false;
  };
  for (int l = first; l >= 0; l--) {
    if (bucketed_now()) issue_grad_buckets(l);
    if (l == grad_attach_layer) {
      check(api->ffh_event_record_with_next_linear_bwd(ctx, ev_grad_ready), "attach event");
      grad_ready_attached = true;
    }
    Linear* up = layers[l]->op_type == OP_LINEAR ? static_cast<Linear*>(layers[l]) : nullptr;
    if (up && up->dx_map && !use_workers()) {
      const bool attach = l == scatter_attach_layer;
      check(api->ffh_linear_bwd_set_dx_scatter(ctx, up->dx_map, up->in_channels, attach ? ev_grad_ready : nullptr), "dx scatter");
      if (dw_chunks > 1 && l == big_dw_layer) { chunked_big_backward(up, l); mark_z_free(l); }
      else { up->backward(*this); mark_z_free(l); }
      if (api->ffh_linear_dx_scatter_used(ctx)) {
        up->dx_map_concat->bwd_done = true;
        if (attach) grad_ready_attached = true;
      }
      continue;
    }
    if (config.profiling) {
      if (layers[l]->op_type == OP_EMBEDDING && static_cast<Embedding*>(layers[l])->table_index != (int)embeddings.size() - 1) continue;
      profiled(layers[l], false, [&] {
        layers[l]->backward(*this);
        if (layers[l]->op_type == OP_EMBEDDING && fused_embedding_update()) embedding_group_update(stream);
      });
      continue;
    }
    if (up && !up->chain_bwd.empty() && mlp_chain_usable(local_rows(up->outputs[0], this), false)) {
      const int n = (int)up->chain_bwd.size();
      const int crc = run_chain_bwd(up);
      if (crc == FFH_OK) {
        if (grad_attach_layer > l - n && grad_attach_layer < l && !grad_ready_attached) {
          check(api->ffh_event_record(ctx, ev_grad_ready, stream), "event");
          grad_ready_attached = true;
        }
        for (int k = 0; k < n; k++) mark_z_free(l - k);
        l -= n - 1;
        continue;
      }
      if (crc != FFH_ERR_UNSUPPORTED) check(crc, up->name);
      up->chain_bwd.clear();
    }
    if (up && up->pair_lower && !use_workers() && l != grad_attach_layer && l >= 1 && layers[l - 1] == up->pair_lower) {
      const int prc = up->backward_pair(*this);
      if (prc == FFH_OK) { l--; continue; }
      if (prc != FFH_ERR_UNSUPPORTED) check(prc, up->name);
      up->pair_lower = nullptr;
    }
    if (up && dw_chunks > 1 && l == big_dw_layer) { chunked_big_backward(up, l); mark_z_free(l); continue; }
    layers[l]->backward(*this);
    mark_z_free(l);
  }
  if (emb_update_pending) {
    issue_embedding_update_on_side_stream();
    emb_update_pending = false;
  }
  if (bucketed_now()) { bwd_alltoall_issued = true; issue_grad_buckets(-1); }
}

void FFModel::update() {
  n_update_calls++;
  if (replaying_trace >= 0) return;
  optimizer->next();
  opt_next_done = true;
  SGDOptimizer* sgd = dynamic_cast<SGDOptimizer*>(optimizer);
  AdamOptimizer* adam = dynamic_cast<AdamOptimizer*>(optimizer);
  AdagradOptimizer* adagrad = dynamic_cast<AdagradOptimizer*>(optimizer);
  if (!sgd && !adam && !adagrad) die("update(): unknown optimizer");
  if (side_worker) side_worker->drain();
  if (dw_forked && !dw_worker && !api->ffh_second_stream_used(ctx, 1) && !dw_stream_used_directly) { dw_forked = false; dw1_used = false; }
  dw_stream_used_directly = false;
  if (dw_forked) {
    if (dw_worker) { dw_worker->drain(); dw1_used = true; }
    if (dw1_used) {
      check(api->ffh_event_record(ctx, ev_dw_done, dw_stream), "join dw");
      check(api->ffh_stream_wait_event(ctx, stream, ev_dw_done), "join dw");
    }
    if (config.overlap_embedding && !embeddings.empty() && !use_workers()) {
      if (z_free_recorded) check(api->ffh_stream_wait_event(ctx, side_stream, ev_z_free), "join dw (embedding stream)");
      else {
        if (dw1_used) check(api->ffh_stream_wait_event(ctx, side_stream, ev_dw_done), "join dw (embedding stream)");
      }
    }
    dw1_used = false;
    dw_forked = false;
  }
  if (exchange && mlp_count) {
    bool any_issued = false;
    for (const GradBucket& b : grad_buckets) any_issued = any_issued || b.issued;
    if (any_issued) {
      for (const GradBucket& b : grad_buckets) if (!b.issued) die("update(): a gradient bucket was not issued");
      probe_record(12, stream, ctx);
      for (const GradBucket& b : grad_buckets) if (!b.inline_issued) check(api->ffh_stream_wait_event(ctx, stream, b.done), "join all-reduce bucket");
      probe_record(13, stream, ctx);
      probe_record(8, stream, ctx);
      for (auto& r : grad_rest)
        if (allreduce_grads(mlp_grads + r.first, (int64_t)r.second, stream, false) != 0) die("allreduce failed");
      probe_record(9, stream, ctx);
    } else {
      probe_record(8, stream, ctx);
      if (allreduce_grads(mlp_grads, (int64_t)mlp_count, stream, false) != 0) die("allreduce failed");
      probe_record(9, stream, ctx);
    }
  }
  const size_t opt_count = mlp_count;
  const ffh_lr_state* lrb = lr_route == kLrDevice ? lr_block[0] : nullptr;
  if (adam) {
    if (mlp_count && lrb) {
      check(api->lr->ffh_adam_update_lr(ctx, mlp_weights, mlp_grads, adam->mlp_m, adam->mlp_v, (int64_t)opt_count, lrb, (float)adam->beta1,
                                        (float)adam->beta2, (float)adam->weight_decay, (float)adam->epsilon, FFH_OPT_ZERO_GRAD, stream),
            "adam_update_lr (MLP slab)");
      mlp_grads_clean = true;
    } else if (mlp_count) {
      check(api->ffh_adam_update(ctx, mlp_weights, mlp_grads, adam->mlp_m, adam->mlp_v, (int64_t)opt_count, (float)adam->alpha_t,
                                 (float)adam->beta1, (float)adam->beta2, (float)adam->weight_decay, (float)adam->epsilon,
                                 FFH_OPT_ZERO_GRAD, stream), "adam_update (MLP slab)");
      mlp_grads_clean = true;
    }
  } else if (adagrad) {
    if (mlp_count && lrb) {
      check(api->adagrad->ffh_adagrad_update_lr(ctx, mlp_weights, mlp_grads, adagrad->mlp_s, (int64_t)opt_count, lrb, (float)adagrad->epsilon,
                                                (float)adagrad->weight_decay, FFH_OPT_ZERO_GRAD, stream), "adagrad_update_lr (MLP slab)");
      mlp_grads_clean = true;
    } else if (mlp_count) {
      check(api->adagrad->ffh_adagrad_update(ctx, mlp_weights, mlp_grads, adagrad->mlp_s, (int64_t)opt_count, (float)adagrad->lr, (float)adagrad->epsilon,
                                             (float)adagrad->weight_decay, FFH_OPT_ZERO_GRAD, stream), "adagrad_update (MLP slab)");
      mlp_grads_clean = true;
    }
  } else if (sgd->momentum > 0.0) {
    for (const Parameter& p : parameters)
      if (in_dense_slab(p)) sgd->update(&p);
  } else if (mlp_count && lrb) {
    check(api->lr->ffh_sgd_update_ex_lr(ctx, mlp_weights, mlp_grads, nullptr, (int64_t)opt_count, lrb, (float)sgd->weight_decay, 0.0f, 0, FFH_OPT_ZERO_GRAD,
                                        stream), "sgd_update_ex_lr (MLP slab)");
    mlp_grads_clean = true;
  } else if (mlp_count) {
    check(api->ffh_sgd_update_ex(ctx, mlp_weights, mlp_grads, nullptr, (int64_t)opt_count, (float)sgd->lr, (float)sgd->weight_decay, 0.0f,
                                 0, FFH_OPT_ZERO_GRAD, stream), "sgd_update (MLP slab)");
    mlp_grads_clean = true;
  }
  if (fused_embedding_update()) {
    if (config.overlap_embedding) {
      if (!embeddings.empty() && (capturing_trace >= 0 || use_workers()))
        check(api->ffh_stream_wait_event(ctx, stream, ev_update_done), "join update");
    } else if (!config.profiling) {
      embedding_group_update(stream);
    }
  } else {
    embedding_dense_update();
  }
  advance_lr(0, stream, ctx);
  if (lr_route == kLrHost) lr_host_set(++lr_host_steps);
}

bool FFModel::trace_replays(int trace_id) const {
  if (!config.enable_graph) return false;
  auto it = trace_tune.find(trace_id);
  return !(trace_adaptive() && it != trace_tune.end() && it->second.decided == 2);
}

void FFModel::begin_trace(int trace_id) {
  if (!config.enable_graph) return;
  if (trace_adaptive()) {
    TraceTune& t = trace_tune[trace_id];
    if (t.decided == 2 || (t.decided == 0 && t.calls < 5)) return;
    if (t.decided == 0 && t.calls == 9) {
      check(api->ffh_event_sync(ctx, t.ev[3]), "trace timing");
      check(api->ffh_event_elapsed_ms(ctx, t.ev[0], t.ev[1], &t.eager_ms), "trace timing");
      check(api->ffh_event_elapsed_ms(ctx, t.ev[2], t.ev[3], &t.graph_ms), "trace timing");
      t.decided = t.graph_ms <= 1.02f * t.eager_ms ? 1 : 2;
      for (ffh_event& e : t.ev) { api->ffh_event_destroy(ctx, e); e = nullptr; }
      if (config.profiling || getenv("FFM_TRACE_VERBOSE"))
        fprintf(stderr, "[DLRM] trace %d: eager %.1f us / step, hipGraph replay %.1f us / step -> %s\n", trace_id, t.eager_ms * 500.f, t.graph_ms * 500.f,
                t.decided == 1 ? "replay" : "eager");
      if (t.decided == 2) return;
    }
  }
  refresh_weight_twin();
  auto it = graphs.find(trace_id);
  if (it != graphs.end()) { replaying_trace = trace_id; return; }
  if (dw_worker) dw_worker->drain();
  if (side_worker) side_worker->drain();
  int rc = api->ffh_graph_begin_capture(ctx, stream);
  if (rc == FFH_ERR_UNSUPPORTED) { config.enable_graph = false; return; }
  check(rc, "begin_trace");
  capturing_trace = trace_id;
}
// ... 236 lines not shown
```

### include/ff_hip_fold.h

```cpp
#ifndef FF_HIP_FOLD_H_
#define FF_HIP_FOLD_H_

#include "ff_hip.h"

#ifdef __cplusplus
extern "C" {
#endif

#define FFH_FOLD_ABI_VERSION 2

#define FFH_FOLD_KTILE      16
#define FFH_FOLD_NTILE      64
#define FFH_FOLD_MAX_GROUPS 64
#define FFH_FOLD_MAX_SEGS   32
#define FFH_FOLD_DW_NTILE   128
#define FFH_FOLD_DW_CHUNK   256

typedef struct ffh_fold_group {
  const float* e;
  int64_t      lde;
  int64_t      col0;
  float*       p;
  int64_t      rows;
} ffh_fold_group;

typedef struct ffh_fold_seg { int32_t k0, len; } ffh_fold_seg;

int ffh_fold_abi_version(void);

int ffh_fold_product(ffh_ctx* ctx, const ffh_fold_group* groups, int ngroups, const float* w, int64_t ldw, int d, int out_dim, ffh_stream s);

int ffh_fold_gather_add(ffh_ctx* ctx, const ffh_emb_table* tables, int ntables, int in_dim, int out_dim, int64_t batch, int aggr,
                        float* S, int64_t ldS, ffh_stream s);

int ffh_fold_linear_fwd(ffh_ctx* ctx, const float* x, int64_t ldx, float* y, int64_t ldy, const float* w, const float* bias,
                        int in_dim, int out_dim, int64_t batch, int activation, const ffh_fold_seg* keep, int nkeep,
                        const float* addend, int64_t ldadd, ffh_stream s);

int ffh_fold_linear_fwd_plan(ffh_ctx* ctx, const float* x, int64_t ldx, const float* y, int64_t ldy, const float* w, const float* bias,
                             int in_dim, int out_dim, int64_t batch, const ffh_fold_seg* keep, int nkeep, const float* addend, int64_t ldadd);


int ffh_fold_segment_sum(ffh_ctx* ctx, const ffh_emb_table* tables, int ntables, int in_dim, int width, int64_t batch, ffh_stream s);

int ffh_fold_dw_product(ffh_ctx* ctx, const ffh_fold_group* groups, int ngroups, float* dw, int64_t lddw, int d, int out_dim, ffh_stream s);

int ffh_fold_linear_bwd_dw(ffh_ctx* ctx, const float* x, int64_t ldx, const float* dy, int64_t lddy, float* dw, float* db, int in_dim, int out_dim,
                           int64_t batch, const int32_t* kept, int nkept, ffh_stream s);

int ffh_fold_linear_bwd_dw_plan(ffh_ctx* ctx, const float* x, int64_t ldx, const float* dy, int64_t lddy, const float* dw, const float* db, int in_dim,
                                int out_dim, int64_t batch, const int32_t* kept, int nkept);

#ifdef __cplusplus
}
#endif

#define FFH_FOLD_API_LIST(X) \
  X(ffh_fold_abi_version) X(ffh_fold_product) X(ffh_fold_gather_add) X(ffh_fold_linear_fwd) X(ffh_fold_linear_fwd_plan) \
  X(ffh_fold_segment_sum) X(ffh_fold_dw_product) X(ffh_fold_linear_bwd_dw) X(ffh_fold_linear_bwd_dw_plan)

#endif
```

Measured before the change: 4.836 million samples/s.

## Fold small-table data gradient: skip their dx columns and update tables via folded product

For embedding tables already folded into the first top-MLP layer, the backward data-gradient GEMM now computes only the kept column tiles, skipping the folded tables' input columns. Those tables are instead updated directly by a new MFMA kernel that multiplies the segment-summed output gradient by the layer weight slice and applies SGD in place. The per-sample embedding update for them is removed. This adds a cross-stream dependency so the weight update waits until the folded table update has read the weights, and it adds an ABI bump with backward-compatibility loading.

```diff
diff --git a/dlrm_flexflow_amd/capi.py b/dlrm_flexflow_amd/capi.py
--- a/dlrm_flexflow_amd/capi.py
+++ b/dlrm_flexflow_amd/capi.py
@@ -798,6 +798,10 @@
     "ffh_fold_dw_product": (I, [P, C.POINTER(FoldGroup), I, P, L, I, I, P]),
     "ffh_fold_linear_bwd_dw": (I, [P, P, L, P, L, P, P, I, I, L, C.POINTER(C.c_int32), I, P]),
     "ffh_fold_linear_bwd_dw_plan": (I, [P, P, L, P, L, P, P, I, I, L, C.POINTER(C.c_int32), I]),
+    "ffh_fold_linear_bwd_dx": (I, [P, P, L, P, L, P, L, P, I, I, L, I, C.POINTER(C.c_int32), I, P, P, P]),
+    "ffh_fold_linear_bwd_dx_plan": (I, [P, P, L, P, L, P, L, P, I, I, L, I, C.POINTER(C.c_int32), I, P]),
+    "ffh_fold_table_update": (I, [P, C.POINTER(FoldGroup), I, P, L, I, I, C.c_float, P]),
+    "ffh_fold_table_update_lr": (I, [P, C.POINTER(FoldGroup), I, P, L, I, I, P, P]),
 }
 
 
diff --git a/dlrm_flexflow_amd/csrc/fold.hip b/dlrm_flexflow_amd/csrc/fold.hip
--- a/dlrm_flexflow_amd/csrc/fold.hip
+++ b/dlrm_flexflow_amd/csrc/fold.hip
@@ -1,5 +1,6 @@
 #include "fold_sum.h"
 #include "linear_gemm.h"
+#include "lr_state.h"
 
 #include "../../include/ff_hip_fold.h"
 
@@ -191,7 +192,125 @@
   }
 }
 
+struct FoldUpdGroup { const float* g; float* e; int64_t lde; int64_t col0; int rows; int tile0; };
+struct FoldUpdArgs {
+  FoldUpdGroup grp[FFH_FOLD_MAX_GROUPS];
+  const float* w; int64_t ldw;
+  const float* lr_ptr; float lr;
+  int ngroups, out, d, ntiles;
+};
+static_assert(sizeof(FoldUpdArgs) <= 4096, "kernel arguments");
+
+__global__ __launch_bounds__(256) void fold_table_update_kernel(const FoldUpdArgs g) {
+  ffh_kernel_prio();
+  const int lane = threadIdx.x & 63;
+  const int wave = __builtin_amdgcn_readfirstlane((int)(threadIdx.x >> 6));
+  const int c = lane & 15, q = lane >> 4;
+  const int wt = (int)blockIdx.x * 4 + wave;
+  if (wt >= g.ntiles) return;
+  int gi = 0;
+  while (gi + 1 < g.ngroups && g.grp[gi + 1].tile0 <= wt) gi++;
+  const FoldUpdGroup G = g.grp[gi];
+  const int dt = g.d / 64, local = wt - G.tile0;
+  const int r0 = (local / dt) * 32, d0 = (local % dt) * 64;
+  const float nlr = -(g.lr_ptr ? *g.lr_ptr : g.lr);
+  const float* gp[2];
+#pragma unroll
+  for (int mt = 0; mt < 2; mt++) {
+    int r = r0 + 16 * mt + c;
+    if (r > G.rows - 1) r = G.rows - 1;
+    gp[mt] = G.g + (int64_t)r * g.out + 4 * q;
+  }
+  const float* wp = g.w + (int64_t)(4 * q) * g.ldw + G.col0 + d0 + 4 * c;
+  f32x4 acc[2][4];
+#pragma unroll
+  for (int mt = 0; mt < 2; mt++)
+#pragma unroll
+    for (int tn = 0; tn < 4; tn++) acc[mt][tn] = f32x4{0.f, 0.f, 0.f, 0.f};
+  f32x4 a[2], b[4], an[2], bn[4];
+  auto load16 = [&](int k, f32x4* av, f32x4* bv) {
+#pragma unroll
+    for (int mt = 0; mt < 2; mt++) av[mt] = *reinterpret_cast<const f32x4*>(gp[mt] + k);
+#pragma unroll
+    for (int e = 0; e < 4; e++) bv[e] = *reinterpret_cast<const f32x4*>(wp + (int64_t)(k + e) * g.ldw);
+  };
+  load16(0, a, b);
+  for (int k = 0; k < g.out; k += 16) {
+    if (k + 16 < g.out) load16(k + 16, an, bn);
+#pragma unroll
+    for (int e = 0; e < 4; e++)
+#pragma unroll
+      for (int tn = 0; tn < 4; tn++)
+#pragma unroll
+        for (int mt = 0; mt < 2; mt++) acc[mt][tn] = __builtin_amdgcn_mfma_f32_16x16x4f32(b[e][tn], a[mt][e], acc[mt][tn], 0, 0, 0);
+#pragma unroll
+    for (int mt = 0; mt < 2; mt++) a[mt] = an[mt];
+#pragma unroll
+    for (int e = 0; e < 4; e++) b[e] = bn[e];
+  }
+#pragma unroll
+  for (int mt = 0; mt < 2; mt++) {
+    const int r = r0 + 16 * mt + c;
+    if (r >= G.rows) continue;
+    float* erow = G.e + (int64_t)r * G.lde + d0 + 16 * q;
+    f32x4 old[4];
+#pragma unroll
+    for (int i = 0; i < 4; i++) old[i] = *reinterpret_cast<const f32x4*>(erow + 4 * i);
+#pragma unroll
+    for (int i = 0; i < 4; i++) {
+      f32x4 v;
+      v.x = fmaf(nlr, acc[mt][0][i], old[i].x); v.y = fmaf(nlr, acc[mt][1][i], old[i].y);
+      v.z = fmaf(nlr, acc[mt][2][i], old[i].z); v.w = fmaf(nlr, acc[mt][3][i], old[i].w);
+      *reinterpret_cast<f32x4*>(erow + 4 * i) = v;
+    }
+  }
+}
+
 inline bool al16(const void* p) { return ((uintptr_t)p & 15) == 0; }
+
+int fold_table_update_launch(ffh_ctx* c, const ffh_fold_group* groups, int ngroups, const float* w, int64_t ldw, int d, int out, const float* lr_ptr, float lr,
+                             ffh_stream s) {
+  FFH_REQUIRE(c, groups && w && ngroups >= 1 && d > 0 && out > 0 && ldw >= d, "fold_table_update: bad arguments");
+  if (ngroups > FFH_FOLD_MAX_GROUPS || d % 64 || out % FFH_FOLD_NTILE || !al16(w) || ldw % 4)
+    return ffh_fail(c, FFH_ERR_UNSUPPORTED, "fold_table_update: d and out_dim multiples of 64, at most 64 tables, aligned weight");
+  FoldUpdArgs a{};
+  int64_t tiles = 0;
+  for (int i = 0; i < ngroups; i++) {
+    const ffh_fold_group& gr = groups[i];
+    FFH_REQUIRE(c, gr.e && gr.p && gr.rows >= 1 && gr.rows < (1LL << 31) && gr.lde >= d && gr.col0 >= 0 && gr.col0 + d <= ldw, "fold_table_update: bad group");
+    if (!al16(gr.e) || !al16(gr.p) || gr.lde % 4 || gr.col0 % 4) return ffh_fail(c, FFH_ERR_UNSUPPORTED, "fold_table_update: group not aligned");
+    a.grp[i] = FoldUpdGroup{gr.p, const_cast<float*>(gr.e), gr.lde, gr.col0, (int)gr.rows, (int)tiles};
+    tiles += ((gr.rows + 31) / 32) * (d / 64);
+    FFH_REQUIRE(c, tiles < (1LL << 30), "fold_table_update: too many rows");
+  }
+  a.w = w; a.ldw = ldw; a.lr_ptr = lr_ptr; a.lr = lr; a.ngroups = ngroups; a.out = out; a.d = d; a.ntiles = (int)tiles;
+  hipLaunchKernelGGL(fold_table_update_kernel, dim3((unsigned)((tiles + 3) / 4)), dim3(256), 0, as_stream(s), a);
+  FFH_LAUNCH_CHECK(c, "fold_table_update_kernel");
+  return FFH_OK;
+}
+
+int fold_dx_check(ffh_ctx* c, const float* x, int64_t ldx, const float* dx, int64_t lddx, const float* dy, int64_t lddy, const float* w, int in, int out,
+                  int64_t batch, int flags, const int32_t* kept, int nkept) {
+  FFH_REQUIRE(c, in > 0 && out > 0 && batch >= 0 && lddx >= in && lddy >= out, "fold_linear_bwd_dx: bad dims");
+  FFH_REQUIRE(c, !(flags & ~(FFH_LINEAR_DX_OVERWRITE | FFH_LINEAR_DX_MASK_BY_X)), "fold_linear_bwd_dx: flags are DX_OVERWRITE and DX_MASK_BY_X");
+  FFH_REQUIRE(c, !(flags & FFH_LINEAR_DX_MASK_BY_X) || (x && ldx >= in), "fold_linear_bwd_dx: the mask needs x");
+  FFH_REQUIRE(c, batch == 0 || (dx && dy && w), "fold_linear_bwd_dx: null pointer");
+  FFH_REQUIRE(c, batch < (1LL << 31), "fold_linear_bwd_dx: batch too large");
+  FFH_REQUIRE(c, nkept >= 1 && kept, "fold_linear_bwd_dx: bad tile list");
+  for (int i = 0; i < nkept; i++)
+    FFH_REQUIRE(c, kept[i] >= 0 && ((int64_t)kept[i] + 1) * FFH_FOLD_DW_NTILE <= in && (i == 0 || kept[i] > kept[i - 1]), "fold_linear_bwd_dx: tiles must ascend inside [0, in_dim)");
+  return FFH_OK;
+}
+GemmArgs fold_dx_gemm(const float* x, int64_t ldx, float* dx, int64_t lddx, const float* dy, int64_t lddy, const float* w, int in, int out, int64_t batch, int flags) {
+  GemmArgs g{};
+  g.A = dy; g.sAm = lddy; g.sAk = 1;
+  g.B = w; g.sBn = 1; g.sBk = in;
+  g.C = dx; g.ldc = lddx;
+  g.M = (int)batch; g.N = in; g.K = out;
+  g.epi = (flags & FFH_LINEAR_DX_OVERWRITE) ? EPI_STORE : EPI_ADD; g.act = FFH_AC_MODE_NONE;
+  if (flags & FFH_LINEAR_DX_MASK_BY_X) { g.mask = x; g.ldmask = ldx; }
+  return g;
+}
 
 int fold_dw_check(ffh_ctx* c, const float* x, int64_t ldx, const float* dy, int64_t lddy, const float* dw, int in, int out, int64_t batch,
                   const int32_t* kept, int nkept) {
@@ -409,4 +528,39 @@
   return FFH_OK;
 }
 
-}
+int ffh_fold_linear_bwd_dx_plan(ffh_ctx* c, const float* x, int64_t ldx, const float* dx, int64_t lddx, const float* dy, int64_t lddy, const float* w, int in,
+                                int out, int64_t batch, int flags, const int32_t* kept, int nkept, const float* colsum) {
+  const int rc = fold_dx_check(c, x, ldx, dx, lddx, dy, lddy, w, in, out, batch, flags, kept, nkept);
+  if (rc != FFH_OK) return rc;
+  if (batch == 0 || c->math_mode != FFH_MATH_DEFAULT) return 0;
+  const GemmArgs g = fold_dx_gemm(x, ldx, const_cast<float*>(dx), lddx, dy, lddy, w, in, out, batch, flags);
+  return launch_gemm_sk_kept_dx(c, g, kept, nkept, const_cast<float*>(colsum), true, nullptr, "") == 1 ? 1 : 0;
+}
+
+int ffh_fold_linear_bwd_dx(ffh_ctx* c, const float* x, int64_t ldx, float* dx, int64_t lddx, const float* dy, int64_t lddy, const float* w, int in, int out,
+                           int64_t batch, int flags, const int32_t* kept, int nkept, float* colsum, ffh_event record_behind, ffh_stream s) {
+  const int rc = fold_dx_check(c, x, ldx, dx, lddx, dy, lddy, w, in, out, batch, flags, kept, nkept);
+  if (rc != FFH_OK) return rc;
+  ffh_route_clear(c);
+  if (batch == 0 || c->math_mode != FFH_MATH_DEFAULT) return ffh_fail(c, FFH_ERR_UNSUPPORTED, "fold_linear_bwd_dx: empty batch / math mode not served");
+  const GemmArgs g = fold_dx_gemm(x, ldx, dx, lddx, dy, lddy, w, in, out, batch, flags);
+  const int r = launch_gemm_sk_kept_dx(c, g, kept, nkept, colsum, false, s, "fold_linear_bwd_dx gemm");
+  if (r < 0) return r;
+  if (r == 0)
+    return ffh_fail(c, FFH_ERR_UNSUPPORTED, "fold_linear_bwd_dx: the layer's data gradient does not run whole tiles on the persistent kernel, too few kept tiles, "
+                                            "deterministic mode, or column sums without tile 0 / without DX_OVERWRITE");
+  if (record_behind) FFH_HIP_TRY(c, hipEventRecord((hipEvent_t)record_behind, as_stream(s)));
+  return FFH_OK;
+}
+
+int ffh_fold_table_update(ffh_ctx* c, const ffh_fold_group* groups, int ngroups, const float* w, int64_t ldw, int d, int out, float lr, ffh_stream s) {
+  return fold_table_update_launch(c, groups, ngroups, w, ldw, d, out, nullptr, lr, s);
+}
+
+int ffh_fold_table_update_lr(ffh_ctx* c, const ffh_fold_group* groups, int ngroups, const float* w, int64_t ldw, int d, int out, const ffh_lr_state* block,
+                             ffh_stream s) {
+  FFH_REQUIRE(c, block, "fold_table_update_lr: null rate block");
+  return fold_table_update_launch(c, groups, ngroups, w, ldw, d, out, ffh_lr_rate_ptr(block, false), 0.0f, s);
+}
+
+}
diff --git a/dlrm_flexflow_amd/csrc/linear_gemm.h b/dlrm_flexflow_amd/csrc/linear_gemm.h
--- a/dlrm_flexflow_amd/csrc/linear_gemm.h
+++ b/dlrm_flexflow_amd/csrc/linear_gemm.h
@@ -87,5 +87,6 @@
 int launch_gemm_sk_fold(ffh_ctx* c, const GemmArgs& g, const unsigned long long keep[2], int nk_kept, const float* addend, int64_t ldadd, bool dry,
                         ffh_stream s, const char* name);
 int launch_gemm_sk_kept(ffh_ctx* c, const GemmArgs& g, const int* tiles, int nkept, bool dry, ffh_stream s, const char* name);
+int launch_gemm_sk_kept_dx(ffh_ctx* c, const GemmArgs& g, const int* tiles, int nkept, float* colsum, bool dry, ffh_stream s, const char* name);
 
 }
diff --git a/dlrm_flexflow_amd/csrc/linear_sk.hip b/dlrm_flexflow_amd/csrc/linear_sk.hip
--- a/dlrm_flexflow_amd/csrc/linear_sk.hip
+++ b/dlrm_flexflow_amd/csrc/linear_sk.hip
@@ -59,7 +59,8 @@
 
 template <bool AKR, bool BKR, int EPI, bool DB = false, bool SPLIT = false, int TMW = 4, bool FOLD = false, bool KEPT = false>
 __global__ __launch_bounds__(256, 1) void gemm_sk_kernel(const std::conditional_t<KEPT, SkArgsKept, std::conditional_t<FOLD, SkArgsFold, SkArgs>> g) {
-  static_assert(!KEPT || (EPI == SK_EPI_DW_ATOMIC && AKR && BKR && !FOLD), "kept column tiles: the weight-gradient form");
+  static_assert(!KEPT || (!FOLD && ((EPI == SK_EPI_DW_ATOMIC && AKR && BKR) || ((EPI == SK_EPI_DX_STORE || EPI == SK_EPI_DX_ADD) && !AKR && BKR && !DB && !SPLIT && TMW == 4))),
+                "kept column tiles: the weight-gradient form and the whole-tile data-gradient forms");
   static_assert(!FOLD || (EPI == SK_EPI_FWD && !SPLIT && !DB && TMW == 4), "kept k-tiles + addend: the whole-tile forward form");
   static_assert(!DB || (EPI == SK_EPI_DW_ATOMIC && AKR), "the bias gradient rides on the weight-gradient form");
   static_assert(!SPLIT || EPI != SK_EPI_DW_ATOMIC, "the weight gradient meets by atomics");
@@ -608,4 +609,45 @@
   return 1;
 }
 
-}
+int launch_gemm_sk_kept_dx(ffh_ctx* c, const GemmArgs& g, const int* tiles, int nkept, float* colsum, bool dry, ffh_stream s, const char* name) {
+  if (g.N % SK_BN || g.N / SK_BN > 128 || nkept < 1 || nkept > g.N / SK_BN) return 0;
+  for (int i = 0; i < nkept; i++)
+    if (tiles[i] < 0 || tiles[i] >= g.N / SK_BN || (i > 0 && tiles[i] <= tiles[i - 1])) return 0;
+  if (colsum && (tiles[0] != 0 || g.epi != EPI_STORE)) return 0;
+  if (c->deterministic || g.colmap) return 0;
+  SkPlan p{};
+  if (!sk_plan(c, g, SK_FORM_DX, p) || p.split || p.tmw != 4) return 0;
+  const int64_t ntk = (int64_t)(g.M / SK_BM) * nkept, rounds = (ntk + p.G - 1) / p.G;
+  if (ntk < p.G || ntk * 100 < rounds * p.G * 80) return 0;
+  if (dry) return 1;
+  SkArgsKept a{};
+  a.A = g.A; a.B = g.B; a.C = g.C; a.mask = g.mask; a.colsum = colsum;
+  a.lda = p.lda; a.ldb = p.ldb; a.ldc = g.ldc; a.ldmask = g.ldmask;
+  a.M = g.M; a.N = g.N; a.K = g.K; a.act = g.act;
+  a.a_bytes = (unsigned)p.a_bytes; a.b_bytes = (unsigned)p.b_bytes;
+  a.mask_bytes = g.mask ? 1u : 0u;
+  a.nkept = (unsigned)nkept;
+  for (int i = 0; i < nkept; i++) a.tile[i] = (unsigned short)tiles[i];
+  constexpr int LDSB = SK_LDS_KC + SK_LDS_KR;
+#define FFH_SK_KEPT_DX_LAUNCH(EPI)                                                                               \
+  {                                                                                                              \
+    auto kern = gemm_sk_kernel<false, true, EPI, false, false, 4, false, true>;                                  \
+    static std::atomic<signed char> ok[64];       \
+    const int dev = c->device & 63;                                                                              \
+    if (ok[dev].load(std::memory_order_acquire) == 0) ok[dev].store(sk_set_lds(kern, LDSB) ? 1 : -1, std::memory_order_release); \
+    if (ok[dev].load(std::memory_order_acquire) < 0) return 0;                                                   \
+    hipLaunchKernelGGL(kern, dim3((unsigned)p.G), dim3(256), LDSB, as_stream(s), a);                             \
+  }
+  if (g.epi == EPI_STORE) FFH_SK_KEPT_DX_LAUNCH(SK_EPI_DX_STORE)
+  else FFH_SK_KEPT_DX_LAUNCH(SK_EPI_DX_ADD)
+#undef FFH_SK_KEPT_DX_LAUNCH
+  {
+    const hipError_t e = hipGetLastError();
+    if (e == hipErrorInvalidValue || e == hipErrorInvalidConfiguration || e == hipErrorLaunchOutOfResources || e == hipErrorSharedObjectInitFailed) return 0;
+    if (e != hipSuccess) return ffh_fail_hip(c, e, name);
+  }
+  { char tok[96]; snprintf(tok, sizeof tok, "%s|sk_128x128x64|kept=%d/%d%s|wgs=%d", name, nkept, g.N / SK_BN, colsum ? "|colsum" : "", p.G); ffh_route_add(c, tok); }
+  return 1;
+}
+
+}
diff --git a/dlrm_flexflow_amd/host/backend.cc b/dlrm_flexflow_amd/host/backend.cc
--- a/dlrm_flexflow_amd/host/backend.cc
+++ b/dlrm_flexflow_amd/host/backend.cc
@@ -3,6 +3,7 @@
 #include <dlfcn.h>
 #include <cstdio>
 #include <cstdlib>
+#include <cstring>
 #include <map>
 #include <mutex>
 
@@ -178,15 +179,17 @@
   }
   if (dlsym(h, "ffh_fold_abi_version")) {
     KernelApiFold* b = new KernelApiFold();
-#define FFH_LOAD(name)                                                        \
-  b->name = reinterpret_cast<decltype(b->name)>(dlsym(h, #name));             \
-  if (!b->name) {                                                             \
+    const int fold_abi = reinterpret_cast<int (*)(void)>(dlsym(h, "ffh_fold_abi_version"))();
+    auto abi3_entry = [](const char* n) { return !strncmp(n, "ffh_fold_linear_bwd_dx", 22) || !strncmp(n, "ffh_fold_table_update", 21); };
+#define FFH_LOAD(name)                                                        \
+  b->name = reinterpret_cast<decltype(b->name)>(dlsym(h, #name));             \
+  if (!b->name && !(fold_abi == 2 && abi3_entry(#name))) {                    \
     fprintf(stderr, "FATAL: %s exports part of include/ff_hip_fold.h: %s is missing\n", path.c_str(), #name);   \
     abort();                                                                  \
   }
     FFH_FOLD_API_LIST(FFH_LOAD)
 #undef FFH_LOAD
-    if (b->ffh_fold_abi_version() != FFH_FOLD_ABI_VERSION) {
+    if (b->ffh_fold_abi_version() != FFH_FOLD_ABI_VERSION && fold_abi != 2) {
       fprintf(stderr, "FATAL: %s has fold ABI version %d, expected %d\n", path.c_str(), b->ffh_fold_abi_version(), FFH_FOLD_ABI_VERSION);
       abort();
     }
diff --git a/dlrm_flexflow_amd/host/ffmodel.h b/dlrm_flexflow_amd/host/ffmodel.h
--- a/dlrm_flexflow_amd/host/ffmodel.h
+++ b/dlrm_flexflow_amd/host/ffmodel.h
@@ -114,6 +114,7 @@
   bool fold_small_tables;
   int64_t fold_max_rows;
   bool fold_dw;
+  bool fold_dx;
   bool mlp_chain;
   int64_t mlp_chain_max_batch;
   int64_t mlp_chain_fwd_max_batch;
@@ -642,7 +643,13 @@
     float* G = nullptr;
     ffh_ctx* sum_ctx = nullptr;
     void* sum_ws = nullptr;
+    bool dx = false;
   } fold;
+  bool fold_dx_table(const Embedding* e) const;
+  void fold_table_update(ffh_stream s, ffh_ctx* cx) const;
+  ffh_event ev_fold_w_read = nullptr;
+  mutable bool fold_w_read_recorded = false;
+  mutable ffh_event fold_dx_event = nullptr;
   ffh_event ev_fold_e_read = nullptr;
   mutable bool fold_e_read_recorded = false;
   void fold_weight_gradient(const Linear* li, float* dbp, ffh_stream dws) const;
@@ -651,6 +658,7 @@
   mutable bool fold_w_recorded = false, fold_on_side = false;
   void plan_fold();
   void plan_fold_dw(FoldRoute& r);
+  void plan_fold_dx(FoldRoute& r);
   void fold_products_and_sum(ffh_stream s, ffh_ctx* cx) const;
   void fold_linear_forward(const Linear* li) const;
   int z_reader_layer;
diff --git a/dlrm_flexflow_amd/host/ffmodel_c.cc b/dlrm_flexflow_amd/host/ffmodel_c.cc
--- a/dlrm_flexflow_amd/host/ffmodel_c.cc
+++ b/dlrm_flexflow_amd/host/ffmodel_c.cc
@@ -177,6 +177,7 @@
   if (n == "graph_replays") return M(m)->n_graph_replays;
   if (n == "folded_tables") return (int64_t)M(m)->fold.tables.size();
   if (n == "folded_dw_tables") return (int64_t)M(m)->fold.dw_tables.size();
+  if (n == "folded_dx_tables") return (int64_t)(M(m)->fold.dx ? M(m)->fold.dw_tables.size() : 0);
   if (n == "tensor_op_exact_backward_layers") {
     int64_t k = 0;
     for (Op* op : M(m)->layers) if (op->op_type == OP_LINEAR && static_cast<Linear*>(op)->bwd_exact) k++;
diff --git a/dlrm_flexflow_amd/host/model.cc b/dlrm_flexflow_amd/host/model.cc
--- a/dlrm_flexflow_amd/host/model.cc
+++ b/dlrm_flexflow_amd/host/model.cc
@@ -369,6 +369,7 @@
   if (ev_fold_w) api->ffh_event_destroy(ctx, ev_fold_w);
   if (ev_fold_done) api->ffh_event_destroy(ctx, ev_fold_done);
   if (ev_fold_e_read) api->ffh_event_destroy(ctx, ev_fold_e_read);
+  if (ev_fold_w_read) api->ffh_event_destroy(ctx, ev_fold_w_read);
   for (void* p : {(void*)fold.P, (void*)fold.S, (void*)fold.G, fold.sum_ws}) if (p) api->ffh_free(ctx, p);
   if (fold.sum_ctx) api->ffh_ctx_destroy(fold.sum_ctx);
   for (auto& kv : trace_tune) for (ffh_event& e : kv.second.ev) if (e) { api->ffh_event_destroy(ctx, e); e = nullptr; }
@@ -559,7 +560,7 @@
       if (lo) ff.check(ff.api->ffh_linear_bwd_set_dx_colsum(ff.ctx, lo->weights[1].impl->grad, lo->out_channels), "dx colsum");
     }
     ~ColsumScope() { if (lo) lo->db_from_upper = ff.api->ffh_linear_dx_colsum_used(ff.ctx) != 0; }
-  } colsum_scope(ff, colsum_lower, dx != nullptr && (part == 0 || part == 1) && !ff.use_workers() && !ff.config.profiling);
+  } colsum_scope(ff, colsum_lower, dx != nullptr && (part == 0 || part == 1) && !ff.use_workers() && !ff.config.profiling && !(ff.fold.layer == this && ff.fold.dx));
   auto image_dx = [&] {
     if (dx_image && dx) ff.check(ff.api->ffh_convert_f32_to_bf16x3(ff.ctx, dx, b, in_channels, lddx, ff.stream), name);
     if (bwd_exact && dx && dx_twin) ff.check(ff.api->ffh_convert_f32_to_bf16(ff.ctx, dx_twin, dx, b * (int64_t)in_channels, ff.stream), name);
@@ -600,7 +601,13 @@
       ff.check(ff.api->ffh_event_record(ff.ctx, ev, ff.stream), "event");
       ff.check(ff.api->ffh_stream_wait_event(ff.ctx, dws, ev), "event");
     }
-    if (dx) {
+    if (dx && ff.fold.dx) {
+      ffh_event ev = ff.fold_dx_event;
+      ff.fold_dx_event = nullptr;
+      ff.check(ff.api->fold->ffh_fold_linear_bwd_dx(ff.ctx, xp, ldx, dx, lddx, dyp, lddy, wp, in_padded, out_channels, b,
+                                                    flags & (FFH_LINEAR_DX_OVERWRITE | FFH_LINEAR_DX_MASK_BY_X), ff.fold.dw_kept.data(), (int)ff.fold.dw_kept.size(),
+                                                    nullptr, ev, ff.stream), name);
+    } else if (dx) {
       ff.check(ff.api->ffh_linear_bwd_ex(ff.ctx, xp, ldx, dx, lddx, yp, ldy, dyp, lddy, wp, dwp, dbp, in_padded, out_channels, b, (int)activation,
                                          flags | FFH_LINEAR_ONLY_DX, ff.stream, nullptr), name);
       image_dx();
diff --git a/dlrm_flexflow_amd/host/model_allocate.cc b/dlrm_flexflow_amd/host/model_allocate.cc
--- a/dlrm_flexflow_amd/host/model_allocate.cc
+++ b/dlrm_flexflow_amd/host/model_allocate.cc
@@ -981,6 +981,26 @@
     grow += e->num_entries;
   }
   if (!ev_fold_e_read) check((config.timing_events ? api->ffh_event_create : api->ffh_event_create_sync)(ctx, &ev_fold_e_read), "event create");
+  plan_fold_dx(r);
+}
+
+void FFModel::plan_fold_dx(FoldRoute& r) {
+  Linear* li = r.layer;
+  if (!config.fold_dx || r.dw_tables.empty() || !api->fold->ffh_fold_linear_bwd_dx || !api->fold->ffh_fold_linear_bwd_dx_plan || !api->fold->ffh_fold_table_update) return;
+  ffh_sparse_opt rule;
+  if (!fused_embedding_update() || sparse_rule(rule) || !config.overlap_embedding || use_workers()) return;
+  if (lr_route == kLrDevice && !api->fold->ffh_fold_table_update_lr) return;
+  if (li->discard_input_grad || li->colsum_lower || li->inputs[0].impl->grad == nullptr) return;
+  const Embedding* e0 = r.dw_tables[0];
+  if (e0->out_channels % 64) return;
+  const Tensor &x = li->inputs[0], &y = li->outputs[0];
+  const int flags = (li->dx_overwrite ? FFH_LINEAR_DX_OVERWRITE : 0) | (li->dx_mask_by_x ? FFH_LINEAR_DX_MASK_BY_X : 0);
+  const int plan = api->fold->ffh_fold_linear_bwd_dx_plan(ctx, (const float*)x.impl->ptr, x.impl->ld, x.impl->grad, x.impl->grad_ld, y.impl->grad, y.impl->grad_ld,
+                                                          (const float*)li->weights[0].impl->ptr, li->in_padded, li->out_channels, local_rows(y, this), flags,
+                                                          r.dw_kept.data(), (int)r.dw_kept.size(), nullptr);
+  if (plan != 1) return;
+  r.dx = true;
+  if (!ev_fold_w_read) check((config.timing_events ? api->ffh_event_create : api->ffh_event_create_sync)(ctx, &ev_fold_w_read), "event create");
 }
 
 void FFModel::init_layers() {
diff --git a/dlrm_flexflow_amd/host/model_exchange.cc b/dlrm_flexflow_amd/host/model_exchange.cc
--- a/dlrm_flexflow_amd/host/model_exchange.cc
+++ b/dlrm_flexflow_amd/host/model_exchange.cc
@@ -1,6 +1,6 @@
 #include "model_internal.h"
 
-void launch_shard_groups(const FFModel* ff, ShardLaunch what, ffh_stream s, ffh_ctx* cx, const std::vector<const int64_t*>* idx_override) {
+void launch_shard_groups(const FFModel* ff, ShardLaunch what, ffh_stream s, ffh_ctx* cx, const std::vector<const int64_t*>* idx_override, bool all_tables) {
   const bool fwd = what == kGather;
   ffh_sparse_opt rule;
   const bool ruled = (what == kFusedUpdate || what == kApplyOnly) && ff->sparse_rule(rule);
@@ -18,6 +18,7 @@
     t.idx = (const int64_t*)e->inputs[0].impl->ptr;
     if (idx_override && owned_i < idx_override->size()) t.idx = (*idx_override)[owned_i];
     owned_i++;
+    if (!fwd && !all_tables && ff->fold_dx_table(e)) continue;
     t.weight = (float*)e->weights[0].impl->ptr;
     t.num_entries = e->num_entries;
     if (!ff->exchange) {
@@ -115,7 +116,7 @@
 
 void FFModel::embedding_kernels_only(bool fwd, ffh_stream s, const std::vector<const int64_t*>* idx_override) const {
   if (embeddings.empty() || (!fwd && !fused_embedding_update())) return;
-  launch_shard_groups(this, fwd ? kGather : kFusedUpdate, s, ctx, idx_override);
+  launch_shard_groups(this, fwd ? kGather : kFusedUpdate, s, ctx, idx_override, true);
   if (!fwd) advance_bf16_counter(s, ctx);
 }
 
diff --git a/dlrm_flexflow_amd/host/model_flags.cc b/dlrm_flexflow_amd/host/model_flags.cc
--- a/dlrm_flexflow_amd/host/model_flags.cc
+++ b/dlrm_flexflow_amd/host/model_flags.cc
@@ -38,6 +38,7 @@
   fold_small_tables = true;
   fold_max_rows = 7420;
   fold_dw = true;
+  fold_dx = true;
   trace_mode = -1;
   bucket_allreduce = -1;
   allreduce_bucket_floats = 1 << 20;
@@ -149,6 +150,7 @@
     if (is("--no-mlp-chain")) { mlp_chain = false; continue; }
     if (is("--no-fold-small-tables")) { fold_small_tables = false; continue; }
     if (is("--no-fold-dw")) { fold_dw = false; continue; }
+    if (is("--no-fold-dx")) { fold_dx = false; continue; }
     if (is("--fold-max-rows")) { fold_max_rows = atoll(next()); continue; }
     if (is("--always-replay")) { trace_mode = 1; continue; }
     if (is("--adaptive-replay")) { trace_mode = 0; continue; }
diff --git a/dlrm_flexflow_amd/host/model_internal.h b/dlrm_flexflow_amd/host/model_internal.h
--- a/dlrm_flexflow_amd/host/model_internal.h
+++ b/dlrm_flexflow_amd/host/model_internal.h
@@ -56,4 +56,5 @@
 }
 
 enum ShardLaunch { kGather, kFusedUpdate, kSortOnly, kApplyOnly };
-void launch_shard_groups(const FFModel* ff, ShardLaunch what, ffh_stream s, ffh_ctx* cx, const std::vector<const int64_t*>* idx_override = nullptr);
+void launch_shard_groups(const FFModel* ff, ShardLaunch what, ffh_stream s, ffh_ctx* cx, const std::vector<const int64_t*>* idx_override = nullptr,
+                         bool all_tables = false);
diff --git a/dlrm_flexflow_amd/host/model_step.cc b/dlrm_flexflow_amd/host/model_step.cc
--- a/dlrm_flexflow_amd/host/model_step.cc
+++ b/dlrm_flexflow_amd/host/model_step.cc
@@ -134,6 +134,25 @@
                                           fold.dw_kept.data(), (int)fold.dw_kept.size(), dws), li->name);
 }
 
+void FFModel::fold_table_update(ffh_stream s, ffh_ctx* cx) const {
+  const Linear* li = fold.layer;
+  const Embedding* e0 = fold.dw_tables[0];
+  const int ng = (int)fold.dw_groups.size();
+  const float* w = (const float*)li->weights[0].impl->ptr;
+  if (lr_route == kLrDevice) {
+    check(api->fold->ffh_fold_table_update_lr(cx, fold.dw_groups.data(), ng, w, li->in_padded, e0->out_channels, li->out_channels, lr_block[1], s), "fold_table_update_lr");
+  } else {
+    ffh_sparse_opt rule;
+    sparse_rule(rule);
+    check(api->fold->ffh_fold_table_update(cx, fold.dw_groups.data(), ng, w, li->in_padded, e0->out_channels, li->out_channels, rule.lr, s), "fold_table_update");
+  }
+}
+bool FFModel::fold_dx_table(const Embedding* e) const {
+  if (!fold.dx) return false;
+  for (const Embedding* t : fold.dw_tables) if (t == e) return true;
+  return false;
+}
+
 void FFModel::fold_linear_forward(const Linear* li) const {
   if (fold_on_side) check(api->ffh_stream_wait_event(ctx, stream, ev_fold_done), "fold: sum ready");
   else fold_products_and_sum(stream, ctx);
@@ -164,6 +183,12 @@
     check(api->ffh_stream_wait_event(ctx, side_stream, ev_grad_ready), "event");
     if (fold_e_read_recorded) check(api->ffh_stream_wait_event(ctx, side_stream, ev_fold_e_read), "fold: table rows read");
     probe_record(2, side_stream, ctx);
+    if (fold.dx) {
+      if (!fold_e_read_recorded) die("fold: the dx-folded tables' update without this step's segmented sum");
+      fold_table_update(side_stream, ctx);
+      check(api->ffh_event_record(ctx, ev_fold_w_read, side_stream), "fold: weights read");
+      fold_w_read_recorded = true;
+    }
     embedding_group_update(side_stream);
     probe_record(3, side_stream, ctx);
     check(api->ffh_event_record(ctx, ev_update_done, side_stream), "event");
@@ -208,6 +233,8 @@
   if (fin.impl->grad_ld != fin.adim[0] || fin.impl->ld != fin.adim[0]) die("final layer output must be contiguous");
   dw_forked = false;
   fold_e_read_recorded = false;
+  fold_w_read_recorded = false;
+  fold_dx_event = nullptr;
   opt_next_done = false;
   int first = (int)layers.size() - 1;
   emb_update_pending = false;
@@ -269,7 +296,8 @@
   for (int l = first; l >= 0; l--) {
     if (bucketed_now()) issue_grad_buckets(l);
     if (l == grad_attach_layer) {
-      check(api->ffh_event_record_with_next_linear_bwd(ctx, ev_grad_ready), "attach event");
+      if (fold.dx && layers[l] == fold.layer) fold_dx_event = ev_grad_ready;
+      else check(api->ffh_event_record_with_next_linear_bwd(ctx, ev_grad_ready), "attach event");
       grad_ready_attached = true;
     }
     Linear* up = layers[l]->op_type == OP_LINEAR ? static_cast<Linear*>(layers[l]) : nullptr;
@@ -369,6 +397,7 @@
       probe_record(9, stream, ctx);
     }
   }
+  if (fold_w_read_recorded) { check(api->ffh_stream_wait_event(ctx, stream, ev_fold_w_read), "fold: weights read"); fold_w_read_recorded = false; }
   const size_t opt_count = mlp_count;
   const ffh_lr_state* lrb = lr_route == kLrDevice ? lr_block[0] : nullptr;
   if (adam) {
diff --git a/include/ff_hip_fold.h b/include/ff_hip_fold.h
--- a/include/ff_hip_fold.h
+++ b/include/ff_hip_fold.h
@@ -7,7 +7,7 @@
 extern "C" {
 #endif
 
-#define FFH_FOLD_ABI_VERSION 2
+#define FFH_FOLD_ABI_VERSION 3
 
 #define FFH_FOLD_KTILE      16
 #define FFH_FOLD_NTILE      64
@@ -51,12 +51,25 @@
 int ffh_fold_linear_bwd_dw_plan(ffh_ctx* ctx, const float* x, int64_t ldx, const float* dy, int64_t lddy, const float* dw, const float* db, int in_dim,
                                 int out_dim, int64_t batch, const int32_t* kept, int nkept);
 
+
+int ffh_fold_linear_bwd_dx(ffh_ctx* ctx, const float* x, int64_t ldx, float* dx, int64_t lddx, const float* dy, int64_t lddy, const float* w, int in_dim,
+                           int out_dim, int64_t batch, int flags, const int32_t* kept, int nkept, float* colsum, ffh_event record_behind, ffh_stream s);
+
+int ffh_fold_linear_bwd_dx_plan(ffh_ctx* ctx, const float* x, int64_t ldx, const float* dx, int64_t lddx, const float* dy, int64_t lddy, const float* w,
+                                int in_dim, int out_dim, int64_t batch, int flags, const int32_t* kept, int nkept, const float* colsum);
+
+int ffh_fold_table_update(ffh_ctx* ctx, const ffh_fold_group* groups, int ngroups, const float* w, int64_t ldw, int d, int out_dim, float lr, ffh_stream s);
+struct ffh_lr_state;
+int ffh_fold_table_update_lr(ffh_ctx* ctx, const ffh_fold_group* groups, int ngroups, const float* w, int64_t ldw, int d, int out_dim,
+                             const struct ffh_lr_state* block, ffh_stream s);
+
 #ifdef __cplusplus
 }
 #endif
 
 #define FFH_FOLD_API_LIST(X) \
   X(ffh_fold_abi_version) X(ffh_fold_product) X(ffh_fold_gather_add) X(ffh_fold_linear_fwd) X(ffh_fold_linear_fwd_plan) \
-  X(ffh_fold_segment_sum) X(ffh_fold_dw_product) X(ffh_fold_linear_bwd_dw) X(ffh_fold_linear_bwd_dw_plan)
+  X(ffh_fold_segment_sum) X(ffh_fold_dw_product) X(ffh_fold_linear_bwd_dw) X(ffh_fold_linear_bwd_dw_plan) \
+  X(ffh_fold_linear_bwd_dx) X(ffh_fold_linear_bwd_dx_plan) X(ffh_fold_table_update) X(ffh_fold_table_update_lr)
 
 #endif
```

New measurement: 5.316 million samples/s, median of 6. +9.9%, better.
